# mikelodder7/bls-bn254

Hardware: AMD Instinct MI355X
Metric: BN254 pairings/sec (= BLS verifies/sec) (higher is better)
Workload: dtype int64; 1 GPU; 262144 batched single-sig BLS verifies per GPU (BASELINE configs[1]), unique 32-byte messages, 1024-key pool, 1/64 invalid tuples; key de-duplication + hash-to-G1 + per-key G2 checks and line tables + 2-pair Miller loop + final exp; tuples_per_gpu=262144, tuples_total=262144, key_pool=1024

## Files before the change

### bls-bn254_amd/csrc/bn254_consts.h

```cpp
#pragma once
#include <stdint.h>

#ifndef BN_CONST
#define BN_CONST static constexpr
#endif

namespace bnc {
BN_CONST int32_t P[9] = {410844487, 17064118, 477274959, 47522512, 361093496, 47923392, 10936641, 240920116, 3171406};
BN_CONST int32_t PINV = 75916169;
BN_CONST int32_t ONE[9] = {360500257, 337389400, 408039635, 21759001, 178483129, 490881230, 299191303, 86689704, 903222};
BN_CONST int32_t R2[9] = {94088208, 219480995, 25171640, 279645352, 40052281, 46143135, 379321683, 294034764, 2757030};
BN_CONST int32_t R3[9] = {237179570, 381705378, 197673865, 484389131, 296595421, 53368462, 493544588, 282381599, 2540242};
BN_CONST int32_t LC_QINV = 1420063842;
BN_CONST int32_t THREE[9] = {7758947, 475297290, 150377082, 65277005, 535449387, 398901866, 360702999, 260069113, 2709666};
BN_CONST int32_t INV2[9] = {385672372, 177226759, 174221841, 303076213, 269788312, 269402311, 155063972, 163804910, 2037314};
BN_CONST int32_t B2[18] = {189306456, 13619797, 266050167, 47090167, 3383508, 443974981, 116276700, 275414465, 1651051, 463465696, 132959441, 275378631, 215966963, 22334433, 231877312, 116106472, 422158901, 2635577};
BN_CONST int32_t B2_3[18] = {157074881, 23795273, 320875542, 93747989, 185927940, 210259726, 337893461, 48452367, 1781748, 31837202, 364750088, 408456887, 15984952, 418558132, 62914238, 326446135, 247765559, 1563920};
BN_CONST int32_t GAMMA1[5][18] = {{168567705, 446838140, 21606957, 76005147, 193575774, 320063457, 492961205, 101471925, 3016032, 466013235, 394132337, 371054763, 25204381, 93145077, 448361909, 29518381, 483951129, 39811}, {77959568, 116720857, 200831163, 387972444, 449106301, 79574741, 198110247, 444835091, 2396851, 286535409, 187804871, 492312764, 403373079, 442701694, 360078139, 294614062, 104485018, 1269326}, {455018104, 57932550, 320278461, 408777911, 37819167, 383878197, 519288526, 32534274, 1918653, 430327765, 436072363, 496131354, 220163167, 145517765, 530932250, 323946238, 161949718, 1410845}, {276953182, 328873349, 306900296, 55370336, 434202341, 186067288, 221116544, 233072759, 1472337, 258042488, 93586473, 404468614, 107881851, 15098452, 202552781, 251052073, 472003299, 457208}, {122035596, 70559408, 351843991, 185247759, 294359775, 74527549, 415682662, 131659696, 1090544, 515197319, 148204830, 209777112, 355922816, 112506023, 137088316, 422875504, 397322748, 530422}};
BN_CONST int32_t GAMMA2[5][9] = {{239698866, 192365459, 64358326, 265999499, 489041563, 23351122, 297356679, 439555315, 2382159}, {416069521, 391846970, 193189602, 244240497, 310558434, 69340804, 535036287, 352865610, 1478937}, {50344230, 216545630, 69235323, 25763511, 182610367, 93913074, 248616249, 154230411, 2268184}, {171145621, 361569571, 412916632, 318393925, 408922844, 24572269, 250450874, 338235712, 789246}, {531645878, 162088059, 284085356, 340152927, 50535061, 515453500, 12771265, 424925417, 1692468}};
BN_CONST int32_t GAMMA3[5][18] = {{241843517, 234894524, 489670951, 377358109, 130864789, 78929213, 242247822, 507627824, 1062952, 256797489, 98403818, 382339799, 433159222, 464404099, 29325343, 50434485, 281019966, 1260793}, {325889741, 432474136, 497955025, 42907526, 200183625, 441570494, 324828416, 301853753, 830815, 115639766, 437132463, 279613835, 73502212, 128670103, 395362884, 114011013, 518486521, 2516630}, {492697295, 496002479, 156996497, 175615513, 323274328, 200916107, 28519026, 208385841, 1252753, 517387634, 117862666, 518014516, 364230256, 215575730, 53862054, 223861314, 78970397, 1760561}, {184051396, 109191840, 495742184, 2670331, 316545484, 294905530, 164669302, 459358945, 1341039, 164889335, 177818119, 378890167, 153193343, 453739841, 53273248, 261318439, 380451190, 765836}, {51698174, 235788407, 418091187, 111773928, 225157088, 39558942, 371182386, 248871861, 1328219, 456881720, 277261468, 92031488, 462668576, 36360912, 212656789, 36108422, 250118305, 1231319}};
BN_CONST int32_t SVDW1_C2[9] = {25172115, 376708271, 303053117, 281317211, 91305183, 315391993, 392743580, 77115205, 1134092};
BN_CONST int32_t SVDW1_C3[9] = {457867599, 493380231, 379858106, 195829369, 20951404, 495257235, 515507638, 211660318, 1792024};
BN_CONST int32_t SVDW1_C4[9] = {109710923, 387889788, 190128975, 352751795, 248555410, 536056522, 40444610, 278758817, 2582763};
BN_CONST int32_t SVDW2_C1[18] = {12935801, 351009198, 137218890, 68849169, 181866637, 397985299, 415468004, 362104169, 2554273, 463465696, 132959441, 275378631, 215966963, 22334433, 231877312, 116106472, 422158901, 2635577};
// ... 39 lines not shown
 {115099161, 361079548, 480148518, 71065809, 413241065, 213126723, 432045244, 299309372, 2268741, 479074021, 348462957, 481692425, 148329581, 64011363, 70419451, 521873344, 159891040, 1324744, 119836463, 250094397, 193017529, 386788224, 428020408, 460771368, 482124439, 421522847, 2425238, 114910552, 328830817, 11540419, 482736450, 81017752, 486418694, 265295458, 205803990, 2412182, 471973933, 150650886, 367600592, 532165343, 430851147, 71155045, 529417599, 178863249, 2191828, 149969822, 426570128, 207472835, 315629756, 133685872, 381189636, 408236876, 327074418, 2188814},
 {2478238, 482236155, 501863109, 216695776, 28133897, 438520593, 478660467, 318003266, 1199697, 192081406, 317937999, 456709271, 526466273, 394728539, 38972406, 212519731, 400106547, 2012913, 378934760, 47780458, 414894863, 300049921, 288627557, 408469358, 444317404, 488663036, 2672762, 13086186, 54236397, 108682135, 92393923, 530514305, 27778254, 105809252, 74710849, 1556614, 209361150, 110510140, 95590690, 157282884, 446948412, 348799352, 455938463, 212273705, 163832, 22070713, 354671070, 84392107, 19937692, 97762133, 428281814, 341164088, 59197099, 2715522},
 {323421647, 351258179, 370279306, 155471307, 424415674, 102275476, 212021690, 87559554, 2340702, 24917374, 235021524, 380342478, 363149794, 227411753, 120703908, 347780407, 368601500, 1628846, 507626604, 130345934, 352142788, 446766788, 227299145, 486890448, 454258698, 432658924, 408411, 387464107, 181431778, 517543077, 450507408, 274152061, 386795811, 316647274, 2653065, 905024, 198687098, 19198232, 468880961, 497531179, 72028957, 445451261, 151597031, 505066845, 266617, 206165872, 383877063, 381756925, 495881619, 309259073, 79698217, 517080274, 394408755, 2370170},
 {330978764, 415936193, 276560320, 10789241, 32709856, 415578960, 204566554, 49026968, 543671, 401282904, 295457946, 459543498, 302532038, 234545929, 435390597, 51269616, 516181269, 989503, 266870546, 37427281, 314094762, 90273590, 90847638, 271513304, 186487054, 352454449, 2617924, 121748973, 147192770, 247959206, 301823486, 444621093, 436582923, 209240503, 422347226, 2002793, 420766975, 95012043, 358452079, 193159195, 332239088, 408573222, 533896885, 168668931, 923997, 225978358, 445442889, 464494416, 256553974, 330088769, 112529492, 268007525, 39581098, 1275248},
 {185059858, 384384543, 195532834, 80761347, 97799465, 380065039, 58976876, 123141856, 1462600, 186838709, 402104131, 276126867, 284741457, 500488675, 514410526, 383061266, 124796755, 2244826, 358011933, 4036403, 469238339, 440068960, 527373348, 334506535, 314766696, 488109457, 2091722, 220763289, 483546112, 315308719, 294479989, 264693218, 504773378, 400722538, 128766796, 1203159, 65502050, 407313301, 102089550, 95898178, 179009806, 249585945, 234878215, 121313140, 2105165, 522286217, 258485470, 418821949, 263539889, 530843810, 16465869, 522864618, 524681011, 866705},
 {491409221, 429532559, 480645853, 526305085, 519184946, 320384023, 366557187, 456445003, 2372451, 46004574, 88114142, 272844542, 240504887, 245152710, 72343087, 452772496, 490931390, 1930332, 365820376, 405670191, 215780242, 398527698, 97510772, 57808733, 25497632, 300993947, 1861604, 101472942, 268743662, 483215740, 262103703, 80623359, 433243363, 270577248, 136079810, 1692806, 526258616, 299110836, 467583615, 175386471, 241633693, 128812340, 475159413, 424889297, 1355872, 334828240, 46302060, 197547862, 437505136, 209280222, 106201003, 250871306, 428783560, 1572123},
 {65131922, 410853902, 281504673, 233607083, 165164706, 161931360, 387368130, 258266354, 2803919, 334380832, 303564680, 469329650, 483978437, 60138085, 65833456, 505774265, 488845355, 732811, 194000581, 438170323, 339874851, 141778324, 114422087, 230441886, 438429275, 99559190, 2946642, 6220226, 12487337, 220716112, 200924448, 81207124, 390196574, 461793634, 229660081, 2302755, 306224412, 191690856, 481273302, 249777865, 233058066, 485912801, 218562582, 429376852, 1812935, 255465103, 179692905, 1478937, 74345539, 513148142, 382481949, 310578590, 389597509, 1275258},
 {275949305, 3228312, 176617213, 302484708, 457024271, 263059331, 258622837, 245199256, 753406, 83841931, 325585899, 277349460, 285128688, 326328912, 15480993, 328169666, 377039357, 2396459, 113270026, 65870630, 96437477, 351096554, 325570632, 198444115, 76462694, 155120365, 996406, 430904607, 193902953, 272620064, 90269516, 102608309, 337293318, 397393431, 355475286, 1895729, 375002109, 523542794, 420835100, 244089057, 314065940, 170681387, 283594264, 200076913, 2351283, 353523119, 365025453, 508021136, 56738678, 102892269, 28605850, 410461759, 165297750, 821801},
 {121101037, 453866970, 408871889, 451715554, 319641813, 194199547, 316486552, 91089131, 808524, 120712549, 135431654, 172072906, 201228322, 470008586, 492966518, 374156269, 532936882, 1168971, 139848472, 40102183, 376920765, 120695385, 9222022, 119036174, 436556597, 431412384, 2480448, 23738614, 100086658, 394051529, 460935441, 426465533, 18451757, 232407558, 515618330, 3011560, 519254845, 256846000, 49605046, 137916175, 344616592, 289345685, 442010228, 227801899, 2750281, 504706552, 99608927, 62959779, 78824121, 378301691, 404974492, 52973827, 431879000, 2103752},
 {57437006, 445209922, 267906252, 61434842, 322380891, 448223867, 314779795, 384467504, 98050, 334623576, 504282724, 410457003, 436857817, 525051919, 379539104, 397162175, 488788414, 1675650, 128798474, 528278283, 271532147, 514886753, 436331545, 85538213, 175830542, 327291145, 2932702, 208811182, 439681250, 485915822, 399974237, 30558037, 318044875, 130194579, 172655195, 2132450, 111448047, 492105644, 275356637, 284787949, 242551611, 425462594, 410102729, 25366096, 965123, 377085709, 111491603, 279628206, 536659377, 363545763, 491060748, 301344554, 217747788, 1765858},
 {189278316, 267054422, 240015347, 263190437, 268026589, 217837374, 213394387, 324721961, 1939655, 362977484, 158704421, 436353096, 498602143, 463553294, 108055305, 173810290, 461672636, 189796, 355213020, 343977698, 358822065, 74044511, 88139862, 518079515, 72571544, 488865441, 562373, 93928340, 179514280, 470213355, 1500725, 59659302, 351864698, 514900587, 277607281, 746298, 424483532, 62821806, 533803893, 328740056, 62104696, 109448841, 488087329, 28719095, 615035, 503689154, 324055796, 273308548, 138602345, 93139326, 227059809, 225062543, 520012847, 1690627},
 {434873579, 345866943, 464692431, 147843125, 214244731, 167340668, 8535887, 135091946, 590262, 507331706, 281122125, 71877124, 182009353, 98073037, 426692907, 256966410, 31385127, 323754, 339206185, 397108277, 158683218, 198966473, 323954183, 410647148, 250511836, 182487353, 2192260, 211663655, 166315194, 278738998, 465340566, 135530598, 220476821, 98038085, 475663347, 689443, 238385349, 45648702, 24191268, 223060677, 56805038, 492858003, 15855826, 219362042, 3169653, 55560961, 496756213, 531337177, 231583741, 370701323, 20903764, 26651393, 72508891, 2939698},
 {370857545, 162561793, 349584675, 305666799, 424318849, 265355541, 335744858, 332264862, 2077939, 229675399, 202135034, 507349300, 66038434, 502299596, 462886795, 216432890, 367950568, 434967, 522930393, 349612231, 359055418, 269223224, 415375677, 73806834, 81410003, 7609490, 2168856, 440219586, 266804181, 348682996, 471526334, 56329094, 445035356, 495708785, 177697745, 1049347, 9590362, 463810573, 472790040, 104478950, 123428722, 344683645, 15445838, 441601197, 345029, 127193134, 22917997, 445375356, 264481634, 418186335, 190775382, 385157115, 441341282, 1622947},
 {525120466, 302156262, 14026670, 79200301, 83863473, 269053555, 271350554, 5118602, 814247, 242412219, 10262438, 115069724, 182751693, 222411097, 463282269, 302495598, 467832431, 433135, 381586988, 376949966, 525473891, 378543561, 528450195, 305002078, 5175203, 530287687, 1864236, 8631814, 399428070, 64818853, 409693044, 53480096, 59985746, 424529766, 117917599, 1958550, 211074005, 241353131, 202088806, 153585924, 274879141, 376560831, 74310929, 362992403, 3023538, 304629166, 231842783, 202606994, 59312311, 437826184, 276953349, 202252965, 152929408, 1380202},
 {45243310, 3113997, 475224255, 399655383, 489901630, 394589394, 219453609, 389562620, 647105, 185052378, 203306772, 510086849, 66201807, 28034831, 265674449, 483208661, 117079303, 2245361, 383725158, 56590503, 238874043, 474720702, 354626127, 5216587, 380497232, 382251138, 2156761, 450163084, 327454365, 96195373, 340957541, 93272866, 447418125, 393654147, 336425233, 1261490, 243056404, 202839389, 291276410, 39489301, 522755053, 433239394, 200191913, 132407280, 995738, 87800718, 39891742, 201642557, 267980703, 381147787, 142064039, 166874100, 148109070, 2183155},
 {419483032, 417302961, 209411699, 395420027, 11875312, 472825098, 25023783, 122248361, 428482, 187120796, 434311260, 523941697, 312353488, 185625814, 149803502, 25267919, 437641082, 58048, 482147204, 44437673, 333141396, 416903804, 328735750, 68751396, 54000275, 18754495, 469924, 118281153, 196797377, 510480140, 174090217, 180762717, 327840995, 522381987, 342541943, 526514, 29386787, 379334880, 495343353, 138079880, 149085614, 205670571, 338603247, 518281092, 947371, 28951025, 167201315, 357427458, 165861015, 133055956, 147545106, 497514072, 418967957, 3122782},
 {40100442, 79249802, 481205136, 295669236, 516832659, 295740353, 154473360, 42698217, 616919, 459226082, 367489041, 172493783, 10772752, 310333315, 469796297, 456832918, 360513025, 1387582, 439740854, 47345612, 232672811, 422188955, 500323364, 225266534, 163349333, 306515768, 477242, 1545029, 11878491, 315137521, 386388304, 482799752, 234821666, 494159689, 490739196, 2025658, 285921861, 387365880, 273585049, 37311821, 367688208, 434533702, 464362157, 527184610, 954346, 423936018, 309641240, 457531941, 133017943, 116916181, 145496292, 266826109, 174694208, 2322607},
 {103410007, 80269727, 107803116, 266138348, 159613881, 218210149, 270129094, 176926138, 1971950, 309770860, 398343381, 531806047, 171136374, 168818136, 221670885, 445114296, 275892636, 1101592, 163848103, 166760855, 355771815, 124065591, 415188034, 189131208, 248659651, 402708254, 845530, 148218911, 225224981, 183319510, 1438760, 465281999, 261483438, 422864871, 401738498, 504587, 259044379, 431246755, 284927319, 98392988, 492002560, 58293889, 86402116, 213719941, 265596, 252917965, 237345777, 96756592, 402569146, 168468661, 174375631, 211020977, 148122777, 1839569},
 {129175245, 7036991, 394205927, 109118652, 420701990, 532730783, 488070123, 230275807, 2505420, 321568924, 108179418, 122921434, 177770554, 127113816, 508034739, 2160192, 484284904, 868789, 464634736, 175998503, 492000730, 81605521, 144765489, 520986768, 305919411, 374066204, 1890535, 237833058, 199277185, 484650377, 114512057, 271342938, 136767975, 392520660, 135535363, 237972, 13806109, 25620002, 460701052, 81031906, 83471693, 347825173, 448355234, 165472987, 2836179, 302810733, 180092351, 371937405, 67528704, 521484666, 251274010, 324067318, 98241568, 319197},
 {402590907, 390173797, 9154836, 91637093, 116097568, 135498950, 412674480, 471852445, 2103104, 45623282, 236388520, 320757064, 250739701, 507203558, 20784063, 349913224, 513830445, 2930463, 191231464, 229262617, 499329381, 391457563, 220103625, 381273631, 121452801, 230708984, 498416, 147675469, 451341783, 356690434, 416036715, 453518419, 195069465, 248991557, 21133377, 2515482, 261837599, 70126348, 170486479, 536345815, 457557007, 123485984, 176457550, 352037844, 849911, 261382441, 87117387, 517387878, 11753697, 168073425, 454808552, 195965950, 96105394, 152175},
 {12512508, 150856564, 395596226, 482091269, 260215011, 354438027, 103441014, 126419430, 252738, 185766822, 521899918, 261643314, 35208125, 305510146, 363820929, 116324864, 100331033, 889085, 500803016, 169611288, 74978053, 271459858, 455136968, 68056467, 40076531, 480527470, 1897865, 429796490, 142915065, 500099793, 459002478, 523553815, 134475327, 405370676, 140840092, 549968, 210967111, 414065589, 351375835, 413127406, 104682486, 235355711, 345576955, 518068253, 1825719, 121695489, 84303843, 520551157, 246713071, 76169206, 128032100, 440504967, 283651112, 366320},
 {54903692, 367398404, 389045954, 103195443, 201407156, 480670888, 520034811, 444665162, 3120009, 301192230, 292344168, 276000918, 329190306, 3207403, 16097252, 377466566, 108801895, 994934, 105164645, 400152816, 477217800, 290340033, 389232304, 248469600, 306422360, 405666417, 1265718, 149978886, 10882107, 96650353, 374648105, 145056091, 209481887, 236014373, 478750587, 1172417, 444164896, 369905875, 51408743, 373893873, 98743229, 307012172, 257015135, 227181011, 2381844, 74179049, 426041869, 180979714, 318267506, 239942663, 263940057, 98072905, 311978671, 150141},
 {142543935, 194580705, 343370161, 391345662, 400042802, 407410933, 413139956, 149550188, 1289303, 528816066, 209720920, 443679922, 400086828, 52320843, 454328967, 413721629, 77976075, 2253187, 63450331, 336126245, 200366993, 8503761, 143191089, 388781579, 24290118, 17560612, 1567680, 243745881, 20656753, 365319391, 73839146, 311195635, 406562419, 388374104, 497778204, 3159579, 268334596, 285203294, 517702133, 517615536, 191607223, 305927169, 398996176, 435289825, 2199364, 296375027, 511422668, 142534303, 147541973, 486527664, 61071306, 133290627, 151365941, 1871814},
 {381447695, 112910439, 164681691, 372267774, 388906816, 442672654, 510817020, 138003284, 2517538, 425925494, 321328277, 407413632, 350272519, 159281071, 490821086, 202786933, 286727689, 2119816, 55117854, 313308608, 360606396, 31742223, 248771333, 255469023, 125500679, 80632572, 2951938, 172822145, 292032153, 304786787, 355702891, 253612283, 295485534, 208552501, 432316545, 2682878, 110822812, 210734962, 393571010, 96421268, 38795732, 58694143, 397188728, 387473943, 102932, 206765486, 143677095, 226830287, 496832911, 260610526, 345967722, 332677737, 83704810, 3148352},
 {62108095, 226732454, 161554664, 324339612, 474398800, 445689529, 310205044, 313295877, 1595036, 521570690, 127595162, 438734366, 44995759, 228814373, 19627764, 211169583, 247295664, 1457005, 60863200, 454338684, 63660680, 436100826, 109781091, 65244919, 193527964, 354189242, 1393252, 219704311, 38957286, 110544435, 160893735, 455670807, 348774005, 138075414, 285707688, 2608894, 1804324, 271533511, 299758214, 352967878, 95296562, 186071519, 83272051, 302583396, 3001394, 128153566, 500555465, 271034625, 432533768, 477284868, 92329198, 324969194, 32623276, 130038},
 {215582193, 126912476, 309311231, 10076884, 314222891, 377366770, 530443407, 477083200, 793328, 533386876, 492530023, 503245648, 91516679, 182906897, 194062228, 492389562, 65590782, 1324892, 38561070, 245414554, 189970182, 152394919, 426151917, 512289777, 22015761, 436702070, 1185947, 52392166, 143466253, 184054606, 364397472, 432510246, 197302902, 148253681, 4271025, 931440, 360382279, 38184803, 427074753, 343932430, 308401295, 504780952, 201263072, 266062393, 424201, 111188963, 450073465, 372852080, 68120216, 21855192, 136104731, 230467091, 249100444, 3131167},
 {503242147, 126031175, 99598615, 332469802, 118529903, 103654630, 336983131, 48695070, 1281178, 122799682, 274622884, 507281707, 415629719, 306308862, 223464264, 75647452, 467875001, 1287621, 286610889, 85716239, 122268177, 517793089, 118854096, 284240661, 109341172, 523299060, 2430687, 247263262, 94849538, 54280861, 507432969, 291253094, 256077794, 441645252, 213205037, 2917285, 155215960, 392828217, 154713476, 366149965, 187736848, 395762272, 411133922, 457751113, 1834994, 523850929, 350840427, 299600675, 379383303, 402170387, 224236460, 187366553, 196507477, 392568},
 {261404048, 60806940, 100479668, 287812062, 271915223, 198406602, 238340931, 408086811, 1901426, 324109934, 513219976, 214408304, 345497341, 221162477, 531649800, 49370849, 170138307, 1040769, 332267139, 126565143, 105261738, 156831366, 427218173, 526690558, 398325027, 48992578, 3150187, 148926025, 82340276, 232496043, 105691656, 409427567, 191008174, 462567125, 144338561, 719208, 136997521, 211607581, 55265913, 93560900, 155893330, 50711175, 522835196, 432651475, 1167786, 104425542, 178779151, 290349679, 84423272, 313764025, 519966625, 405776928, 459400273, 2933873},
 {310825741, 384456194, 426889952, 532157184, 489413414, 222371274, 254619296, 305726429, 1200037, 226431895, 191449196, 147394219, 512980816, 112239727, 123673014, 345317845, 68260117, 1834849, 158028187, 373938733, 55317016, 281026384, 386220711, 418030963, 103573954, 71301023, 478347, 23351998, 306678241, 111291365, 453611291, 112088103, 99686904, 79519778, 510270407, 926535, 214206952, 82455080, 241084664, 103779255, 360047249, 26043312, 42338008, 263251530, 2293413, 431541426, 164219745, 91904174, 107196656, 359655013, 207187685, 211089583, 28421216, 2693257},
 {128984559, 408128418, 354064874, 279268254, 470256108, 48320565, 91070471, 175298789, 521515, 339864578, 231958707, 225812807, 90243946, 198929659, 262631414, 187740668, 131953518, 679825, 302468239, 395971309, 196126185, 197552126, 16644241, 520798160, 194513995, 448317350, 2671784, 88087896, 328335140, 144335943, 102062007, 340283116, 286846647, 176155623, 365474765, 2487316, 363197687, 306159665, 453821877, 77580983, 243190174, 115169461, 197970032, 182888387, 163558, 134896947, 35963039, 144316924, 219126585, 120283426, 274799187, 533258181, 527633730, 480391},
 {341746340, 308302796, 430625402, 101511254, 466164565, 480666054, 127770429, 443615350, 2308080, 31431165, 319419446, 227721353, 416355218, 141796468, 120324224, 177014659, 409950156, 1927475, 251290807, 478940226, 446910893, 212080491, 429870139, 311429590, 433888467, 97060592, 2428767, 308935399, 254634792, 494014342, 484461508, 175949596, 222997971, 507697494, 6855563, 198079, 331310478, 8636836, 78610090, 167333250, 276995305, 320565486, 401578983, 468493720, 186082, 443619717, 57975269, 125159984, 199762973, 384348548, 303284969, 146339162, 141845832, 1661690},
 {380822515, 156254098, 174290075, 379414457, 498231268, 451298257, 449171729, 433962997, 1742136, 195831119, 281549253, 311228002, 399685262, 205543257, 93314873, 366022684, 481414289, 964076, 360837042, 96132473, 323506526, 129202646, 438203512, 195211450, 25899375, 118356221, 267310, 276216682, 373509754, 38238354, 220219388, 80173204, 222174402, 128252521, 284030621, 959358, 499785411, 80697964, 282876190, 191336693, 179576951, 247438212, 357625786, 298992331, 1304370, 318099190, 58142073, 352186437, 84637684, 459118970, 185918866, 263207063, 136859350, 17203},
 {22201984, 265618155, 5732562, 312280272, 428285398, 399081532, 390586660, 195672556, 384993, 197544349, 359334084, 379212116, 533597950, 121884326, 345868827, 250766308, 176976589, 2405209, 150296893, 352839861, 187428747, 309943127, 398751357, 183724921, 90389245, 393368450, 1055795, 193582117, 421104415, 345293445, 131519433, 445932976, 357186327, 87574441, 195345724, 2546016, 390825220, 219248238, 282044142, 139758925, 128477841, 37456477, 445576370, 475394833, 2077533, 50169050, 205628584, 22939628, 483296354, 138203379, 489066399, 528359038, 87569497, 1779567},
 {485635694, 91489940, 369095772, 277539277, 69873299, 58285921, 140553732, 404251382, 2338306, 384638836, 65644667, 41235970, 423864904, 172015351, 369068400, 268252068, 306791038, 409687, 30563928, 183319989, 102070816, 85226297, 514801246, 240250988, 532874397, 449593201, 2734700, 207295019, 516870558, 429981826, 110660854, 477085381, 429989041, 52354241, 150924792, 1646533, 113663700, 536839513, 306803055, 112881191, 439661605, 246706288, 18664305, 501459450, 1317964, 341627473, 76166713, 146626525, 1733909, 8778891, 371460037, 535514595, 103941542, 2880078},
 {219122481, 521376588, 48819747, 453090089, 232489950, 529687297, 126590199, 192595820, 2170623, 158964325, 138670954, 70538403, 433509637, 268378921, 159736347, 167078372, 472007564, 2642738, 146711122, 180163548, 79656276, 62999074, 427174551, 174151461, 236927641, 94058253, 827399, 498654006, 153397663, 31817787, 244161073, 334416319, 71911351, 298777560, 319420192, 2250830, 299438274, 421802083, 189128091, 59988885, 196191526, 48343, 23947445, 384065173, 2999593, 222421153, 352796023, 419827954, 204257747, 197219243, 481381734, 483432526, 136798688, 2510232},
 {471399504, 225290108, 479825663, 208285264, 95998907, 247686025, 476587084, 415349662, 2989291, 415430977, 42648197, 36657301, 434095102, 342823308, 92920887, 189264745, 364268235, 3098747, 236437400, 450843323, 95084128, 118707480, 37831298, 505369479, 80648224, 409498161, 516702, 383869702, 412856052, 472404438, 404526549, 520906484, 262355910, 465546569, 176317220, 384400, 307844836, 237693820, 335097902, 439545630, 248997287, 116103597, 43530126, 360074078, 887654, 256539533, 189232881, 521948944, 130137976, 494864697, 533420778, 467441818, 242664914, 2360911},
 {6341116, 258953661, 130165135, 121567663, 85734040, 362525194, 446386664, 221487232, 2418285, 67600948, 254157951, 226775185, 363959709, 120458917, 42640378, 417110163, 232465096, 3078420, 427739614, 188726393, 495980930, 324226172, 384839974, 411097953, 276079125, 472007051, 859799, 164129877, 494401711, 448417012, 366162538, 6462208, 155008799, 72770354, 166128252, 2791168, 227075349, 108651955, 255460112, 376253096, 521726666, 203860061, 217738487, 89258585, 1761282, 438061118, 265245702, 341611701, 71841372, 494561940, 345314017, 454454515, 308232774, 512869},
 {388123801, 82315330, 42726244, 478978184, 473426981, 319753532, 223939613, 159127356, 716500, 91233489, 486241299, 190304271, 364630277, 369664745, 215648258, 16385655, 360116749, 1604186, 292146332, 131277078, 438844626, 524436726, 498055021, 91158254, 171272336, 82826493, 2900140, 237091141, 248682792, 356460465, 216723839, 48245380, 247622337, 483244203, 179351009, 2746259, 116116257, 365456058, 154479586, 192349368, 85192525, 289995721, 112977154, 92335699, 136314, 452992599, 385210575, 1099038, 238791418, 18935313, 89476660, 301485804, 217597180, 2954969},
 {136943908, 18208356, 404922159, 463169914, 311803918, 346171465, 11838672, 423116572, 540100, 141896998, 195863719, 45697336, 192503381, 256542019, 81673477, 43642530, 38848267, 1468289, 508779843, 75730439, 209636058, 457851658, 304698551, 458293478, 392091706, 422667130, 468044, 398299416, 470320832, 173064410, 465823042, 365112625, 59195844, 439497728, 70241388, 2477266, 419402448, 215564443, 199572801, 265196137, 177356156, 176224811, 196089759, 315451236, 108510, 136072149, 428681825, 334127467, 452465188, 203237528, 73965396, 232642935, 428577660, 734022},
 {440860920, 83597737, 71788760, 4773679, 460570279, 223207920, 436035796, 398734372, 656541, 481111816, 66740800, 118181206, 218954997, 242302821, 354825473, 189551084, 288107682, 1228799, 79417144, 142486372, 312428128, 275428832, 316981410, 237485005, 224672500, 191667892, 495131, 412962820, 462769059, 312027323, 119892722, 218910436, 5847613, 239249143, 479317593, 138253, 337396732, 218879545, 30296354, 13955357, 421024186, 57906020, 191012581, 137209362, 2722985, 135005313, 375307002, 418714293, 327448236, 516046957, 298981707, 281311663, 232523326, 787909},
 {421882971, 346072605, 213508351, 124603514, 12713635, 387029899, 153312083, 356938635, 3135484, 185025588, 392430028, 30735720, 162160774, 68103380, 68360853, 56078781, 374528341, 1284754, 97299261, 147709562, 382526238, 25706632, 411103733, 17887524, 102419314, 158212278, 2179507, 68756409, 408623604, 525390344, 331525772, 69339206, 464082682, 137855506, 393884866, 3019165, 300006882, 173952888, 216039979, 255807306, 176378987, 388535127, 280690262, 536698090, 2484175, 468135898, 34190575, 211134462, 454582962, 169066562, 330433300, 483525464, 387667530, 148723},
 {332227983, 57357084, 334050684, 43489651, 482498330, 304681939, 341896219, 443742571, 2437451, 12250895, 160665840, 219191270, 36256471, 386592779, 444851143, 325838334, 352243405, 1474793, 479082934, 431105170, 97846306, 105778213, 138739391, 505974881, 147824753, 72435794, 2757268, 106049943, 25102438, 360775953, 376983765, 122671492, 333355075, 52176328, 435301593, 715756, 532854540, 193948231, 505703644, 523162571, 218455565, 509630947, 8980570, 358113216, 920581, 13158795, 17751672, 57746186, 414675497, 472210620, 4708792, 226710205, 49341192, 1376576},
 {430955708, 264381247, 337096023, 351853749, 20383220, 411008042, 59652391, 330831616, 2659533, 408978128, 191887919, 105571894, 232797019, 43766784, 309332417, 268493775, 33580806, 1649466, 264590990, 346513002, 245153061, 291939935, 302699159, 458351889, 422831022, 172176136, 2582643, 249931154, 155575599, 37643848, 494072352, 83127062, 216595132, 119157193, 144910063, 1938120, 301984105, 187990127, 519334054, 103086537, 482009609, 426075322, 524567878, 105731577, 3056969, 135091568, 190493310, 134058471, 383578297, 451388586, 306348237, 362414496, 152852857, 2313526},
 {156049048, 348569387, 345912211, 108243764, 39862758, 340985293, 526986285, 486529373, 2756757, 70148830, 361656205, 232267683, 499676662, 55080252, 11325608, 388061743, 373594328, 877029, 397671269, 400681839, 65130041, 262490050, 283062759, 405415808, 461459608, 489448736, 2202039, 397115625, 518867667, 227573257, 57170780, 47003329, 192147289, 32943434, 36595122, 2904836, 418071867, 224056616, 380555394, 61600834, 220544322, 101581422, 126185470, 370629032, 1587125, 422449844, 210141206, 495244492, 159725210, 393378025, 459104351, 413093230, 535784292, 2467414},
 {374971361, 189256118, 514349215, 260192216, 201693892, 46684475, 86038945, 45798971, 596475, 354780560, 166199176, 126676648, 20087358, 8163231, 443871444, 380934380, 15879837, 2832889, 52684906, 521371086, 390867791, 101904211, 260915672, 182440845, 68224676, 228157599, 2402653, 8442567, 370238665, 105072341, 281343440, 475493017, 519100621, 421211414, 331232706, 2713541, 415194087, 506485752, 184326039, 87917025, 118769502, 421077858, 366086855, 347850511, 643412, 210607613, 239757828, 257344574, 176541047, 126352649, 461160536, 325971653, 410321501, 1859419},
 {346138147, 183589712, 192669952, 440482540, 335490519, 23087938, 38013450, 414816160, 11088, 402635274, 508754875, 528205898, 260674993, 208706555, 339115408, 323234820, 179171832, 2221386, 426553627, 112047373, 385712345, 300968502, 341498138, 355471730, 142898578, 70820285, 1765035, 281326098, 143615771, 294300190, 343890894, 12537596, 236250928, 171742033, 81667137, 2226899, 25416948, 345664344, 167296106, 520318029, 241956023, 57184892, 494901324, 60468401, 2000935, 2993812, 152844357, 515142068, 274834179, 461835240, 279725567, 239967821, 348485226, 1472537},
 {430272925, 523309779, 159176126, 64114552, 7599812, 275194210, 227486424, 402628020, 2147710, 32902820, 490191070, 54357085, 533266873, 395036647, 424428525, 535518286, 280410232, 2920968, 296779742, 412228251, 503765170, 218914658, 241878384, 230177558, 468682218, 424848977, 1394588, 233801316, 236752259, 172198580, 293699517, 62687391, 221253270, 499455778, 153199542, 3046004, 279442699, 160682080, 321402742, 22130196, 534886950, 418643497, 231459356, 133404613, 1211833, 455283136, 111355409, 446906248, 441602466, 348034517, 263104034, 400474216, 170955027, 2605900},
 {436035161, 247373067, 125798067, 389725623, 6288592, 42833077, 516498379, 521445566, 1886790, 184263419, 48195789, 422452995, 231173944, 533728815, 88671371, 207203408, 367383526, 2267220, 203108664, 193164284, 180890202, 528984086, 354640285, 258786511, 136754148, 530754252, 2435046, 412114265, 158840910, 4204732, 381206110, 524422907, 105857206, 48027475, 171131517, 1288815, 235451170, 399660963, 214158541, 316727956, 497939107, 332057718, 116914421, 231502284, 67606, 420272217, 412168364, 271325459, 335552449, 90905491, 64178567, 201413962, 442922653, 1121259},
 {299184217, 414960404, 318291790, 185622238, 367049483, 402495234, 341748370, 437982520, 2045795, 19477984, 249305720, 429912029, 461389527, 315066191, 275999417, 180961226, 139859282, 2826593, 39144516, 55422143, 4587787, 206150160, 396564513, 477425243, 495183114, 206289587, 6552, 117906371, 101024087, 510444434, 453278004, 175014561, 229819228, 350767294, 441008500, 3142255, 7426088, 133832626, 356941477, 309926291, 274258323, 486660256, 289374288, 235101466, 357776, 34819623, 244190314, 358405397, 443658477, 357664916, 174948832, 204568663, 198916489, 1795169},
 {344880916, 485864836, 128038544, 183700157, 303951303, 417725573, 29735238, 331651302, 1803381, 354013505, 44946024, 97088622, 470300883, 10632754, 49099620, 532392985, 471635872, 444945, 182853991, 422119400, 276418095, 116677872, 48565822, 5255579, 432637183, 237201307, 949170, 402960287, 234588459, 424200806, 60774998, 201936971, 269440315, 135570892, 497241165, 1473037, 98814076, 69597269, 71295596, 514821842, 217886650, 153833815, 131588020, 427103757, 966636, 295915695, 460908713, 377597627, 517877798, 458919916, 225274860, 124292261, 111683940, 2746827},
 {518656702, 488249738, 7278702, 290418227, 225912336, 394700482, 530898514, 259426784, 1978070, 361278641, 183914759, 52646095, 242709033, 72608589, 219216813, 56677820, 330469468, 2371300, 428300565, 180500926, 160633184, 517116766, 10598290, 22285930, 316776114, 126200239, 1447245, 478054283, 132434667, 127134921, 299595849, 231458914, 188088751, 465838830, 156854382, 1010051, 124319470, 431725364, 256338614, 513617633, 270873983, 212643967, 248921239, 519052682, 2280194, 306994602, 241460816, 250923483, 31965397, 19740949, 213555458, 216627367, 45246112, 120116},
 {293160492, 245941755, 73442732, 404135672, 207614525, 120178985, 379937182, 89551655, 621586, 79473740, 337984177, 79264647, 93294149, 7971693, 393334056, 368916157, 81801052, 2106207, 440306136, 503791711, 479588939, 489491137, 410166973, 14621930, 505587363, 488473959, 887037, 380514496, 52096291, 310971389, 45923102, 370044752, 93285453, 332980638, 63634843, 1130600, 392821194, 418824308, 240376313, 224275292, 455434369, 277669007, 371906250, 373704681, 310847, 331214354, 510727251, 123531010, 152463125, 442565065, 42499403, 310012621, 233375412, 1687544},
 {459544001, 391471594, 25575482, 192315806, 512283260, 229830790, 296261571, 189785566, 1994877, 533652656, 511037612, 138939831, 267891826, 271878679, 362676324, 403256550, 7446027, 1593828, 398539344, 524236377, 201010774, 383778641, 315414171, 26786658, 123832312, 185180095, 2602473, 213570084, 481028506, 53314778, 168675715, 346762600, 456335430, 134019067, 372692310, 1393242, 31664457, 47744192, 466416925, 304247197, 340814346, 87836883, 327891107, 332472178, 1815581, 227941551, 222271169, 9261168, 405098383, 161968106, 375092235, 169346447, 46544412, 781100},
 {481548188, 214741736, 240350070, 12012500, 377756157, 270945313, 50135567, 45913065, 884284, 456765927, 289042023, 195839783, 67043321, 432298369, 280901733, 96207641, 420493817, 2718622, 388852431, 322343875, 283482318, 315017940, 465898945, 349554570, 53095133, 226022090, 2016489, 392942489, 334126532, 394229114, 60241890, 35434634, 280761896, 416868051, 351542500, 2734105, 283240893, 88720328, 344233496, 511860616, 128181406, 282487018, 181873990, 6976297, 3167753, 477651976, 456530921, 317767618, 190821317, 233115539, 139469982, 367863448, 58909471, 1662784},
 {202767458, 453256221, 40761137, 446365799, 365985752, 446050190, 497895002, 41047040, 3095360, 74607829, 444889648, 523552515, 145945486, 404457399, 251028894, 93766472, 372001962, 100303, 170138087, 193614804, 318792614, 439536147, 477434124, 228485055, 534091926, 155749842, 2276449, 405215224, 444385000, 524465072, 211904860, 30038886, 442931262, 502463559, 152695011, 2089704, 149956433, 312575983, 59240429, 436435538, 62833367, 11191233, 438260993, 17344802, 1937400, 439218886, 403065571, 193234881, 12915827, 501712098, 93787484, 392498397, 403859438, 1016411},
 {436656284, 359905360, 101223246, 489351504, 3657958, 384101949, 411196791, 380427572, 2571034, 393485923, 208952735, 521386055, 481096, 239270552, 32414421, 179291139, 171927397, 969014, 498233196, 178876263, 470532999, 2665997, 469647577, 229911587, 74856801, 112939172, 2001555, 416183585, 181587888, 175524846, 491051689, 408447450, 455605718, 324931618, 4689734, 488914, 333638614, 401276274, 535821439, 48345823, 316619007, 298189350, 409219897, 220762652, 989429, 186867115, 260273710, 349435877, 403490373, 93917204, 144732036, 175749141, 388077615, 2517682},
 {287574667, 195537458, 497438093, 285360180, 145888726, 33019073, 258962939, 137762083, 2183989, 514390807, 414879403, 400777039, 371818954, 184570898, 380591635, 54817320, 467430913, 420463, 270933454, 498342011, 116808119, 403954222, 342364641, 30811629, 67526331, 369389871, 69412, 109168654, 89512855, 320028402, 418325651, 410409818, 275971329, 98753658, 373947392, 131243, 406899020, 164738448, 66826334, 481117969, 514460024, 117856498, 439611387, 301623572, 881303, 254359548, 150778625, 397147446, 400927161, 311807650, 291267789, 210433882, 458123653, 889392},
 {529634438, 395020387, 108093242, 475767096, 289150317, 237339105, 438871389, 229144053, 863679, 367571939, 57943390, 252342320, 453230619, 534849941, 39507622, 256714209, 97288288, 502696, 476782345, 227320360, 12420741, 239942260, 428908049, 370993522, 524227993, 117952539, 39613, 524531981, 381845637, 465982430, 272568792, 16808060, 153088464, 296339629, 371493215, 2469462, 421277729, 389812836, 167537784, 365554318, 128762787, 447247816, 123616227, 145939449, 928609, 397386148, 336421292, 521321073, 247639461, 229285539, 85996274, 383972709, 258664804, 1653094},
 {206961616, 381079739, 269593227, 402726100, 14538206, 444867933, 70904296, 387084730, 842917, 363453306, 416500523, 467532540, 413073582, 447013703, 179563435, 162474537, 245531731, 1148209, 252576564, 285412103, 88916683, 43311484, 96753579, 364204461, 372433977, 262971741, 1488142, 514833759, 441119544, 214499877, 381724849, 532269602, 170892059, 462648916, 394029910, 3088805, 317182934, 203370385, 229723113, 167901654, 420180670, 421862275, 475961650, 157282786, 606030, 170565178, 133408998, 307215134, 140651646, 274714847, 428926323, 210858395, 437580467, 1611559},
 {428117646, 34022814, 154722467, 132755685, 122068739, 493618771, 139622274, 172498314, 2847252, 291633030, 274194775, 531858012, 144402698, 196681234, 9258711, 314775141, 528082404, 2673935, 463441689, 123768625, 3948302, 86001732, 338857223, 191043638, 119408198, 52181253, 1749096, 359249064, 109688593, 94402094, 181413537, 186492090, 24969004, 488664237, 449160119, 406543, 114508015, 102789443, 459719719, 408889277, 26876464, 115711357, 287223829, 481968893, 1990518, 439490694, 75124594, 294181975, 526377703, 197129499, 271661232, 471150834, 30721416, 2422508},
 {242939259, 412783622, 471303906, 192058816, 105613554, 200351016, 185651272, 116111166, 380075, 116919016, 44980791, 118255186, 336201211, 492185226, 215423527, 535352552, 298494615, 330685, 468809653, 273377370, 415937808, 356085620, 305055772, 234561145, 115126109, 412038193, 2330777, 226531982, 531939410, 196877215, 205982089, 450956423, 184374411, 43456923, 326110495, 1332390, 495507394, 153926551, 386101394, 312990856, 210150327, 83320656, 174813766, 401693105, 2304832, 142919764, 427347211, 262488407, 255935794, 267272831, 363987954, 192572795, 414162563, 311899},
 {492850946, 83178123, 253668660, 474965034, 436447538, 24145095, 79743109, 174938088, 1825060, 319698026, 215683917, 224311769, 170490546, 382977480, 425031066, 458737052, 519196122, 490490, 23400646, 413713278, 183752261, 122853282, 307960228, 485960869, 506338186, 323599517, 2359325, 128015026, 98186099, 186918078, 500109092, 265222921, 384663883, 336091284, 78604597, 1543388, 528217684, 519346581, 136688447, 135308455, 417532446, 532591185, 366571968, 264784252, 1490877, 59145682, 93913550, 246772293, 374924084, 76451296, 496346135, 115518558, 400766082, 2779322},
 {74427174, 316623412, 23675861, 334126763, 13176646, 232809289, 155541939, 72228454, 2041212, 223546547, 39809592, 430026316, 461496123, 103565608, 186511401, 376911596, 173378117, 2013790, 148348236, 428852572, 533703899, 8051787, 259534980, 154770121, 287113594, 176515032, 2128049, 304215290, 285689321, 49950046, 312168505, 56098899, 396352110, 106689639, 83980306, 112317, 428157728, 421524631, 342427138, 493639879, 178570351, 279205191, 19926514, 340648123, 537251, 205965075, 487813757, 479910751, 261176063, 22342432, 483891590, 78435476, 443577918, 40148},
 {245617288, 123175829, 297826511, 458896068, 241764471, 231632607, 359840708, 280803868, 1903173, 208825547, 199996367, 459909105, 234782504, 76292385, 515020774, 464695317, 335518206, 1507300, 443788596, 506199681, 325325070, 285054850, 513447046, 300959514, 350146814, 261232659, 1056560, 511066014, 165963439, 506953704, 224195656, 167564066, 85118324, 450098451, 528850463, 2136823, 454347216, 490807827, 399975633, 229421869, 164096225, 459597559, 326414675, 336617775, 2755194, 373766664, 351697410, 127130679, 260765326, 100562905, 479367856, 368211999, 293492131, 1866570},
 {245059318, 463441635, 322639623, 428310962, 276526834, 259438497, 259460084, 284033542, 1914551, 446196205, 71389884, 28378485, 227051864, 24899243, 319354978, 403507892, 142246580, 1035731, 383275586, 383407055, 62259511, 43124759, 438435885, 220904326, 67527927, 451988882, 1158168, 265697257, 192397136, 283611844, 241128875, 224521733, 507674344, 505150213, 313413044, 2764367, 88931525, 125647936, 210359394, 81090266, 400614554, 488361106, 91717877, 376314259, 2657259, 124767231, 515059692, 169614140, 147285524, 148427957, 469343083, 405195547, 184094142, 2282633},
 {283949290, 224585391, 387868692, 134470700, 303193727, 448046774, 352543777, 211263354, 2798858, 194293620, 393760483, 497938725, 503905221, 429888991, 80080179, 498291004, 175629855, 2516950, 352383472, 134024744, 163753863, 347850850, 85651656, 214018496, 350423646, 346299626, 923916, 247508017, 297963687, 273418374, 173382835, 52468082, 519077880, 116994839, 282382304, 917907, 223092338, 327407993, 65285009, 51077305, 57230120, 288595597, 358338612, 353896855, 3000924, 361066685, 148632114, 424642269, 118560696, 213195914, 102741443, 396098212, 463778511, 80713},
 {283112081, 62163922, 15285746, 184678173, 416946919, 422793912, 427895760, 169272309, 478315, 493550027, 267712255, 22406168, 366289293, 534932369, 314255603, 228325538, 106989998, 2279429, 278652919, 455265061, 491187464, 515942130, 439087513, 55731747, 165162718, 226315791, 1706004, 419312073, 331338263, 501464547, 23996291, 88136940, 346944743, 441707665, 244460432, 1716749, 216670401, 179999684, 532912431, 315997436, 1457314, 463396740, 412632783, 529692613, 1363030, 15814396, 455016475, 358234367, 324799376, 507454070, 191107457, 48521367, 535342990, 469131},
 {353724426, 246951758, 356895745, 263153409, 166221217, 527460908, 408776437, 180329720, 2074466, 350542864, 172693688, 528929391, 449515530, 242628823, 502634791, 325881967, 326418351, 2824014, 6211503, 172822135, 487595616, 235534058, 83694625, 250324374, 59949222, 358315171, 140984, 456021003, 245324642, 478802151, 358788042, 86103668, 11744115, 84313809, 326569761, 1543169, 65445570, 99254724, 261961647, 242735888, 158766603, 422676747, 54714193, 95543337, 2526467, 379539315, 142863568, 420734362, 133156177, 479080502, 331652827, 361501306, 195531172, 476820},
 {317549885, 198697761, 249380953, 495123692, 453947158, 249203722, 86749406, 417148591, 1475877, 237283213, 3241341, 423184088, 18795847, 427863335, 16040214, 110200455, 251524210, 1536713, 107639984, 20072597, 149189468, 428015298, 504385698, 37314867, 385750891, 414404719, 27851, 33958399, 385169620, 498529230, 401284295, 454333519, 321731256, 390462645, 184294845, 3078660, 494095629, 58065239, 58845098, 384312739, 456755048, 286073792, 286791495, 339282540, 2514723, 514391628, 359967790, 36516999, 194259209, 203785548, 255357864, 504836880, 394958850, 726555},
 {311633655, 131811432, 25398033, 403841593, 322115575, 411293880, 18124295, 313074943, 1758952, 465227322, 342407623, 150372597, 248889719, 483108493, 484579230, 497417539, 52196962, 835321, 385381891, 33104285, 128891397, 175809299, 508462802, 113213291, 143378814, 330223714, 3111509, 8907364, 425999037, 12685138, 129991581, 183470742, 354061234, 479225391, 324114126, 794985, 104661603, 134083376, 498763072, 523935167, 84413167, 420274427, 372011915, 266936511, 1832300, 245545999, 459057437, 317368478, 118888668, 205600319, 155899518, 528397898, 148747741, 2503274},
 {281479439, 528562003, 363098899, 336344374, 334922502, 19252294, 219010773, 120096268, 334925, 469435664, 522063190, 321990810, 322313526, 34411411, 155471800, 439756490, 13265237, 2678778, 307714251, 387237933, 281157113, 458703192, 295248262, 150067309, 239439310, 458374633, 294731, 505677572, 418978856, 261146195, 418595975, 48411027, 317828536, 428175647, 395441932, 2462780, 102022309, 268732306, 533037255, 196300118, 309364786, 353571676, 169172951, 455255622, 617142, 100882411, 18013065, 473322700, 1072795, 361513363, 288652241, 15588916, 481236440, 1708153},
 {78571987, 361177887, 443998338, 263075369, 70263042, 493726944, 535962191, 127043271, 240062, 397136396, 210646202, 390127152, 167668320, 248745889, 101020297, 476579152, 219747776, 2761125, 41140832, 184387078, 146744831, 256252326, 49807238, 449542423, 227261990, 260471214, 3062208, 525127283, 301154849, 324701277, 365662396, 341585785, 211435912, 180828780, 33088091, 1542729, 277290806, 363851994, 435830295, 358876156, 309952369, 71088530, 33326580, 365431691, 2484596, 228693420, 442482570, 179541425, 186143321, 468865264, 184526935, 430176262, 329282558, 1978018},
 {334852098, 447934948, 79443961, 129228070, 24354253, 48477975, 454023539, 409993992, 2734970, 252455794, 88354609, 238705096, 337451121, 509324887, 377113426, 353457692, 484461504, 3151075, 30273128, 38294371, 95800251, 283261923, 11148736, 412039228, 283771755, 78282908, 332934, 466452697, 408280540, 68630333, 400795547, 363393231, 451322782, 513557020, 87708113, 2516599, 1474989, 245982418, 413800578, 447897561, 302850044, 426778887, 172716362, 449729011, 905236, 446215920, 174849968, 188780190, 128296608, 187418943, 281206446, 333755580, 368298541, 534803},
 {363697647, 285325938, 434722059, 45579462, 201973848, 474212666, 509636120, 184182192, 2064968, 234715851, 38141659, 178588306, 534136360, 7939644, 350012596, 12958086, 298819088, 2993351, 216734195, 240593912, 425991579, 523032660, 208302347, 46323594, 225474280, 435024773, 620780, 218895451, 112326747, 455023803, 408508051, 293004444, 376821145, 226784757, 60787535, 203412, 89496320, 94265377, 166096921, 444267378, 388934921, 180246479, 82754499, 199580496, 1055662, 397155459, 158822569, 235174623, 386896911, 163916411, 273528224, 411861325, 410622147, 328359},
 {201488625, 50957238, 102304395, 380060116, 223771241, 130517402, 435321712, 299390440, 2235652, 108535259, 444775626, 77579088, 31956246, 210186067, 306243370, 385817896, 372735497, 321894, 385233421, 180622935, 409074521, 198964499, 283286026, 308937856, 399091608, 264124425, 1002653, 96082886, 457455230, 184729783, 483382084, 41502754, 223103679, 41738397, 295708136, 2011427, 226581221, 308353232, 355792123, 466623293, 297947519, 355198579, 2931546, 491778089, 1313650, 64242208, 249109684, 65494917, 93199926, 276018694, 138777245, 129213055, 389657785, 1072199},
 {45705453, 143714487, 86307088, 78913109, 147374975, 180957191, 151133129, 489339976, 1771405, 473819502, 18118557, 535636238, 480177567, 333137611, 375380390, 286843472, 468899487, 2820877, 384183509, 191736051, 225531995, 291298185, 245563785, 502637833, 161583766, 457641843, 725657, 495758470, 499253568, 253172769, 342707160, 105926098, 70835746, 86210055, 18923348, 1992080, 475781590, 43350802, 343223350, 458816390, 91405471, 412690255, 460119077, 198442996, 1152636, 260405015, 266436221, 492905943, 532643754, 101236968, 286896498, 298117023, 69177552, 1088979},
 {142623616, 73447938, 472968444, 281091874, 108821799, 419205582, 252984000, 82673195, 1081090, 370209387, 255472044, 183573082, 80973558, 27971357, 21261924, 281424325, 422863884, 2866203, 226861365, 297493201, 87406300, 200247153, 515720525, 243992102, 251901746, 261600094, 1404379, 30950022, 226078069, 96689508, 302682309, 219162382, 53852572, 307069894, 520566561, 519903, 312360512, 399813465, 147484965, 45860077, 366845051, 485642865, 202533828, 245786935, 2240314, 483140654, 424156184, 171736471, 392447265, 310743250, 285399021, 231132855, 110553928, 1580353},
 {518950315, 166524578, 318973779, 208801084, 203654704, 518574409, 367342361, 212732044, 267211, 346834938, 311664457, 28289258, 166837241, 185476264, 240293064, 27521832, 41500912, 1827852, 192671097, 463723310, 318425315, 219804188, 228021022, 450959355, 320662857, 355567309, 381911, 54390987, 531844638, 277544222, 259123543, 351332576, 198209147, 230796763, 144375015, 1532825, 313852906, 129182620, 290984000, 322011448, 398352613, 263155621, 226583053, 196853404, 1278929, 326310244, 117621872, 410625076, 82125642, 397095880, 409752438, 248834139, 338630724, 1320201},
 {55878625, 108956286, 398558293, 380795966, 327699164, 96727383, 441060671, 240953991, 485316, 335290700, 164606168, 447327121, 346715094, 3829772, 157458878, 207194831, 80360049, 320838, 8715817, 280742723, 46597024, 443039108, 287762215, 93179656, 466061073, 203112441, 2378325, 79434527, 121708912, 229280302, 10141767, 246110096, 93770821, 391394252, 478945112, 696660, 367903438, 292984164, 303749863, 10248808, 474419406, 225020304, 479091881, 505749740, 917582, 155299559, 269273660, 392448063, 36485923, 93297644, 265708075, 431439551, 207339751, 1846136},
 {493808963, 482302668, 204399090, 362293888, 514159840, 378918588, 426691502, 472571071, 2351725, 413910404, 15913881, 204492988, 247758060, 412134986, 115823135, 66968791, 299334015, 1262480, 188930798, 194294115, 45816802, 99693215, 358389925, 168281711, 63684769, 296317229, 2275024, 438763849, 504132989, 531624029, 187379805, 61104814, 363323519, 377087611, 256199988, 2311937, 167379084, 375468130, 502802420, 67689135, 41456191, 503979958, 305671863, 354691468, 317874, 60197100, 137848056, 55566537, 386244007, 258790455, 13634469, 73766086, 292447699, 1528865},
 {248938176, 350466153, 134753901, 435380835, 72917553, 156155176, 291307518, 32259336, 1028390, 379779376, 231645262, 229723036, 193965067, 153531491, 375312851, 491839129, 441506130, 1041786, 115764437, 313016821, 369953093, 454752130, 484813132, 417728943, 512613884, 477427683, 2993031, 253811470, 122990100, 443458760, 301470983, 82635724, 51241845, 135246996, 100410326, 735740, 106669830, 500727615, 185253398, 80759155, 174390583, 427362052, 435938546, 75098748, 2455921, 158248225, 274759410, 28245215, 72408984, 11419683, 86345775, 16182697, 81920639, 3124442},
};
#endif
```

### bls-bn254_amd/csrc/fp29.h

```cpp
#pragma once
#include <stdint.h>
#include "bn254_consts.h"

#if defined(__HIPCC__)
#include <hip/hip_runtime.h>
#define BN_HD __host__ __device__
#else
#define BN_HD
#endif
#define BN_INL BN_HD inline __attribute__((always_inline))
#ifdef BN_FORCE_INLINE
#define BN_FUNC BN_INL
#else
#define BN_FUNC BN_HD inline
#endif

#define BN_UNROLL _Pragma("unroll")
#if defined(__HIP_DEVICE_COMPILE__)
#define BN_SCHED_BARRIER __builtin_amdgcn_sched_barrier(0)
#else
#define BN_SCHED_BARRIER ((void)0)
#endif

#ifdef BN_CHECK
// ... 353 lines not shown
  ok = c < 0;
  return fp_to_mont(x);
}
BN_INL void fp_to_be(uint8_t* b, const Fp& a) {
  Fp c = fp_from_mont(a);
  uint32_t w[8];
  limbs_to_words(w, c.l);
  BN_UNROLL for (int j = 0; j < 8; ++j) store_be32(b + 4 * (7 - j), w[j]);
}
BN_INL Fp fp_from_okm(const uint8_t* okm) {
  uint32_t w[12];
  BN_UNROLL for (int j = 0; j < 12; ++j) w[j] = load_be32(okm + 4 * (11 - j));
  Fp lo, hi;
  BN_UNROLL for (int i = 0; i < NL; ++i) {
    int bit = RB * i, j = bit >> 5, s = bit & 31;
    uint32_t v = w[j] >> s;
    if (s > 32 - RB) v |= w[j + 1] << (32 - s);
    lo.l[i] = (int32_t)(v & (uint32_t)MASK);
  }
  BN_UNROLL for (int i = 0; i < NL; ++i) {
    int bit = RB * (i + NL), j = bit >> 5, s = bit & 31;
    uint32_t v = 0;
    if (j < 12) { v = w[j] >> s; if (s > 32 - RB && j + 1 < 12) v |= w[j + 1] << (32 - s); }
    hi.l[i] = (int32_t)(v & (uint32_t)MASK);
  }
  BN_TRK(set_trk(lo, 0, 1, 0, 1, 170); set_trk(hi, 0, 1, 0, 0, 1e-30);)
  return fp_dot2(lo, fp_const(bnc::R2), hi, fp_const(bnc::R3));
}

struct Exp256 { uint64_t w[4]; };
#define BN_EXP(name) (::bn::Exp256{{bnc::name[0], bnc::name[1], bnc::name[2], bnc::name[3]}})
BN_FUNC Fp fp_pow(const Fp& a, Exp256 e) {
  Fp tab[16];
  tab[0] = fp_one();
  tab[1] = fp_norm(a);
  for (int i = 2; i < 16; ++i) tab[i] = fp_mul(tab[i - 1], tab[1]);
  const uint64_t e0 = e.w[0], e1 = e.w[1], e2 = e.w[2], e3 = e.w[3];
  Fp r = tab[(int)(e3 >> 60)];
  for (int w = 62; w >= 0; --w) {
    uint64_t word = w >= 48 ? e3 : w >= 32 ? e2 : w >= 16 ? e1 : e0;
    int d = (int)((word >> ((w & 15) * 4)) & 15);
    Fp t = tab[d];
    BN_SCHED_BARRIER;
    r = fp_sqr(r); r = fp_sqr(r); r = fp_sqr(r); r = fp_sqr(r);
    r = fp_mul(r, t);
  }
  return r;
}
BN_FUNC Fp fp_inv_pow(const Fp& a) { return fp_pow(a, BN_EXP(EXP_PM2)); }

BN_INL void sg_divsteps29(int32_t& zeta, uint32_t f, uint32_t g, int32_t& u, int32_t& v, int32_t& q, int32_t& r) {
  u = 1; v = 0; q = 0; r = 1;
  BN_UNROLL for (int i = 0; i < RB; ++i) {
    int32_t c1 = zeta >> 31;
    const int32_t c2 = -(int32_t)(g & 1u);
    const uint32_t x = (f ^ (uint32_t)c1) - (uint32_t)c1;
    const int32_t y = (u ^ c1) - c1, z = (v ^ c1) - c1;
    g += x & (uint32_t)c2; q += y & c2; r += z & c2;
    c1 &= c2;
    zeta = (zeta ^ c1) - 1;
    f += g & (uint32_t)c1; u += q & c1; v += r & c1;
    g >>= 1; u *= 2; v *= 2;
  }
}
template <bool MODP>
BN_INL void sg_update(int32_t* a, int32_t* b, int32_t u, int32_t v, int32_t q, int32_t r) {
  int64_t ca = (int64_t)u * a[0] + (int64_t)v * b[0], cb = (int64_t)q * a[0] + (int64_t)r * b[0];
  int32_t ka = 0, kb = 0;
  if (MODP) {
    ka = (int32_t)(((uint32_t)ca * (uint32_t)bnc::PINV) & (uint32_t)MASK); kb = (int32_t)(((uint32_t)cb * (uint32_t)bnc::PINV) & (uint32_t)MASK);
    ca += (int64_t)ka * bnc::P[0]; cb += (int64_t)kb * bnc::P[0];
  }
  ca >>= RB; cb >>= RB;
  BN_UNROLL for (int i = 1; i < NL; ++i) {
    const int32_t ai = a[i], bi = b[i];
    ca += (int64_t)u * ai + (int64_t)v * bi; cb += (int64_t)q * ai + (int64_t)r * bi;
    if (MODP) { ca += (int64_t)ka * bnc::P[i]; cb += (int64_t)kb * bnc::P[i]; }
    a[i - 1] = (int32_t)((uint32_t)ca & (uint32_t)MASK); b[i - 1] = (int32_t)((uint32_t)cb & (uint32_t)MASK);
    ca >>= RB; cb >>= RB;
  }
  a[NL - 1] = (int32_t)ca; b[NL - 1] = (int32_t)cb;
}
constexpr int SG_BATCHES = 21;
BN_FUNC Fp fp_inv(const Fp& a) {
  const Fp x = fp_from_mont(a);
  int32_t f[NL], g[NL], d[NL], e[NL];
  BN_UNROLL for (int i = 0; i < NL; ++i) { f[i] = bnc::P[i]; g[i] = x.l[i]; d[i] = 0; e[i] = i == 0 ? 1 : 0; }
  int32_t zeta = -1;
  for (int b = 0; b < SG_BATCHES; ++b) {
    int32_t u, v, q, r;
    sg_divsteps29(zeta, (uint32_t)f[0] | ((uint32_t)f[1] << RB), (uint32_t)g[0] | ((uint32_t)g[1] << RB), u, v, q, r);
    sg_update<false>(f, g, u, v, q, r);
    sg_update<true>(d, e, u, v, q, r);
  }
  int32_t gnz = 0;
  BN_UNROLL for (int i = 0; i < NL; ++i) gnz |= g[i];
#if defined(__HIP_DEVICE_COMPILE__)
  if (__builtin_amdgcn_ballot_w64(gnz != 0) != 0) return fp_inv_pow(a);
#else
  if (gnz != 0) return fp_inv_pow(a);
#endif
  const bool neg = f[NL - 1] < 0;
  Fp di;
  BN_UNROLL for (int i = 0; i < NL; ++i) di.l[i] = neg ? -d[i] : d[i];
  BN_TRK(set_trk(di, -1, 1, -0.14, 0.14, 22);)
  return fp_mul(di, fp_const(bnc::R2));
}
BN_FUNC Fp fp_sqrt_cand(const Fp& a, bool& is_sq) {
  Fp y = fp_pow(a, BN_EXP(EXP_PP1_4));
  is_sq = fp_eq(fp_sqr(y), a);
  return y;
}

BN_INL uint32_t bn_funnel_shr(uint32_t hi, uint32_t lo, uint32_t k) {
#if defined(__HIP_DEVICE_COMPILE__)
  return __builtin_amdgcn_alignbit(hi, lo, k);
#else
  return (uint32_t)((((uint64_t)hi << 32) | lo) >> k);
#endif
}
BN_FUNC bool fp_is_square(const Fp& x) {
  Fp c = fp_canon(x);
  uint32_t a[8], n[8];
  limbs_to_words(a, c.l);
  limbs_to_words(n, bnc::P);
  uint32_t t = 0;
  for (int it = 0; it < 520; ++it) {
    const uint32_t k = (uint32_t)__builtin_ctz(a[0] | 0x80000000u);
    BN_UNROLL for (int j = 0; j < 7; ++j) a[j] = bn_funnel_shr(a[j + 1], a[j], k);
    a[7] >>= k;
    t ^= k & ((n[0] >> 1) ^ (n[0] >> 2));
    const uint32_t odd = a[0] & 1u;
    uint32_t d[8], borrow = 0;
    BN_UNROLL for (int j = 0; j < 8; ++j) {
      const uint64_t v = (uint64_t)a[j] - n[j] - borrow;
      d[j] = (uint32_t)v; borrow = (uint32_t)(v >> 63);
    }
    const uint32_t swap = odd & borrow;
    t ^= swap & ((a[0] & n[0]) >> 1);
    const uint32_t sm = 0u - swap, om = 0u - odd;
    uint32_t carry = swap, nz = 0;
    BN_UNROLL for (int j = 0; j < 8; ++j) {
      const uint64_t v = (uint64_t)(d[j] ^ sm) + carry;
      carry = (uint32_t)(v >> 32);
      n[j] = swap ? a[j] : n[j];
      a[j] = (a[j] & ~om) | ((uint32_t)v & om);
      nz |= a[j];
    }
#if defined(__HIP_DEVICE_COMPILE__)
    if (__builtin_amdgcn_ballot_w64(nz != 0) == 0) break;
#else
    if (nz == 0) break;
#endif
  }
  return (t & 1u) == 0;
}

}
```

### bls-bn254_amd/csrc/host_verify.hip

```cpp
#include "host_common.h"

extern "C" {


int launch_g2_prepare(blsbn254_ctx* c, hipStream_t s, const uint8_t* pks, const uint32_t* keys, size_t u, int32_t* raw, uint8_t* ok, const uint32_t* d_u) {
  if (c->quad_prep && 8 * u <= c->lanes_per_round)
    return launch(c, s, "g2_prepare", grid_lanes(2 * 256 * (size_t)nblocks(4 * u)), k_g2_prepare_quad, pks, keys, (uint32_t)u, raw, ok, d_u);
  return launch(c, s, "g2_prepare", grid_lanes(2 * 256 * (size_t)nblocks(u)), k_g2_prepare, pks, keys, (uint32_t)u, raw, ok, d_u);
}
int prepare_keys_async(blsbn254_ctx* c, const uint8_t* d_pks, const uint32_t* d_keys, size_t u, int32_t* table, uint8_t* key_ok, const uint32_t* d_u) {
  HIPCHK(c, c->prep_raw.reserve(u * PREP_RAW_LIMBS * 4));
  HIPCHK(c, fork_stream2(c));
  TRY(launch_g2_prepare(c, c->stream2, d_pks, d_keys, u, (int32_t*)c->prep_raw.p, key_ok, d_u));
  TRY(launch(c, c->stream2, "g2_expand", grid_lanes(u * (size_t)BN_NEG_G2_LINES), k_g2_expand, (const int32_t*)c->prep_raw.p, (uint32_t)u, table, d_u));
  HIPCHK(c, hipEventRecord(c->ev_join, c->stream2));
  return 0;
}
int check_key_indices(blsbn254_ctx* c, const uint32_t* d_kid, size_t n, size_t u, uint32_t* hist, const char* what, bool armed) {
  if (!armed) { HIPCHK(c, c->misc.reserve(64)); TRY(min_index_arm(c, (int*)c->misc.p, 1)); }
  int* d_bad = (int*)c->misc.p;
  HIPCHK(c, hipMemsetAsync(hist, 0, 4 * u, c->stream));
  TRY(launch(c, c->stream, "kd_hist", grid_lanes(n), k_kd_hist, d_kid, (uint32_t)n, (uint32_t)u, hist, d_bad));
  int bad;
  TRY(min_index_read(c, d_bad, &bad));
  if (bad >= 0) { c->last_error = std::string("key index out of range at ") + what + " " + std::to_string(bad); return BLSBN254_E_ARG; }
  return 0;
}
int launch_miller_prepared(blsbn254_ctx* c, const uint32_t* perm, const uint32_t* kid, const uint8_t* sigs, const int32_t* h_ws, size_t h_stride,
                           const int32_t* table, const uint8_t* key_ok, size_t n) {
  int32_t* f = (int32_t*)c->f_ws.p; uint8_t* flags = (uint8_t*)c->flags.p;
  if (c->wide_fe && n <= c->wide_fe_max)
    return launch(c, c->stream, "miller_wide_prepared", grid_wide(n), k_miller_wide_prepared, perm, kid, sigs, h_ws, h_stride, table, key_ok, n, f, flags);
  if (n <= c->tri_max && c->tri_miller)
    return launch(c, c->stream, "miller_tri_prepared", grid_tri(n), k_miller_tri_prepared, perm, kid, sigs, h_ws, h_stride, table, key_ok, n, f, flags);
  return launch(c, c->stream, "miller_prepared", grid_lanes(n), k_miller_prepared, perm, kid, sigs, h_ws, h_stride, table, key_ok, n, f, flags);
}
int verify_prepared_dev(blsbn254_ctx* c, const int32_t* table, const uint8_t* key_ok, size_t u, const uint32_t* d_kid, bool hist_done,
                               const uint8_t* d_msgs, const uint64_t* d_off, const uint8_t* d_sigs, size_t n, uint32_t dl, uint8_t* d_bitmap, bool join) {
  HIPCHK(c, c->h_ws.reserve(n * 27 * 4)); HIPCHK(c, c->f_ws.reserve(n * 108 * 4)); HIPCHK(c, c->flags.reserve(n));
  HIPCHK(c, c->kd_hist.reserve(4 * (u + 1))); HIPCHK(c, c->kd_cursor.reserve(4 * (u + 1))); HIPCHK(c, c->kd_perm.reserve(4 * n));
  HIPCHK(c, c->prep_isone.reserve(n)); HIPCHK(c, c->prep_valid.reserve(n));
  uint32_t* hist = (uint32_t*)c->kd_hist.p; uint32_t* cursor = (uint32_t*)c->kd_cursor.p; uint32_t* perm = (uint32_t*)c->kd_perm.p;
  TRY(launch(c, c->stream, "hash_to_g1", grid_lanes(n), k_hash_to_g1, d_msgs, d_off, n, (const uint8_t*)c->dst.p, dl, (int32_t*)c->h_ws.p, n, (uint8_t*)nullptr,
             3));
  if (!hist_done) TRY(check_key_indices(c, d_kid, n, u, hist, "tuple", false));
  TRY(launch(c, c->stream, "kd_scan", Shape{dim3(1), dim3(1024)}, k_scan_excl, (const uint32_t*)hist, (uint32_t)u, cursor));
  TRY(launch(c, c->stream, "kd_scatter", grid_lanes(n), k_kd_scatter, d_kid, (uint32_t)n, (uint32_t)u, cursor, perm));
  if (join) HIPCHK(c, join_stream2(c));
  TRY(launch_miller_prepared(c, perm, d_kid, d_sigs, (const int32_t*)c->h_ws.p, n, table, key_ok, n));
  int rc = run_final_exp(c, (int32_t*)c->f_ws.p, n, n, 4, nullptr, nullptr, nullptr, (uint8_t*)c->prep_isone.p, nullptr);
  if (rc) return rc;
  TRY(launch(c, c->stream, "prep_unsort", grid_lanes(n), k_prep_unsort, (const uint8_t*)c->prep_isone.p, (const uint8_t*)c->flags.p, (const uint32_t*)perm, (uint32_t)n,
             (uint8_t*)c->prep_valid.p));
  return launch(c, c->stream, "pack_bitmap", grid_lanes(n), k_pack_bitmap, (const uint8_t*)c->prep_valid.p, n, d_bitmap);
}
static int dedup_enqueue(blsbn254_ctx* c, const uint8_t* d_pks, size_t n) {
  size_t m = 1;
  while (m < 2 * n) m <<= 1;
  HIPCHK(c, c->kd_slots.reserve(4 * m)); HIPCHK(c, c->kd_rep.reserve(4 * (n + 1))); HIPCHK(c, c->kd_kid.reserve(4 * (n + 1))); HIPCHK(c, c->kd_keys.reserve(4 * (n + 1)));
  HIPCHK(c, c->kd_hist.reserve(4 * (n + 2))); HIPCHK(c, c->kd_cnt.reserve(64));
  HIPCHK(c, hipMemsetAsync(c->kd_slots.p, 0xff, 4 * m, c->stream));
  HIPCHK(c, hipMemsetAsync(c->kd_cnt.p, 0, 4, c->stream));
  TRY(launch(c, c->stream, "kd_insert", grid_lanes(n), k_kd_insert, d_pks, (uint32_t)n, (uint32_t*)c->kd_slots.p, (uint32_t)(m - 1), c->kd_seed, (uint32_t*)c->kd_rep.p));
  return launch(c, c->stream, "kd_assign", grid_lanes(n), k_kd_assign, (const uint32_t*)c->kd_rep.p, (uint32_t)n, (uint32_t*)c->kd_kid.p, (uint32_t*)c->kd_cnt.p, (uint32_t*)c->kd_keys.p);
}
int dedup_keys(blsbn254_ctx* c, const uint8_t* d_pks, size_t n, size_t* u_out) {
  int rc = dedup_enqueue(c, d_pks, n);
  if (rc) return rc;
  uint32_t u = 0;
  TRY(download(c, &u, c->kd_cnt.p, 4));
  *u_out = u;
  return 0;
}
int verify_exact_dev(blsbn254_ctx* c, const uint8_t* d_pks, const uint8_t* d_msgs, const uint64_t* d_off,
                            const uint8_t* d_sigs, size_t n, uint32_t dl, uint8_t* d_bitmap) {
  ++c->stat_exact_chunks;
  HIPCHK(c, c->h_ws.reserve(n * 18 * 4)); HIPCHK(c, c->f_ws.reserve(n * 108 * 4));
  HIPCHK(c, c->flags.reserve(n)); HIPCHK(c, c->sub_ok.reserve(n));
  TRY(launch(c, c->stream, "hash_to_g1", grid_lanes(n), k_hash_to_g1, d_msgs, d_off, n, (const uint8_t*)c->dst.p, dl, (int32_t*)c->h_ws.p, n, (uint8_t*)nullptr, 0));
  TRY(launch(c, c->stream, "g2_check", grid_lanes(n), k_g2_check, d_pks, n, (uint8_t*)c->sub_ok.p, (uint8_t*)nullptr));
  TRY(launch(c, c->stream, "miller_verify", grid_lanes(n), k_miller_verify, d_pks, d_sigs, (const int32_t*)c->h_ws.p, n, (int32_t*)c->f_ws.p, (uint8_t*)c->flags.p));
  return run_final_exp(c, (int32_t*)c->f_ws.p, n, n, 0, (const uint8_t*)c->flags.p, (const uint8_t*)c->sub_ok.p, d_bitmap, nullptr, nullptr);
}
int verify_chunk_dev(blsbn254_ctx* c, const uint8_t* d_pks, const uint8_t* d_msgs, const uint64_t* d_off,
                            const uint8_t* d_sigs, size_t n, uint32_t dl, uint8_t* d_bitmap) {
  Stream2Guard s2_guard(c);
  const bool small = small_for_prepared(c, n, true);
  if (c->auto_prepare && (n >= 1024 || small)) {
    size_t u = 0;
    int rc = dedup_keys(c, d_pks, n, &u);
    if (rc) return rc;
    if ((u * 2 <= n || small) && u <= PREP_MAX_KEYS) {
      HIPCHK(c, c->prep_table.reserve(u * PREP_KEY_LIMBS * 4)); HIPCHK(c, c->prep_ok.reserve(u));
      rc = prepare_keys_async(c, d_pks, (const uint32_t*)c->kd_keys.p, u, (int32_t*)c->prep_table.p, (uint8_t*)c->prep_ok.p, nullptr);
      if (rc) return rc;
      HIPCHK(c, hipMemsetAsync(c->kd_hist.p, 0, 4 * u, c->stream));
      TRY(launch(c, c->stream, "kd_propagate", grid_lanes(n), k_kd_propagate, (const uint32_t*)c->kd_rep.p, (uint32_t)n, (uint32_t)u, (uint32_t*)c->kd_kid.p, (uint32_t*)c->kd_hist.p));
// ... 37 lines not shown
  if (rc) return rc;
  HIPCHK(c, hipMemsetAsync(c->kd_hist.p, 0, 4 * cap, c->stream));
  TRY(launch(c, c->stream, "kd_propagate", grid_lanes(n), k_kd_propagate, (const uint32_t*)c->kd_rep.p, (uint32_t)n, (uint32_t)cap, (uint32_t*)c->kd_kid.p, (uint32_t*)c->kd_hist.p));
  rc = verify_prepared_dev(c, (const int32_t*)c->prep_table.p, (const uint8_t*)c->prep_ok.p, cap, (const uint32_t*)c->kd_kid.p, true,
                           d_msgs, d_off, d_sigs, n, dl, d_bitmap, true);
  if (rc) return rc;
  blsbn254_ctx::PendingVerify& pv = c->pend[slot];
  HIPCHK(c, hipMemcpyAsync(c->pend_host + 2 * slot, d_res, 2 * sizeof(uint32_t), hipMemcpyDeviceToHost, c->stream));
  HIPCHK(c, hipEventRecord(pv.ev, c->stream));
  pv.active = true; pv.d_pks = d_pks; pv.d_msgs = d_msgs; pv.d_off = d_off; pv.d_sigs = d_sigs; pv.n = n; pv.d_bitmap = d_bitmap;
  pv.dst_len = dst_len;
  if (dst_len) std::memcpy(pv.dst, dst, dst_len);
  ++c->pend_count;
  ++c->stat_async_chunks;
  return 0;
}
int resolve_pending(blsbn254_ctx* c, bool blocking) {
  while (c->pend_count) {
    blsbn254_ctx::PendingVerify& pv = c->pend[c->pend_head];
    if (!blocking && hipEventQuery(pv.ev) != hipSuccess) { (void)hipGetLastError(); break; }
    HIPCHK(c, hipEventSynchronize(pv.ev));
    const uint32_t u = c->pend_host[2 * c->pend_head], ok = c->pend_host[2 * c->pend_head + 1];
    const blsbn254_ctx::PendingVerify done = pv;
    pv.active = false;
    c->pend_head = (c->pend_head + 1) & 3; --c->pend_count;
    if (ok) { c->u_hint = u ? u : 1; if (u > c->u_max_seen) c->u_max_seen = u; ++c->stat_prepared_chunks; continue; }
    ++c->stat_async_reruns;
    c->u_hint = 0;
    uint32_t dl; int rc = stage_dst(c, done.dst, done.dst_len, &dl);
    if (rc) return rc;
    rc = verify_chunk_dev(c, done.d_pks, done.d_msgs, done.d_off, done.d_sigs, done.n, dl, done.d_bitmap);
    if (rc) return rc;
  }
  return 0;
}
static int verify_batch_dev_impl(blsbn254_ctx* c, const uint8_t* d_pks, const uint8_t* d_msgs, const uint64_t* d_off,
                                 const uint8_t* d_sigs, size_t n, const uint8_t* dst, size_t dst_len, uint8_t* d_bitmap, bool allow_async) {
  if (!c || (n && (!d_pks || !d_off || !d_sigs || !d_bitmap)) || (dst_len && !dst)) return BLSBN254_E_ARG;
  if (n == 0) return 0;
  HIPCHK(c, hipSetDevice(c->device));
  int rc = resolve_pending(c, !allow_async);
  if (rc) return rc;
  const size_t cap = (allow_async && n <= c->chunk) ? async_capacity(c, n, dst_len) : 0;
  if (c->pend_count && (cap == 0 || c->pend_count == 4)) { rc = resolve_pending(c, true); if (rc) return rc; }
  uint32_t dl; rc = stage_dst(c, dst, dst_len, &dl);
  if (rc) return rc;
  if (cap) return verify_chunk_async(c, d_pks, d_msgs, d_off, d_sigs, n, cap, dl, dst, dst_len, d_bitmap);
  return for_chunks(c, n, [&](size_t lo, size_t m) {
    return verify_chunk_dev(c, d_pks + 128 * lo, d_msgs, d_off + lo, d_sigs + 64 * lo, m, dl, d_bitmap + lo / 8);
  });
}
int blsbn254_verify_batch_dev(blsbn254_ctx* c, const uint8_t* d_pks, const uint8_t* d_msgs, const uint64_t* d_off,
                              const uint8_t* d_sigs, size_t n, const uint8_t* dst, size_t dst_len, uint8_t* d_bitmap) {
  return verify_batch_dev_impl(c, d_pks, d_msgs, d_off, d_sigs, n, dst, dst_len, d_bitmap, true);
}
int blsbn254_internal_verify_batch_dev_sync(blsbn254_ctx* c, const uint8_t* d_pks, const uint8_t* d_msgs, const uint64_t* d_off,
                                            const uint8_t* d_sigs, size_t n, const uint8_t* dst, size_t dst_len, uint8_t* d_bitmap) {
  return verify_batch_dev_impl(c, d_pks, d_msgs, d_off, d_sigs, n, dst, dst_len, d_bitmap, false);
}
int blsbn254_async_stats(blsbn254_ctx* c, uint64_t out[2]) {
  if (!c || !out) return BLSBN254_E_ARG;
  out[0] = c->stat_async_chunks; out[1] = c->stat_async_reruns;
  return 0;
}
int blsbn254_set_async_verify(blsbn254_ctx* c, int on) {
  if (!c) return BLSBN254_E_ARG;
  ENTER(c);
  c->async_verify = on != 0;
  return 0;
}
int blsbn254_g2_prepare_batch(blsbn254_ctx* c, const uint8_t* pks, size_t u, blsbn254_g2prepared** out) {
  if (!c || !out || (u && !pks)) return BLSBN254_E_ARG;
  *out = nullptr;
  if (u + 1 > PREP_MAX_KEYS) { c->last_error = "more than 65535 keys in one prepared table"; return BLSBN254_E_ARG; }
  ENTER(c);
  struct Owner { blsbn254_g2prepared* p; ~Owner() { delete p; } } own{new blsbn254_g2prepared()};
  blsbn254_g2prepared* p = own.p;
  p->ctx = c; p->u = u;
  const size_t u1 = u + 1;
  HIPCHK(c, p->table.reserve(u1 * PREP_KEY_LIMBS * 4)); HIPCHK(c, p->ok.reserve(u1)); HIPCHK(c, c->in_a.reserve(128 * u1)); HIPCHK(c, p->raw.reserve(u1 * PREP_RAW_LIMBS * 4));
  if (u) HIPCHK(c, hipMemcpyAsync(c->in_a.p, pks, 128 * u, hipMemcpyHostToDevice, c->stream));
  HIPCHK(c, hipMemcpyAsync((uint8_t*)c->in_a.p + 128 * u, NEG_G2_BYTES, 128, hipMemcpyHostToDevice, c->stream));
  TRY(launch_g2_prepare(c, c->stream, (const uint8_t*)c->in_a.p, nullptr, u1, (int32_t*)p->raw.p, (uint8_t*)p->ok.p, nullptr));
  TRY(launch(c, c->stream, "g2_expand", grid_lanes(u1 * (size_t)BN_NEG_G2_LINES), k_g2_expand, (const int32_t*)p->raw.p, (uint32_t)u1, (int32_t*)p->table.p, (const uint32_t*)nullptr));
  hipError_t es = hipStreamSynchronize(c->stream);
  if (es != hipSuccess) { (void)hipDeviceSynchronize(); }
  HIPCHK(c, es);
  own.p = nullptr;
  *out = p;
  return 0;
}
void blsbn254_g2prepared_destroy(blsbn254_g2prepared* p) {
  if (!p) return;
  (void)hipSetDevice(p->ctx->device);
  (void)hipStreamSynchronize(p->ctx->stream);
  delete p;
}
size_t blsbn254_g2prepared_count(const blsbn254_g2prepared* p) { return p ? p->u : 0; }
int blsbn254_g2prepared_valid(blsbn254_ctx* c, const blsbn254_g2prepared* p, uint8_t* ok_bitmap) {
  if (!c || !p || p->ctx != c || (p->u && !ok_bitmap)) return BLSBN254_E_ARG;
  if (!p->u) return 0;
  ENTER(c);
  HIPCHK(c, c->bitmap.reserve((p->u + 7) / 8 + 8));
  TRY(launch(c, c->stream, "pack_bitmap", grid_lanes(p->u), k_pack_bitmap, (const uint8_t*)p->ok.p, p->u, (uint8_t*)c->bitmap.p));
  return download(c, ok_bitmap, c->bitmap.p, (p->u + 7) / 8);
}
int blsbn254_verify_batch_prepared(blsbn254_ctx* c, const blsbn254_g2prepared* keys, const uint32_t* key_idx, const uint8_t* msgs, const uint64_t* off,
                                   const uint8_t* sigs, size_t n, const uint8_t* dst, size_t dst_len, uint8_t* bm) {
  if (!c || !keys || keys->ctx != c || !off || (n && (!key_idx || !sigs || !bm)) || (dst_len && !dst)) return BLSBN254_E_ARG;
  if (n == 0) return 0;
  ENTER(c);
  uint32_t dl; int rc = stage_dst(c, dst, dst_len, &dl);
  if (rc) return rc;
  rc = stage_msgs(c, msgs, off, n);
  if (rc) return rc;
  const size_t nb = (n + 7) / 8;
  HIPCHK(c, c->bitmap.reserve(nb + 8));
  TRY(upload(c, c->in_b, sigs, 64 * n));
  TRY(upload(c, c->kd_kid, key_idx, 4 * n));
  TRY(for_chunks(c, n, [&](size_t lo, size_t m) {
    return verify_prepared_dev(c, (const int32_t*)keys->table.p, (const uint8_t*)keys->ok.p, keys->u, (const uint32_t*)c->kd_kid.p + lo, false,
                               (const uint8_t*)c->in_c.p, (const uint64_t*)c->in_off.p + lo, (const uint8_t*)c->in_b.p + 64 * lo, m, dl, (uint8_t*)c->bitmap.p + lo / 8, false);
  }));
  return download(c, bm, c->bitmap.p, nb);
}
int blsbn254_multi_miller_loop_prepared(blsbn254_ctx* c, const blsbn254_g2prepared* keys, const uint32_t* key_idx, const uint8_t* g1, size_t n,
                                        uint8_t ml_out[384]) {
  if (!c || !keys || keys->ctx != c || !ml_out || (n && (!key_idx || !g1))) return BLSBN254_E_ARG;
  if (n == 0) { std::memset(ml_out, 0, 384); ml_out[31] = 1; return 0; }
  CHECK_LANES(c, n);
  ENTER(c);
  const size_t n_lanes = (n + 1) / 2;
  HIPCHK(c, c->h_ws.reserve(n * 18 * 4)); HIPCHK(c, c->f_ws.reserve(n_lanes * 108 * 4));
  HIPCHK(c, c->status.reserve(n)); HIPCHK(c, c->flags.reserve(n)); HIPCHK(c, c->kd_hist.reserve(4 * (keys->u + 1))); HIPCHK(c, c->out.reserve(384));
  TRY(upload(c, c->in_a, g1, 64 * n));
  TRY(upload(c, c->kd_kid, key_idx, 4 * n));
  TRY(check_key_indices(c, (const uint32_t*)c->kd_kid.p, n, keys->u, (uint32_t*)c->kd_hist.p, "pair", false));
  int bad;
  TRY(launch(c, c->stream, "g1_to_ws", grid_lanes(n), k_g1_to_ws_batch, (const uint8_t*)c->in_a.p, n, (int32_t*)c->h_ws.p, (uint8_t*)c->status.p));
  int rc = first_bad(c, (const uint8_t*)c->status.p, n, 1, 1, &bad);
  if (rc) return rc;
  if (bad >= 0) return BLSBN254_ERR_G1;
  const bool wide = c->wide_fe && n <= c->wide_fe_max;
  const size_t f_cnt = wide ? n : n_lanes;
  if (wide) {
    HIPCHK(c, c->f_ws.reserve(n * 108 * 4));
    TRY(launch(c, c->stream, "miller_wide_1p", grid_wide(n), k_miller_wide_1p, (const int32_t*)c->h_ws.p, n, (const uint32_t*)c->kd_kid.p, (const int32_t*)keys->raw.p,
               (const uint8_t*)keys->ok.p, n, (int32_t*)c->f_ws.p, n, (uint8_t*)c->flags.p, (const uint8_t*)c->status.p));
  } else {
    TRY(launch(c, c->stream, "miller_hpk2p", grid_lanes(n_lanes), k_miller_hpk2p, (const int32_t*)c->h_ws.p, n, (const uint32_t*)c->kd_kid.p, (const int32_t*)keys->raw.p,
               (const uint8_t*)keys->ok.p, n, (int32_t*)c->f_ws.p, n_lanes, (uint8_t*)c->flags.p, (const uint8_t*)c->status.p));
  }
  rc = first_bad(c, (const uint8_t*)c->flags.p, n, 1, 1, &bad);
  if (rc) return rc;
  if (bad >= 0) return BLSBN254_ERR_G2;
  int32_t* res; size_t rs;
  rc = fp12_tree(c, (int32_t*)c->f_ws.p, f_cnt, f_cnt, &res, &rs);
  if (rc) return rc;
  TRY(launch(c, c->stream, "fp12_to_bytes", grid_lanes(1), k_fp12_to_bytes, (const int32_t*)res, (size_t)1, rs, (uint8_t*)c->out.p));
  return download(c, ml_out, c->out.p, 384);
}
int blsbn254_aggregate_verify_prepared(blsbn254_ctx* c, const blsbn254_g2prepared* keys, const uint32_t* key_idx, const uint8_t* msgs, const uint64_t* off,
                                       size_t n, const uint8_t agg_sig[64], const uint8_t* dst, size_t dst_len, int* valid) {
  if (!c || !keys || keys->ctx != c || !valid || !agg_sig || !off || (n && !key_idx) || (dst_len && !dst)) return BLSBN254_E_ARG;
  *valid = 0;
  if (n == 0) return 0;
  const size_t np = n + 1, n_lanes = (np + 1) / 2;
// ... 64 lines not shown
```

### bls-bn254_amd/csrc/k_keyprep.hip

```cpp
#define BN_WANT_LINE_TABLE
#define BN_LINE_TABLE_QUAL static __device__ const
#include "lane_ops.h"
#include "kernels.h"
using namespace bn;

namespace {
__device__ inline uint32_t load_u32(const uint8_t* p) { return (uint32_t)p[0] | ((uint32_t)p[1] << 8) | ((uint32_t)p[2] << 16) | ((uint32_t)p[3] << 24); }
__device__ inline uint32_t key_hash(const uint8_t* pk, uint32_t seed) {
  uint32_t h = seed ^ 0x9e3779b9u;
  for (int k = 0; k < 32; ++k) { h ^= load_u32(pk + 4 * k); h *= 0x01000193u; h = (h << 13) | (h >> 19); }
  h ^= h >> 16; h *= 0x85ebca6bu; h ^= h >> 13; h *= 0xc2b2ae35u; h ^= h >> 16;
  return h;
}
__device__ inline bool key_equal(const uint8_t* a, const uint8_t* b) {
  uint32_t d = 0;
  for (int k = 0; k < 32; ++k) d |= load_u32(a + 4 * k) ^ load_u32(b + 4 * k);
  return d == 0;
}
}

__global__ void k_kd_insert(const uint8_t* pks, uint32_t n, uint32_t* slots, uint32_t mask, uint32_t seed, uint32_t* rep) {
  uint32_t i = blockIdx.x * blockDim.x + threadIdx.x;
  if (i >= n) return;
  const uint8_t* mine = pks + 128 * (size_t)i;
  uint32_t s = key_hash(mine, seed) & mask;
  for (;;) {
    uint32_t old = __atomic_load_n(&slots[s], __ATOMIC_RELAXED);
    if (old == 0xffffffffu) old = atomicCAS(&slots[s], 0xffffffffu, i);
    if (old == 0xffffffffu) { rep[i] = i; return; }
    if (key_equal(mine, pks + 128 * (size_t)old)) { rep[i] = old; return; }
    s = (s + 1) & mask;
  }
}
__global__ void k_kd_assign(const uint32_t* rep, uint32_t n, uint32_t* kid, uint32_t* counter, uint32_t* keys) {
  uint32_t i = blockIdx.x * blockDim.x + threadIdx.x;
  if (i >= n || rep[i] != i) return;
  uint32_t id = atomicAdd(counter, 1u);
  kid[i] = id; keys[id] = i;
}
__global__ void __launch_bounds__(256) k_kd_propagate(const uint32_t* rep, uint32_t n, uint32_t u, uint32_t* kid, uint32_t* hist) {
  __shared__ uint32_t lh[8192];
  const uint32_t i = blockIdx.x * blockDim.x + threadIdx.x;
  const bool use_lds = hist != nullptr && u <= 8192u;
  if (use_lds) {
    for (uint32_t k = threadIdx.x; k < u; k += blockDim.x) lh[k] = 0;
    __syncthreads();
  }
  if (i < n) {
    const uint32_t id0 = kid[rep[i]], id = id0 < u ? id0 : 0u;
    kid[i] = id;
    if (use_lds) atomicAdd(&lh[id], 1u);
    else if (hist) atomicAdd(&hist[id], 1u);
  }
  if (use_lds) {
    __syncthreads();
    for (uint32_t k = threadIdx.x; k < u; k += blockDim.x) { uint32_t v = lh[k]; if (v) atomicAdd(&hist[k], v); }
  }
}
__global__ void k_kd_hist(const uint32_t* kid, uint32_t n, uint32_t u, uint32_t* hist, int* bad) {
  uint32_t i = blockIdx.x * blockDim.x + threadIdx.x;
  if (i >= n) return;
  if (kid[i] >= u) { atomicMin(bad, (int)(i > 0x7ffffffeu ? 0x7ffffffeu : i)); return; }
  atomicAdd(&hist[kid[i]], 1u);
}
__global__ void __launch_bounds__(1024) k_scan_excl(const uint32_t* hist, uint32_t u, uint32_t* cursor) {
  __shared__ uint32_t part[1024];
  const uint32_t t = threadIdx.x, per = (u + 1023) / 1024, lo = t * per, hi = (lo + per < u) ? lo + per : u;
  uint32_t s = 0;
  for (uint32_t k = lo; k < hi; ++k) s += hist[k];
  part[t] = s;
  __syncthreads();
  for (uint32_t d = 1; d < 1024; d <<= 1) {
    uint32_t v = t >= d ? part[t - d] : 0;
    __syncthreads();
    part[t] += v;
    __syncthreads();
  }
  uint32_t run = t ? part[t - 1] : 0;
  for (uint32_t k = lo; k < hi; ++k) { cursor[k] = run; run += hist[k]; }
}
__global__ void __launch_bounds__(256) k_kd_scatter(const uint32_t* kid, uint32_t n, uint32_t u, uint32_t* cursor, uint32_t* perm) {
  __shared__ uint32_t cnt[8192];
  const uint32_t i = blockIdx.x * blockDim.x + threadIdx.x;
  const bool live = i < n && kid[i] < u;
  if (u > 8192u) {
    if (live) perm[atomicAdd(&cursor[kid[i]], 1u)] = i;
    return;
  }
  for (uint32_t k = threadIdx.x; k < u; k += blockDim.x) cnt[k] = 0;
  __syncthreads();
  const uint32_t k = live ? kid[i] : 0;
  uint32_t rank = 0;
  if (live) rank = atomicAdd(&cnt[k], 1u);
  __syncthreads();
  for (uint32_t j = threadIdx.x; j < u; j += blockDim.x) { const uint32_t v = cnt[j]; if (v) cnt[j] = atomicAdd(&cursor[j], v); }
  __syncthreads();
  if (live) perm[cnt[k] + rank] = i;
}
BN_KERNEL k_g2_prepare(const uint8_t* pks, const uint32_t* keys, uint32_t u, int32_t* table, uint8_t* key_ok, const uint32_t* d_u) {
  const uint32_t nb = (u + 255u) / 256u;
  const bool check_role = blockIdx.x >= nb;
  const uint32_t k = (check_role ? blockIdx.x - nb : blockIdx.x) * blockDim.x + threadIdx.x;
  if (k >= u || (d_u && k >= *d_u)) return;
  const uint8_t* b = pks + 128 * (size_t)(keys ? keys[k] : k);
  bool okd;
  G2A q = g2_decode(b, okd);
  const bool curve_ok = okd & !q.inf & g2_on_curve(q);
  if (check_role) {
    key_ok[k] = (curve_ok & g2_torsion_free(q)) ? 1 : 0;
  } else {
    q.x = fp2_select(curve_ok, q.x, fp2_const(bnc::G2_GEN_X)); q.y = fp2_select(curve_ok, q.y, fp2_const(bnc::G2_GEN_Y)); q.inf = false;
    g2_prepare_lines(q, Ws{table, 1, k * (uint32_t)(BN_NEG_G2_LINES * 54 * 4), true});
  }
}
BN_KERNEL k_g2_expand(const int32_t* raw, uint32_t u, int32_t* expanded, const uint32_t* d_u) {
  __shared__ int32_t stage[256 * 54];
  const uint32_t e0 = blockIdx.x * blockDim.x, e = e0 + threadIdx.x;
  uint32_t total = u * (uint32_t)BN_NEG_G2_LINES;
  if (d_u && *d_u * (uint32_t)BN_NEG_G2_LINES < total) total = *d_u * (uint32_t)BN_NEG_G2_LINES;
  if (e0 >= total) return;
  const uint32_t here = total - e0 < 256u ? total - e0 : 256u;
  for (uint32_t x = threadIdx.x; x < here * 54u; x += 256u) stage[x] = raw[(size_t)e0 * 54u + x];
  __syncthreads();
  const bool live = threadIdx.x < here;
  const uint32_t t = e % (uint32_t)BN_NEG_G2_LINES;
  const Line a = line_from_table(BN_NEG_G2_LINE_TABLE[t]);
  const Line b = line_load_limbs(Ws{stage, 1, (live ? threadIdx.x : 0u) * (uint32_t)(54 * 4), false});
  __syncthreads();
  BN_UNROLL for (int j = 0; j < 9; ++j) {
    const Fp2 p = j == 0 ? fp2_mul(a.c0, b.c0) : j == 1 ? fp2_mul_xi(fp2_mul(a.c2, b.c2)) : j == 2 ? fp2_mul(a.c1, b.c1) : j == 3 ? fp2_mul(a.c1, b.c2)
                : j == 4 ? fp2_mul(a.c2, b.c1) : j == 5 ? fp2_mul(a.c0, b.c1) : j == 6 ? fp2_mul(a.c1, b.c0) : j == 7 ? fp2_mul(a.c0, b.c2) : fp2_mul(a.c2, b.c0);
    fp2_store_limbs_lazy(Ws{stage, 1, threadIdx.x * (uint32_t)(18 * 4), false}, p);
    __syncthreads();
    for (uint32_t x = threadIdx.x; x < here * 18u; x += 256u) {
      const uint32_t lane = x / 18u, limb = x - 18u * lane;
      expanded[((size_t)e0 + lane) * 162u + 18u * (uint32_t)j + limb] = stage[x];
    }
    __syncthreads();
  }
}
__global__ void k_prep_unsort(const uint8_t* is_one, const uint8_t* flags, const uint32_t* perm, uint32_t n, uint8_t* valid) {
  uint32_t s = blockIdx.x * blockDim.x + threadIdx.x;
  if (s >= n) return;
  valid[perm[s]] = (is_one[s] != 0 && flags[s] != 0) ? 1 : 0;
}
__global__ void __launch_bounds__(256) k_pack_bitmap(const uint8_t* valid, size_t n, uint8_t* bitmap) {
  size_t i = (size_t)blockIdx.x * blockDim.x + threadIdx.x;
  write_ballot(bitmap, n, i, i < n && valid[i] != 0);
}

__global__ void k_kd_decide(const uint32_t* cnt, uint32_t n, uint32_t cap, int small, uint32_t* res) {
  if (blockIdx.x != 0 || threadIdx.x != 0) return;
  const uint32_t u = *cnt;
  res[0] = u;
  res[1] = (u <= cap && (small || 2u * u <= n)) ? 1u : 0u;
}
```

### bls-bn254_amd/csrc/k_miller_prep.hip

```cpp
#include "lane_ops.h"
#include "kernels.h"
using namespace bn;

BN_KERNEL k_miller_prepared(const uint32_t* perm, const uint32_t* kid, const uint8_t* sigs, const int32_t* h_ws, size_t h_stride,
                            const int32_t* table, const uint8_t* key_ok, size_t n, int32_t* f_ws, uint8_t* flags) {
  __shared__ int32_t inv_lds[81 * 256];
  const uint32_t s = blockIdx.x * blockDim.x + threadIdx.x;
  if (s >= n) return;
  const uint32_t i = perm[s], k = kid[i];
  bool oks;
  G1A sig = g1_decode(sigs + 64 * (size_t)i, oks);
  const bool sig_ok = oks & !sig.inf & g1_on_curve(sig);
  G1A gp; gp.x = fp_one(); gp.y = fp_norm(fp_add(fp_one(), fp_one()));
  const Ws inv = {inv_lds, 256, threadIdx.x * 4u, false};
  const Ws hw = {const_cast<int32_t*>(h_ws), h_stride, i * 4u, true};
  const Fp xs = fp_norm(fp_select(sig_ok, sig.x, gp.x)), ys = fp_norm(fp_select(sig_ok, sig.y, gp.y));
  const Fp X = fp_load_mem(hw), Y = fp_load_mem(ws_at(hw, 9)), Z = fp_load_mem(ws_at(hw, 18));
  fp_store_mem(inv, X); fp_store_mem(ws_at(inv, 9), Y); fp_store_mem(ws_at(inv, 18), Z);
  fp_store_mem(ws_at(inv, 27), fp_mul(xs, X)); fp_store_mem(ws_at(inv, 36), fp_mul(ys, Y)); fp_store_mem(ws_at(inv, 45), fp_mul(xs, Z));
  fp_store_mem(ws_at(inv, 54), fp_mul(ys, Z)); fp_store_mem(ws_at(inv, 63), fp_mul(ys, X)); fp_store_mem(ws_at(inv, 72), fp_mul(xs, Y));
  BN_MEM_FENCE;
  const Ws kt = {const_cast<int32_t*>(table), 1, k * (uint32_t)(BN_NEG_G2_LINES * 162 * 4), true};
#ifdef BN_MILLER_UNIFORM_KEY
  const uint32_t k0 = __builtin_amdgcn_readfirstlane(k);
  Fp12 f;
  if (__builtin_amdgcn_ballot_w64(k != k0) == 0)
    f = miller_loop_prepared_uniform(inv, table + (size_t)k0 * (BN_NEG_G2_LINES * 162));
  else
    f = miller_loop_prepared(inv, kt);
  fp12_store_limbs(Ws{f_ws, n, s * 4u, true}, f);
#else
  fp12_store_limbs(Ws{f_ws, n, s * 4u, true}, miller_loop_prepared(inv, kt));
#endif
  flags[s] = (sig_ok && key_ok[k] != 0) ? 1 : 0;
}
```

### bls-bn254_amd/csrc/kernels.h

```cpp
#pragma once
#include <hip/hip_runtime.h>
#include <stddef.h>
#include <stdint.h>

#ifndef BN_WAVES_PER_SIMD
#define BN_WAVES_PER_SIMD 1
#endif
#define BN_KERNEL __global__ void __launch_bounds__(256, BN_WAVES_PER_SIMD)

#if defined(__HIPCC__)
__device__ inline void write_ballot(uint8_t* bitmap, size_t n, size_t i, bool bit) {
  unsigned long long m = __ballot(bit);
  unsigned lane = threadIdx.x & 63;
  size_t base = (i - lane) >> 3;
  size_t nbytes = (n + 7) >> 3;
  if (lane < 8 && base + lane < nbytes) bitmap[base + lane] = (uint8_t)(m >> (8 * lane));
}
#endif

BN_KERNEL k_hash_to_g1(const uint8_t* msgs, const uint64_t* off, size_t n, const uint8_t* dst, uint32_t dst_len,
                       int32_t* h_ws, size_t h_stride, uint8_t* out_bytes, int mode);
BN_KERNEL k_hash_to_g2(const uint8_t* msgs, const uint64_t* off, size_t n, const uint8_t* dst, uint32_t dst_len,
                       uint8_t* out_bytes, int ro);
BN_KERNEL k_g1_check(const uint8_t* g1, size_t n, uint8_t* bitmap);
// ... 7 lines not shown
                         int32_t* f_ws, size_t f_stride, uint8_t* flags, const uint8_t* skip);
BN_KERNEL k_g1_to_ws_batch(const uint8_t* g1, size_t n, int32_t* h_ws, uint8_t* status);
BN_KERNEL k_g1_to_ws(const uint8_t* g1, int32_t* h_ws, size_t slot, size_t stride, uint8_t* ok);
BN_KERNEL k_miller_verify(const uint8_t* pks, const uint8_t* sigs, const int32_t* h_ws, size_t n, int32_t* f_ws, uint8_t* flags);
BN_KERNEL k_fe_easy(const int32_t* in, int32_t* out, size_t n, size_t stride);
BN_KERNEL k_fe_easy_head(const int32_t* in, size_t n, size_t stride, int32_t* head, int32_t* nu);
BN_KERNEL k_fe_inv4(int32_t* nu, size_t n, size_t stride);
BN_KERNEL k_fe_easy_tail(const int32_t* in, int32_t* out, size_t n, size_t stride, const int32_t* head, const int32_t* nu);
BN_KERNEL k_fe_expx(const int32_t* in, int32_t* out, int32_t* slots, size_t n, size_t stride);
BN_KERNEL k_fe_expx_h1(const int32_t* in, int32_t* slots, size_t n, size_t stride, int32_t* a_out, int32_t* b_out);
BN_KERNEL k_fe_expx_h2(const int32_t* in, int32_t* slots, size_t n, size_t stride, int32_t* b_in, int32_t* c_out, int32_t* b2_out, int32_t* d2_out);
BN_KERNEL k_fe_h3(const int32_t* t, const int32_t* a, const int32_t* c, const int32_t* b2, const int32_t* x0, int32_t* tmp, size_t n, size_t stride,
                  const uint8_t* flags, const uint8_t* sub_ok, uint8_t* bitmap, uint8_t* gt_bytes, int* is_one, int mode);
__global__ void __launch_bounds__(128) k_miller_wide_prepared(const uint32_t* perm, const uint32_t* kid, const uint8_t* sigs, const int32_t* h_ws, size_t h_stride,
                                                             const int32_t* table, const uint8_t* key_ok, size_t n, int32_t* f_ws, uint8_t* flags);
__global__ void __launch_bounds__(128) k_miller_wide_1p(const int32_t* h_ws, size_t h_stride, const uint32_t* kid, const int32_t* table, const uint8_t* key_ok, size_t n,
                                                       int32_t* f_ws, size_t f_stride, uint8_t* flags, const uint8_t* skip);
__global__ void __launch_bounds__(128) k_miller_wide_1(const uint8_t* g1, const uint8_t* g2, size_t n, int32_t* f_ws, size_t f_stride, uint8_t* status);
__global__ void __launch_bounds__(128) k_fe_hard_wide(const int32_t* t_ws, size_t n, size_t stride, const uint8_t* flags, const uint8_t* sub_ok,
                                                     uint8_t* one, uint8_t* gt_bytes, int* is_one, int mode);
BN_KERNEL k_fp12_from_bytes(const uint8_t* in, size_t n, int32_t* f_ws, size_t f_stride, uint8_t* status);
BN_KERNEL k_fp12_to_bytes(const int32_t* f_ws, size_t n, size_t stride, uint8_t* out);
BN_KERNEL k_fp12_mul_pairs(const int32_t* in, size_t n_in, size_t in_stride, int32_t* out, size_t out_stride);
BN_KERNEL k_g1_load(const uint8_t* g1, size_t n, int32_t* ws, uint8_t* status);
BN_KERNEL k_g1_add_pairs(const int32_t* in, size_t n_in, size_t in_stride, int32_t* out, size_t out_stride);
BN_KERNEL k_g1_to_bytes(const int32_t* ws, size_t stride, uint8_t* out);
BN_KERNEL k_sign(const uint8_t* sks, const uint8_t* msgs, const uint64_t* off, size_t n, const uint8_t* dst, uint32_t dst_len,
                 uint8_t* sigs, uint8_t* status);
BN_KERNEL k_sk_to_pk(const uint8_t* sks, size_t n, uint8_t* pks, uint8_t* status);
BN_KERNEL k_g1_mul(const uint8_t* g1, const uint8_t* scalars, size_t n, uint8_t* out, uint8_t* status);
BN_KERNEL k_g2_mul(const uint8_t* g2, const uint8_t* scalars, size_t n, uint8_t* out, uint8_t* status);
BN_KERNEL k_g2_load(const uint8_t* g2, size_t n, int32_t* ws, uint8_t* ok);
BN_KERNEL k_g2_seg_sum(const int32_t* in_ws, size_t in_stride, const uint8_t* ok_in, const uint32_t* chunk_start, const uint32_t* chunk_len, size_t m,
                       int32_t* out_ws, size_t out_stride, uint8_t* ok_out);
BN_KERNEL k_pair_ok(const uint8_t* g1, const uint8_t* g2, size_t n, uint8_t* ok);
BN_KERNEL k_fp12_seg_prod(const int32_t* in_ws, size_t in_stride, const uint8_t* ok_in, const uint32_t* chunk_start, const uint32_t* chunk_len,
                          size_t m, int32_t* out_ws, size_t out_stride, uint8_t* ok_out, int carry);
BN_KERNEL k_g2p_to_bytes(const int32_t* ws, size_t stride, const uint8_t* ok, size_t m, uint8_t* out, int poison);
BN_KERNEL k_keygen(const uint8_t* ikm, size_t ikm_len, size_t n, const uint8_t* key_info, size_t key_info_len,
                   uint8_t* sks, uint8_t* status);
BN_KERNEL k_hash_to_scalar(const uint8_t* msgs, const uint64_t* off, size_t n, const uint8_t* dst, uint32_t dst_len, uint8_t* out);
BN_KERNEL k_iota_off(uint64_t* off, size_t n, uint64_t step);
BN_KERNEL k_g1_codec(const uint8_t* in, size_t n, uint8_t* out, uint8_t* status, int mode);
BN_KERNEL k_g2_codec(const uint8_t* in, size_t n, uint8_t* out, uint8_t* status, int mode);
BN_KERNEL k_rlc_prep(const uint8_t* pks, const uint8_t* sigs, const int32_t* h_ws, const uint8_t* sub_ok, const uint8_t* seed,
                     size_t n, size_t n_pad, int32_t* a_ws, int32_t* b_ws, uint8_t* elig);
BN_KERNEL k_fp12_mask_one(int32_t* f_ws, size_t stride, const uint8_t* elig, size_t n_pad);
BN_KERNEL k_fp12_mul_elem(int32_t* a, size_t sa, const int32_t* b, size_t sb, size_t m);
BN_KERNEL k_g1p_to_bytes(const int32_t* ws, size_t stride, size_t m, uint8_t* out);
BN_KERNEL k_rlc_gather(const uint32_t* idx, size_t m, const uint8_t* pks, const uint8_t* sigs, const int32_t* h_ws, size_t n,
                       const uint8_t* sub_ok, uint8_t* c_pks, uint8_t* c_sigs, int32_t* c_h, uint8_t* c_sub);
BN_KERNEL k_rlc2_prep(const uint32_t* perm, const uint8_t* pks, const uint8_t* sigs, const int32_t* h_ws, size_t n, const uint8_t* seed,
                      int32_t* a_ws, int32_t* b_ws, uint8_t* sig_ok);
__global__ void k_rlc2_chunk_counts(const uint32_t* hist, uint32_t u, uint32_t G, uint32_t* cnt);
__global__ void k_rlc2_mark(const uint32_t* perm, const uint32_t* kid, const uint32_t* hist, const uint32_t* run_end, const uint32_t* chunk_base,
                            uint32_t n, uint32_t G, uint32_t* tuple_chunk, uint32_t* chunk_kid, uint32_t* chunk_start, uint32_t* chunk_len);
BN_KERNEL k_rlc2_sum(const int32_t* a_ws, const int32_t* b_ws, size_t n, const uint8_t* sig_ok, const uint32_t* chunk_start, const uint32_t* chunk_len,
                     size_t m, int32_t* sa_ws, int32_t* sb_ws, uint32_t* elig_out);
__global__ void k_rlc2_key_elig(const uint32_t* chunk_kid, const uint32_t* chunk_elig, uint32_t m, uint32_t* key_elig);
BN_KERNEL k_rlc2_virtual(const int32_t* sa_ws, const int32_t* sb_ws, size_t stride, const uint32_t* elig, const uint32_t* list, size_t cnt,
                         uint8_t* c_sig, int32_t* c_h, uint8_t* c_state);
__global__ void k_rlc2_keys_pass(const uint8_t* key_ok, const uint8_t* state, const uint8_t* isone, uint32_t u, uint8_t* key_pass, int* all_pass);
__global__ void __launch_bounds__(256) k_rlc2_chunk_need(const uint32_t* chunk_kid, const uint8_t* key_pass, uint32_t m, uint8_t* need, uint32_t* block_cnt);
__global__ void k_rlc2_chunk_pass(const uint32_t* list, const uint8_t* state, const uint8_t* isone, const uint8_t* flags, uint32_t cnt, uint8_t* chunk_pass);
__global__ void k_rlc2_valid_fast(const uint32_t* perm, const uint32_t* kid, const uint8_t* sig_ok, const uint8_t* key_ok, uint32_t n, uint8_t* valid);
__global__ void k_iota_u32(uint32_t* out, uint32_t n);
__global__ void __launch_bounds__(256) k_rlc2_resolve(const uint32_t* perm, const uint32_t* kid, const uint32_t* tuple_chunk, const uint8_t* sig_ok,
                                                      const uint8_t* key_ok, const uint8_t* chunk_pass, uint32_t n, uint8_t* valid, uint8_t* need, uint32_t* block_cnt);
__global__ void __launch_bounds__(256) k_rlc2_compact(const uint8_t* need, const uint32_t* perm, uint32_t n, const uint32_t* block_base, uint32_t* list);
BN_KERNEL k_g1_seg_sum(const int32_t* in_ws, size_t in_stride, const uint32_t* perm, const uint32_t* chunk_start, const uint32_t* chunk_len, size_t m,
                       int32_t* out_ws, size_t out_stride);
BN_KERNEL k_g1p_to_h_affine(const int32_t* in_ws, size_t in_stride, size_t u, int32_t* h_ws, size_t h_stride, uint8_t* status);
BN_KERNEL k_field_op(int op, const uint8_t* a, const uint8_t* b, size_t n, uint8_t* out, uint8_t* status);
BN_KERNEL k_gt_pow(const uint8_t* gt, const uint8_t* scalars, size_t n, uint8_t* out, uint8_t* status);
BN_KERNEL k_fr_decode(const uint8_t* ids, size_t t, int32_t* x_ws, uint8_t* status);
__global__ void k_kd_insert(const uint8_t* pks, uint32_t n, uint32_t* slots, uint32_t mask, uint32_t seed, uint32_t* rep);
__global__ void k_kd_assign(const uint32_t* rep, uint32_t n, uint32_t* kid, uint32_t* counter, uint32_t* keys);
__global__ void __launch_bounds__(256) k_kd_propagate(const uint32_t* rep, uint32_t n, uint32_t u, uint32_t* kid, uint32_t* hist);
__global__ void k_kd_hist(const uint32_t* kid, uint32_t n, uint32_t u, uint32_t* hist, int* bad);
__global__ void __launch_bounds__(1024) k_scan_excl(const uint32_t* hist, uint32_t u, uint32_t* cursor);
__global__ void __launch_bounds__(256) k_kd_scatter(const uint32_t* kid, uint32_t n, uint32_t u, uint32_t* cursor, uint32_t* perm);
BN_KERNEL k_g2_prepare(const uint8_t* pks, const uint32_t* keys, uint32_t u, int32_t* table, uint8_t* key_ok, const uint32_t* d_u);
BN_KERNEL k_g2_prepare_quad(const uint8_t* pks, const uint32_t* keys, uint32_t u, int32_t* table, uint8_t* key_ok, const uint32_t* d_u);
BN_KERNEL k_g2_expand(const int32_t* raw, uint32_t u, int32_t* expanded, const uint32_t* d_u);
__global__ void k_kd_decide(const uint32_t* cnt, uint32_t n, uint32_t cap, int small, uint32_t* res);
__global__ void k_prep_unsort(const uint8_t* is_one, const uint8_t* flags, const uint32_t* perm, uint32_t n, uint8_t* valid);
__global__ void __launch_bounds__(256) k_pack_bitmap(const uint8_t* valid, size_t n, uint8_t* bitmap);
BN_KERNEL k_miller_prepared(const uint32_t* perm, const uint32_t* kid, const uint8_t* sigs, const int32_t* h_ws, size_t h_stride,
                            const int32_t* table, const uint8_t* key_ok, size_t n, int32_t* f_ws, uint8_t* flags);
BN_KERNEL k_miller_tri_prepared(const uint32_t* perm, const uint32_t* kid, const uint8_t* sigs, const int32_t* h_ws, size_t h_stride,
                                const int32_t* table, const uint8_t* key_ok, size_t n, int32_t* f_ws, uint8_t* flags);
BN_KERNEL k_miller_tri_1(const uint8_t* g1, const uint8_t* g2, size_t n, int32_t* f_ws, size_t f_stride, uint8_t* status);
BN_KERNEL k_miller_tri_1p(const int32_t* h_ws, size_t h_stride, const uint32_t* kid, const int32_t* table, const uint8_t* key_ok, size_t n,
                          int32_t* f_ws, size_t f_stride, uint8_t* flags, const uint8_t* skip);
BN_KERNEL k_fe_tri_hard(const int32_t* t_ws, size_t n, size_t stride, int32_t* vals, const uint8_t* flags, const uint8_t* sub_ok,
                        uint8_t* one, uint8_t* gt_bytes, int* is_one, int mode);
BN_KERNEL k_lagrange_partial(const int32_t* x_ws, size_t t, size_t J, int32_t* pnum, int32_t* pden, uint8_t* dup);
BN_KERNEL k_lagrange_finish(const int32_t* pnum, const int32_t* pden, size_t t, size_t S, uint8_t* scalars, uint32_t* glv_ws);
BN_KERNEL k_msm_window(const uint8_t* g1, const uint32_t* glv_ws, size_t t, int32_t* part, uint8_t* status);
__global__ void __launch_bounds__(64) k_msm_finish(const int32_t* part, size_t n_chunks, uint8_t* out);
BN_KERNEL k_msm_fold(const int32_t* in, size_t n_in, int32_t* out);
BN_KERNEL k_lagrange_seg(const int32_t* x_ws, const uint8_t* id_ok, size_t m, uint32_t lo, const uint32_t* goff, uint32_t ng, uint32_t t_big,
                         uint8_t* scalars, uint32_t* glv_ws, uint32_t* gid, uint32_t* gstat);
BN_KERNEL k_g1_smul_glv(const uint8_t* g1, const uint32_t* glv_ws, const uint32_t* gid, size_t m, int32_t* out_ws, uint32_t* gstat);
__global__ void __launch_bounds__(256) k_th_finish(const uint32_t* gstat, size_t n_groups, uint8_t* out, uint8_t* status);
__global__ void __launch_bounds__(256) k_valu_peak(uint32_t* out, uint32_t seed, int iters, int kind, uint64_t* stamps);
__global__ void k_status_reduce(const uint8_t* status, size_t n, uint8_t want_mask, uint8_t want_val, int* first_bad);
__global__ void k_and_reduce(const uint8_t* flags, const uint8_t* sub_ok, size_t n, int* all_ok);
```

### bls-bn254_amd/csrc/pairing.h

```cpp
#pragma once
#include "curve.h"

namespace bn {

struct G2J { Fp2 x, y, z; };
struct Line { Fp2 c0, c1, c2; };

BN_FUNC Line doubling_step(G2J& r) {
  BN_CTX;
  Fp2 tmp0 = fp2_sqr(r.x);
  Fp2 tmp1 = fp2_sqr(r.y);
  Fp2 tmp2 = fp2_sqr(tmp1);
  Fp2 s3 = fp2_sqr(fp2_norm(fp2_add(tmp1, r.x)));
  Fp2 tmp3 = f_lc3<2, -2, -2>(s3, tmp0, tmp2);
  Fp2 tmp4 = f_lc2<3, 0>(tmp0, tmp0);
  Fp2 tmp6 = fp2_norm(fp2_add(r.x, tmp4));
  Fp2 tmp5 = fp2_sqr(tmp4);
  Fp2 zsq = fp2_sqr(r.z);
  Fp2 nx = f_lc2<1, -2>(tmp5, tmp3);
  Fp2 nz = fp2_norm(fp2_sub(fp2_sub(fp2_sqr(fp2_norm(fp2_add(r.z, r.y))), tmp1), zsq));
  Fp2 ny = f_lc2<1, -8>(fp2_mul(fp2_sub(tmp3, nx), tmp4), tmp2);
  Line l;
  l.c1 = f_lc2<-2, 0>(fp2_mul(tmp4, zsq), zsq);
  Fp2 s6 = fp2_sub(fp2_sub(fp2_sqr(tmp6), tmp0), tmp5);
// ... 264 lines not shown
  g2j_store(pk, T);
  BN_MEM_FENCE;
  Line lb;
  if (KIND == 0) lb = doubling_step(Tb);
  else { Fp2 qx, qy; q_of(1, qx, qy); lb = addition_step(Tb, qx, qy); }
  lb = line_mask(live_b, lb);
  T = g2j_load(pk);
  BN_MEM_FENCE;
  g2j_store(pk, Tb);
  BN_MEM_FENCE;
  la = line_load(lp);
  Fp hax = fp_load_mem(hh), hay = fp_load_mem(ws_at(hh, 9)), hbx = fp_load_mem(ws_at(hh, 18)), hby = fp_load_mem(ws_at(hh, 27));
  return ell2(f_in, la, hax, hay, lb, hbx, hby);
}
BN_FUNC Fp12 miller_loop_2var_ws(const Ws& hh, const Ws& qw, const Ws& park, const Ws& lpark, bool live_a, bool live_b) {
  Fp12 f = fp12_one();
  G2J T = {fp2_load_mem(qw), fp2_load_mem(ws_at(qw, 18)), fp2_one()};
  g2j_store(park, G2J{fp2_load_mem(ws_at(qw, 36)), fp2_load_mem(ws_at(qw, 54)), fp2_one()});
  BN_MEM_FENCE;
  for (int j = bnc::ATE_NAF_LEN - 2; j >= 0; --j) {
    f = fp12_sqr(f);
    f = miller2_step<0>(f, T, park, lpark, hh, qw, false, live_a, live_b);
    int d = ate_naf_digit(j);
    if (d != 0) f = miller2_step<1>(f, T, park, lpark, hh, qw, d < 0, live_a, live_b);
  }
  f = miller2_step<2>(f, T, park, lpark, hh, qw, false, live_a, live_b);
  f = miller2_step<3>(f, T, park, lpark, hh, qw, false, live_a, live_b);
  return f;
}

BN_FUNC Fp12 cyclotomic_exp_x(const Fp12& f) {
  BN_CTX;
  Fp12 r = f;
  for (int i = 61; i >= 0; --i) {
    r = fp12_cyclotomic_sqr(r);
    if ((bnc::BN_X >> i) & 1) r = fp12_mul(r, f);
  }
  return r;
}
BN_FUNC Fp12 cyclotomic_exp_x_chain(const Fp12& f, const Ws& slots, const Ws* park = nullptr) {
  const ChainOp prog[BN_X_CHAIN_LEN] = BN_X_CHAIN;
  fp12_store_mem(slots, f);
  BN_MEM_FENCE;
  Fp12 r = f;
  for (int k = 0; k < BN_X_CHAIN_LEN; ++k) {
    const ChainOp op = prog[k];
    if (op.load >= 0) r = fp12_load_mem(ws_at(slots, 108 * op.load));
    for (int q = 0; q < op.sq; ++q) r = fp12_cyclotomic_sqr(r);
    if (op.mul >= 0) r = fp12_mul_mem(r, ws_at(slots, 108 * op.mul), park);
    if (op.store >= 0) fp12_store_mem(ws_at(slots, 108 * op.store), r);
    if (op.cstore >= 0) { fp6_store_mem(ws_at(slots, 108 * op.cstore), r.c0); fp6_store_mem(ws_at(slots, 108 * op.cstore + 54), fp6_norm(fp6_neg(r.c1))); }
    if (op.store >= 0 || op.cstore >= 0) BN_MEM_FENCE;
  }
  return r;
}
BN_FUNC Fp12 fe_easy(const Fp12& f) {
  Fp12 t = fp12_mul(fp12_conj(f), fp12_inv(f));
  return fp12_mul(fp12_frob<2>(t), t);
}
struct FeEasyHead { Fp2 c0, c1, c2, nrm; Fp nu; };
BN_FUNC FeEasyHead fe_easy_head(const Fp12& a) {
  BN_CTX;
  Fp6 s0 = fp6_sqr(a.c0), s1 = fp6_sqr(a.c1);
  Fp6 d = {fp2_sub_mul_xi(s0.c0, s1.c2), fp2_norm(fp2_sub(s0.c1, s1.c0)), fp2_norm(fp2_sub(s0.c2, s1.c1))};
  Fp2 q0 = fp2_sqr(d.c0), q1 = fp2_sqr(d.c1), q2 = fp2_sqr(d.c2);
  Fp2 m01 = fp2_mul(d.c0, d.c1), m02 = fp2_mul(d.c0, d.c2), m12 = fp2_mul(d.c1, d.c2);
  FeEasyHead h;
  h.c0 = fp2_sub_mul_xi(q0, m12);
  h.c1 = fp2_norm(fp2_sub(fp2_mul_xi(q2), m01));
  h.c2 = fp2_norm(fp2_sub(q1, m02));
  Fp2 u = fp2_add(fp2_mul(d.c2, h.c1), fp2_mul(d.c1, h.c2));
  h.nrm = fp2_add_mul_xi(fp2_mul(d.c0, h.c0), u);
  h.nu = fp_dot2(h.nrm.c0, h.nrm.c0, h.nrm.c1, h.nrm.c1);
  return h;
}
BN_FUNC Fp12 fe_easy_tail(const Fp12& a, const FeEasyHead& h, const Fp& nu_inv) {
  BN_CTX;
  Fp2 ti = {fp_mul(h.nrm.c0, nu_inv), fp_mul(fp_neg(h.nrm.c1), nu_inv)};
  Fp6 t6 = {fp2_mul(h.c0, ti), fp2_mul(h.c1, ti), fp2_mul(h.c2, ti)};
  Fp12 inv = {fp6_mul(a.c0, t6), fp6_norm(fp6_neg(fp6_mul(a.c1, t6)))};
  Fp12 t = fp12_mul(fp12_conj(a), inv);
  return fp12_mul(fp12_frob<2>(t), t);
}
BN_FUNC void fp_inv4(Fp x[4]) {
  BN_CTX;
  bool z[4];
  Fp v[4], pre[4];
  for (int i = 0; i < 4; ++i) { z[i] = fp_is_zero(x[i]); v[i] = fp_select(z[i], fp_one(), fp_norm(x[i])); }
  pre[0] = v[0];
  for (int i = 1; i < 4; ++i) pre[i] = fp_mul(pre[i - 1], v[i]);
  Fp inv = fp_inv(pre[3]);
  for (int i = 3; i >= 1; --i) {
    Fp r = fp_mul(inv, pre[i - 1]);
    inv = fp_mul(inv, v[i]);
    x[i] = fp_select(z[i], fp_zero(), r);
  }
  x[0] = fp_select(z[0], fp_zero(), inv);
}
BN_FUNC void fe_h1(const Fp12& x0, Fp12& a, Fp12& b) {
  a = fp12_cyclotomic_sqr(fp12_conj(x0));
  Fp12 a2 = fp12_cyclotomic_sqr(a);
  b = fp12_mul(a, a2);
}
BN_FUNC void fe_h2(const Fp12& x0, const Fp12& b, Fp12& c, Fp12& b2, Fp12& d2) {
  c = fp12_conj(x0);
  b2 = fp12_mul(c, fp12_conj(b));
  d2 = fp12_cyclotomic_sqr(c);
}
BN_FUNC Fp12 fe_h3(const Fp12& t, const Fp12& a, const Fp12& c, const Fp12& b2, const Fp12& x0) {
  Fp12 e = fp12_mul(b2, x0);
  Fp12 d = fp12_mul(a, e);
  Fp12 l0 = fp12_mul(t, fp12_mul(c, e));
  Fp12 r = fp12_mul(l0, fp12_frob<1>(d));
  r = fp12_mul(r, fp12_frob<2>(e));
  Fp12 l3 = fp12_mul(fp12_conj(t), d);
  return fp12_mul(r, fp12_frob<3>(l3));
}
BN_FUNC Fp12 final_exponentiation(const Fp12& f) {
  Fp12 t = fe_easy(f), a, b, c, b2, d2;
  fe_h1(cyclotomic_exp_x(t), a, b);
  fe_h2(cyclotomic_exp_x(b), b, c, b2, d2);
  return fe_h3(t, a, c, b2, cyclotomic_exp_x(d2));
}

BN_INL void fp2_to_be(uint8_t* out, const Fp2& c) { fp_to_be(out, c.c0); fp_to_be(out + 32, c.c1); }
BN_FUNC void fp12_to_be(uint8_t* out, const Fp12& a) {
  BN_CTX;
  fp2_to_be(out, a.c0.c0); fp2_to_be(out + 64, a.c0.c1); fp2_to_be(out + 128, a.c0.c2);
  fp2_to_be(out + 192, a.c1.c0); fp2_to_be(out + 256, a.c1.c1); fp2_to_be(out + 320, a.c1.c2);
}
BN_INL Fp2 fp2_from_be(const uint8_t* in, bool& ok) {
  bool o0, o1;
  Fp2 c = {fp_from_be(in, o0), fp_from_be(in + 32, o1)};
  ok &= o0 & o1;
  return c;
}
BN_FUNC Fp12 fp12_from_be(const uint8_t* in, bool& ok) {
  BN_CTX;
  ok = true;
  Fp12 a;
  a.c0.c0 = fp2_from_be(in, ok); a.c0.c1 = fp2_from_be(in + 64, ok); a.c0.c2 = fp2_from_be(in + 128, ok);
  a.c1.c0 = fp2_from_be(in + 192, ok); a.c1.c1 = fp2_from_be(in + 256, ok); a.c1.c2 = fp2_from_be(in + 320, ok);
  return a;
}
BN_INL void fp2_store_limbs(int32_t* out, size_t stride, const Fp2& c) {
  Fp c0 = fp_canon(c.c0), c1 = fp_canon(c.c1);
  BN_UNROLL for (int k = 0; k < NL; ++k) { out[(size_t)k * stride] = c0.l[k]; out[(size_t)(9 + k) * stride] = c1.l[k]; }
}
BN_INL void fp2_store_limbs(const Ws& w, const Fp2& c) {
  Fp c0 = fp_canon(c.c0), c1 = fp_canon(c.c1);
  BN_UNROLL for (int k = 0; k < NL; ++k) { ws_store(w, k, c0.l[k]); ws_store(w, 9 + k, c1.l[k]); }
}
BN_FUNC void fp12_store_limbs(const Ws& w, const Fp12& a) {
  BN_CTX;
  fp2_store_limbs(w, a.c0.c0); fp2_store_limbs(ws_at(w, 18), a.c0.c1); fp2_store_limbs(ws_at(w, 36), a.c0.c2);
  fp2_store_limbs(ws_at(w, 54), a.c1.c0); fp2_store_limbs(ws_at(w, 72), a.c1.c1); fp2_store_limbs(ws_at(w, 90), a.c1.c2);
}
BN_INL Fp2 fp2_load_limbs(const Ws& w) {
  Fp2 c;
  BN_UNROLL for (int k = 0; k < NL; ++k) { c.c0.l[k] = ws_load(w, k); c.c1.l[k] = ws_load(w, 9 + k); }
  BN_TRK(set_trk(c.c0, 0, 1, 0, 0.006, 1); set_trk(c.c1, 0, 1, 0, 0.006, 1);)
  return c;
}
BN_FUNC Fp12 fp12_load_limbs(const Ws& w) {
  BN_CTX;
  return {{fp2_load_limbs(w), fp2_load_limbs(ws_at(w, 18)), fp2_load_limbs(ws_at(w, 36))},
          {fp2_load_limbs(ws_at(w, 54)), fp2_load_limbs(ws_at(w, 72)), fp2_load_limbs(ws_at(w, 90))}};
}
BN_FUNC void fp12_store_limbs(int32_t* out, size_t stride, const Fp12& a) {
  BN_CTX;
  fp2_store_limbs(out, stride, a.c0.c0); fp2_store_limbs(out + 18 * stride, stride, a.c0.c1);
  fp2_store_limbs(out + 36 * stride, stride, a.c0.c2); fp2_store_limbs(out + 54 * stride, stride, a.c1.c0);
  fp2_store_limbs(out + 72 * stride, stride, a.c1.c1); fp2_store_limbs(out + 90 * stride, stride, a.c1.c2);
}
BN_INL Fp2 fp2_load_limbs(const int32_t* in, size_t stride) {
  Fp2 c;
  BN_UNROLL for (int k = 0; k < NL; ++k) { c.c0.l[k] = in[(size_t)k * stride]; c.c1.l[k] = in[(size_t)(9 + k) * stride]; }
  BN_TRK(set_trk(c.c0, 0, 1, 0, 0.006, 1); set_trk(c.c1, 0, 1, 0, 0.006, 1);)
  return c;
}
// ... 47 lines not shown
  for (int j = bnc::ATE_NAF_LEN - 2; j >= 0; --j) {
    line_store_limbs(ws_at(out, 54 * (size_t)ti++), doubling_step(T));
    int d = ate_naf_digit(j);
    if (d != 0) line_store_limbs(ws_at(out, 54 * (size_t)ti++), addition_step(T, q.x, d > 0 ? q.y : nqy));
  }
  Fp2 g2 = fp2_const(bnc::GAMMA1[1]), g3 = fp2_const(bnc::GAMMA1[2]);
  Fp2 q1x = fp2_mul(fp2_norm(fp2_conj(q.x)), g2), q1y = fp2_mul(fp2_norm(fp2_conj(q.y)), g3);
  Fp2 q2x = fp2_mul(fp2_norm(fp2_conj(q1x)), g2);
  Fp2 q2y = fp2_norm(fp2_neg(fp2_mul(fp2_norm(fp2_conj(q1y)), g3)));
  line_store_limbs(ws_at(out, 54 * (size_t)ti++), addition_step(T, q1x, q1y));
  line_store_limbs(ws_at(out, 54 * (size_t)ti++), addition_step(T, q2x, q2y));
}
BN_INL void fp_store_limbs_lazy(const Ws& w, const Fp& c) {
  BN_TRK(if (c.lo < -4e-6 || c.hi > 1.0 + 4e-6 || c.tlo < -0.02 || c.thi > 0.02 || c.vb > 1.2) check_fail("pair table entry outside its declared range", c.vb);)
  BN_UNROLL for (int k = 0; k < NL; ++k) ws_store(w, k, c.l[k]);
}
BN_INL Fp fp_load_limbs_lazy(const Ws& w) {
  Fp c;
  BN_UNROLL for (int k = 0; k < NL; ++k) c.l[k] = ws_load(w, k);
  BN_TRK(set_trk(c, -4e-6, 1.0 + 4e-6, -0.02, 0.02, 1.2); check_actual(c, "pair table entry");)
  return c;
}
BN_INL void fp2_store_limbs_lazy(const Ws& w, const Fp2& c) { fp_store_limbs_lazy(w, c.c0); fp_store_limbs_lazy(ws_at(w, 9), c.c1); }
BN_INL Fp2 fp2_load_limbs_lazy(const Ws& w) {
  Fp2 c;
  BN_UNROLL for (int k = 0; k < NL; ++k) { c.c0.l[k] = ws_load(w, k); c.c1.l[k] = ws_load(w, 9 + k); }
  BN_TRK(set_trk(c.c0, -4e-6, 1.0 + 4e-6, -0.02, 0.02, 1.2); set_trk(c.c1, -4e-6, 1.0 + 4e-6, -0.02, 0.02, 1.2);
         check_actual(c.c0, "pair table entry"); check_actual(c.c1, "pair table entry");)
  return c;
}
BN_FUNC void line_pair_expand(const Line& a, const Line& b, const Ws& out) {
  BN_CTX;
  fp2_store_limbs_lazy(out, fp2_mul(a.c0, b.c0));
  fp2_store_limbs_lazy(ws_at(out, 18), fp2_mul_xi(fp2_mul(a.c2, b.c2)));
  fp2_store_limbs_lazy(ws_at(out, 36), fp2_mul(a.c1, b.c1));
  fp2_store_limbs_lazy(ws_at(out, 54), fp2_mul(a.c1, b.c2));
  fp2_store_limbs_lazy(ws_at(out, 72), fp2_mul(a.c2, b.c1));
  fp2_store_limbs_lazy(ws_at(out, 90), fp2_mul(a.c0, b.c1));
  fp2_store_limbs_lazy(ws_at(out, 108), fp2_mul(a.c1, b.c0));
  fp2_store_limbs_lazy(ws_at(out, 126), fp2_mul(a.c0, b.c2));
  fp2_store_limbs_lazy(ws_at(out, 144), fp2_mul(a.c2, b.c0));
}
BN_INL Fp2 fp2_dot_fp(const Fp2& t, const Fp& s, const Fp2& u, const Fp& r) {
  return {fp_dot2(t.c0, s, u.c0, r), fp_dot2(t.c1, s, u.c1, r)};
}
BN_FUNC Fp12 ell_pair_expanded(const Fp12& f, const Ws& e, const Ws& cw) {
  BN_CTX;
  Fp X = fp_load_mem(cw), Y = fp_load_mem(ws_at(cw, 9)), Z = fp_load_mem(ws_at(cw, 18));
  Fp xsX = fp_load_mem(ws_at(cw, 27)), ysY = fp_load_mem(ws_at(cw, 36)), xsZ = fp_load_mem(ws_at(cw, 45));
  Fp ysZ = fp_load_mem(ws_at(cw, 54)), ysX = fp_load_mem(ws_at(cw, 63)), xsY = fp_load_mem(ws_at(cw, 72));
  Fp6 l0 = {fp2_dot_fp(fp2_load_limbs_lazy(e), ysY, fp2_load_limbs_lazy(ws_at(e, 18)), Z),
            fp2_mul_fp(fp2_load_limbs_lazy(ws_at(e, 36)), xsX),
            fp2_dot_fp(fp2_load_limbs_lazy(ws_at(e, 54)), xsZ, fp2_load_limbs_lazy(ws_at(e, 72)), X)};
  Fp2 l10 = fp2_dot_fp(fp2_load_limbs_lazy(ws_at(e, 90)), ysX, fp2_load_limbs_lazy(ws_at(e, 108)), xsY);
  Fp2 l11 = fp2_dot_fp(fp2_load_limbs_lazy(ws_at(e, 126)), ysZ, fp2_load_limbs_lazy(ws_at(e, 144)), Y);
  Fp6 v0 = fp6_mul(f.c0, l0);
  Fp6 v1 = fp6_mul_by_01(f.c1, l10, l11);
  Fp6 dl = {fp2_norm(fp2_sub(l10, l0.c0)), fp2_norm(fp2_sub(l11, l0.c1)), fp2_norm(fp2_neg(l0.c2))};
  Fp6 w = fp6_mul(fp6_norm(fp6_sub(f.c0, f.c1)), dl);
  return {fp6_add_mul_v(v0, v1), fp6_norm(fp6_add(fp6_add(w, v0), v1))};
}
BN_FUNC Fp12 miller_loop_prepared(const Ws& inv, const Ws& ktab_in) {
  Fp12 f = fp12_one();
  Ws p = inv, kt = ktab_in;
  int ti = 0;
  for (int j = bnc::ATE_NAF_LEN - 2; j >= 0; --j) {
    f = fp12_sqr(f);
    BN_OPAQUE(kt); BN_OPAQUE(p);
    f = ell_pair_expanded(f, ws_at(kt, 162 * (size_t)ti), p);
    ++ti;
    if (ate_naf_digit(j) != 0) {
      BN_OPAQUE(kt); BN_OPAQUE(p);
      f = ell_pair_expanded(f, ws_at(kt, 162 * (size_t)ti), p);
      ++ti;
    }
  }
  for (int e = 0; e < 2; ++e) {
    BN_OPAQUE(kt); BN_OPAQUE(p);
    f = ell_pair_expanded(f, ws_at(kt, 162 * (size_t)ti), p);
    ++ti;
  }
  return f;
}
#if defined(__HIP_DEVICE_COMPILE__)
typedef const __attribute__((address_space(4))) int32_t* bn_const_i32p;
#else
typedef const int32_t* bn_const_i32p;
#endif
BN_INL Fp2 fp2_load_limbs_const(bn_const_i32p e) {
  Fp2 c;
  BN_UNROLL for (int k = 0; k < NL; ++k) { c.c0.l[k] = e[k]; c.c1.l[k] = e[9 + k]; }
  BN_TRK(set_trk(c.c0, -4e-6, 1.0 + 4e-6, -0.02, 0.02, 1.2); set_trk(c.c1, -4e-6, 1.0 + 4e-6, -0.02, 0.02, 1.2);
         check_actual(c.c0, "pair table entry"); check_actual(c.c1, "pair table entry");)
  return c;
}
BN_FUNC Fp12 ell_pair_expanded_uniform(const Fp12& f, bn_const_i32p e, const Ws& cw) {
  Fp X = fp_load_mem(cw), Y = fp_load_mem(ws_at(cw, 9)), Z = fp_load_mem(ws_at(cw, 18));
  Fp xsX = fp_load_mem(ws_at(cw, 27)), ysY = fp_load_mem(ws_at(cw, 36)), xsZ = fp_load_mem(ws_at(cw, 45));
  Fp ysZ = fp_load_mem(ws_at(cw, 54)), ysX = fp_load_mem(ws_at(cw, 63)), xsY = fp_load_mem(ws_at(cw, 72));
  Fp6 l0 = {fp2_dot_fp(fp2_load_limbs_const(e), ysY, fp2_load_limbs_const(e + 18), Z),
            fp2_mul_fp(fp2_load_limbs_const(e + 36), xsX),
            fp2_dot_fp(fp2_load_limbs_const(e + 54), xsZ, fp2_load_limbs_const(e + 72), X)};
  Fp2 l10 = fp2_dot_fp(fp2_load_limbs_const(e + 90), ysX, fp2_load_limbs_const(e + 108), xsY);
  Fp2 l11 = fp2_dot_fp(fp2_load_limbs_const(e + 126), ysZ, fp2_load_limbs_const(e + 144), Y);
  Fp6 v0 = fp6_mul(f.c0, l0);
  Fp6 v1 = fp6_mul_by_01(f.c1, l10, l11);
  Fp6 dl = {fp2_norm(fp2_sub(l10, l0.c0)), fp2_norm(fp2_sub(l11, l0.c1)), fp2_norm(fp2_neg(l0.c2))};
  Fp6 w = fp6_mul(fp6_norm(fp6_sub(f.c0, f.c1)), dl);
  return {fp6_add_mul_v(v0, v1), fp6_norm(fp6_add(fp6_add(w, v0), v1))};
}
BN_FUNC Fp12 miller_loop_prepared_uniform(const Ws& inv, const int32_t* ktab_uniform) {
  Fp12 f = fp12_one();
  Ws p = inv;
  bn_const_i32p kt = (bn_const_i32p)ktab_uniform;
  int ti = 0;
  for (int j = bnc::ATE_NAF_LEN - 2; j >= 0; --j) {
    f = fp12_sqr(f);
    BN_OPAQUE(p);
    f = ell_pair_expanded_uniform(f, kt + 162 * ti, p);
    ++ti;
    if (ate_naf_digit(j) != 0) {
      BN_OPAQUE(p);
      f = ell_pair_expanded_uniform(f, kt + 162 * ti, p);
      ++ti;
    }
  }
  for (int e = 0; e < 2; ++e) {
    BN_OPAQUE(p);
    f = ell_pair_expanded_uniform(f, kt + 162 * ti, p);
    ++ti;
  }
  return f;
}

BN_FUNC Fp12 miller_loop_1prepared(const Ws& hh_in, const Ws& ta_in) {
  Fp12 f = fp12_one();
  Ws hh = hh_in, ta = ta_in;
  int ti = 0;
  for (int j = bnc::ATE_NAF_LEN - 2; j >= 0; --j) {
    f = fp12_sqr(f);
    BN_OPAQUE(ta); BN_OPAQUE(hh);
    f = ell(f, line_load_limbs(ws_at(ta, 54 * (size_t)ti)), fp_load_mem(hh), fp_load_mem(ws_at(hh, 9)));
    ++ti;
    if (ate_naf_digit(j) != 0) {
      BN_OPAQUE(ta); BN_OPAQUE(hh);
      f = ell(f, line_load_limbs(ws_at(ta, 54 * (size_t)ti)), fp_load_mem(hh), fp_load_mem(ws_at(hh, 9)));
      ++ti;
    }
  }
  for (int e = 0; e < 2; ++e) {
    BN_OPAQUE(ta); BN_OPAQUE(hh);
    f = ell(f, line_load_limbs(ws_at(ta, 54 * (size_t)ti)), fp_load_mem(hh), fp_load_mem(ws_at(hh, 9)));
    ++ti;
  }
  return f;
}

BN_FUNC Fp12 ell2_from_tables(const Fp12& f, const Ws& ta_in, const Ws& tb_in, int ti, const Ws& hh_in, bool live_a, bool live_b) {
  Ws hh = hh_in, ta = ta_in, tb = tb_in;
  BN_OPAQUE(ta); BN_OPAQUE(tb); BN_OPAQUE(hh);
  Line la = line_mask(live_a, line_load_limbs(ws_at(ta, 54 * (size_t)ti)));
  Line lb = line_mask(live_b, line_load_limbs(ws_at(tb, 54 * (size_t)ti)));
  Fp hax = fp_load_mem(hh), hay = fp_load_mem(ws_at(hh, 9)), hbx = fp_load_mem(ws_at(hh, 18)), hby = fp_load_mem(ws_at(hh, 27));
  return ell2(f, la, hax, hay, lb, hbx, hby);
}
BN_FUNC Fp12 miller_loop_2prepared(const Ws& hh, const Ws& ta, const Ws& tb, bool live_a, bool live_b) {
  Fp12 f = fp12_one();
  int ti = 0;
  for (int j = bnc::ATE_NAF_LEN - 2; j >= 0; --j) {
    f = fp12_sqr(f);
    f = ell2_from_tables(f, ta, tb, ti++, hh, live_a, live_b);
    if (ate_naf_digit(j) != 0) f = ell2_from_tables(f, ta, tb, ti++, hh, live_a, live_b);
  }
  f = ell2_from_tables(f, ta, tb, ti++, hh, live_a, live_b);
  f = ell2_from_tables(f, ta, tb, ti++, hh, live_a, live_b);
  return f;
}

}
```

Before: 7.243 million verifies/s.

## Normalize pair line tables to unit coefficients with batched Fp2 inversions

Result: faster. 7.322 million verifies/s, median of 6 (+1.1%).

```diff
diff --git a/bls-bn254_amd/csrc/bn254_consts.h b/bls-bn254_amd/csrc/bn254_consts.h
--- a/bls-bn254_amd/csrc/bn254_consts.h
+++ b/bls-bn254_amd/csrc/bn254_consts.h
@@ -145,3 +145,95 @@
  {248938176, 350466153, 134753901, 435380835, 72917553, 156155176, 291307518, 32259336, 1028390, 379779376, 231645262, 229723036, 193965067, 153531491, 375312851, 491839129, 441506130, 1041786, 115764437, 313016821, 369953093, 454752130, 484813132, 417728943, 512613884, 477427683, 2993031, 253811470, 122990100, 443458760, 301470983, 82635724, 51241845, 135246996, 100410326, 735740, 106669830, 500727615, 185253398, 80759155, 174390583, 427362052, 435938546, 75098748, 2455921, 158248225, 274759410, 28245215, 72408984, 11419683, 86345775, 16182697, 81920639, 3124442},
 };
 #endif
+#ifdef BN_WANT_UNIT_LINE_TABLE
+BN_LINE_TABLE_QUAL int32_t BN_NEG_G2_UNIT_LINE_TABLE[88][36] = {
+ {448429663, 213992044, 464726047, 361702903, 163242314, 457193204, 217690972, 204270039, 1976569, 406784824, 320538958, 165772379, 78848451, 530502566, 414448413, 240901472, 292200723, 1231736, 350501726, 119998407, 33598490, 305696541, 62290573, 2029978, 122691778, 359076065, 1817345, 180057908, 282954532, 64370959, 533197261, 323570160, 526703857, 486947605, 273606777, 1376642},
+ {229681845, 476817180, 36789859, 104361835, 340713354, 442174084, 330246424, 33957633, 1838117, 475934161, 241130873, 68115809, 156731198, 163704957, 89875672, 326291953, 288854315, 2391771, 97682960, 502630585, 277857492, 37180399, 111899524, 223768447, 378720672, 88459396, 195593, 11619510, 147401638, 291670075, 449976874, 269008449, 374252245, 84181391, 181385569, 1438560},
+ {90704835, 296154153, 527448317, 483646191, 436468307, 380927981, 403066226, 448664567, 1123329, 102580888, 507269825, 454936762, 176393190, 431462933, 203169500, 240661886, 120001924, 1952679, 223558622, 46422639, 350109364, 121450449, 210233726, 86872857, 511443990, 119786025, 681978, 536493044, 29250511, 101222058, 196316674, 89261311, 257316239, 146849942, 232618346, 920740},
+ {324980528, 110467290, 331914180, 105337506, 271174727, 522683593, 74431607, 296353519, 553, 533168545, 289037008, 329490023, 20909591, 469397491, 409969590, 350890789, 91262698, 443997, 386582316, 421301705, 113170338, 369845066, 120335735, 3538326, 53092454, 175652639, 1238847, 393709293, 146139435, 470127673, 305499751, 214055852, 246172388, 328729575, 526552350, 365510},
+ {122855496, 504174573, 432771186, 92624938, 195073049, 490839836, 222992465, 383721730, 1145704, 251551270, 224247421, 346996764, 221291443, 85360426, 100595607, 475933881, 19805860, 2478840, 375672223, 280390960, 24106509, 26221586, 520810298, 416987392, 297248109, 343869922, 1438833, 149827559, 454258205, 78355568, 146407826, 233256941, 380545412, 106008474, 511143252, 1873457},
+ {305048931, 96027645, 418042098, 97529550, 164224642, 337233024, 276934651, 162396148, 2534077, 182078081, 327155166, 423365946, 391994501, 95931867, 25690822, 193425397, 71454695, 41597, 527960283, 105913182, 328384580, 311973479, 68114651, 45328723, 361839298, 312645862, 768145, 402990343, 357233564, 228692903, 392543353, 226144497, 502397811, 313378317, 93204130, 348565},
+ {276060958, 261353695, 516826928, 497388198, 223232333, 303147650, 292985979, 395211594, 2262403, 312912142, 134482703, 321855093, 214096849, 88671894, 172009631, 124189937, 164543527, 2562458, 139613972, 444067530, 364153961, 150630166, 361014099, 349490664, 218972253, 91136697, 1566342, 315590161, 229953117, 216896671, 316471209, 289320182, 225246378, 26381731, 417826227, 2561646},
+ {393137481, 73462645, 323672554, 184141143, 207479718, 374174546, 302885704, 172409364, 2506082, 188222181, 47739336, 415347409, 418082845, 200547871, 429365341, 994770, 465043703, 2197831, 151753988, 403175369, 104453548, 328109200, 142748054, 78775218, 416222053, 399688185, 2066115, 417149606, 219631341, 234052245, 527563366, 359123307, 117976861, 533332518, 81222930, 1846320},
+ {256389452, 28721752, 480265403, 398764591, 112762564, 404846813, 81008997, 307171288, 2342135, 483998866, 358716487, 405370251, 444185219, 465901664, 535586925, 199542017, 119336408, 1674616, 107140060, 247390343, 528133475, 181915899, 102487246, 271093407, 442052678, 198122903, 2890729, 137467066, 516017507, 516214764, 459337064, 270077982, 78283911, 514910730, 19510905, 2388917},
+ {258624749, 50044621, 352975624, 342206406, 338661056, 240535077, 42568733, 402935909, 1308319, 456666878, 94685999, 395940614, 368224534, 226403877, 46267375, 1711584, 310832645, 2096375, 427052274, 157783080, 450108248, 47094773, 286770847, 91522819, 521590720, 468541321, 488479, 233725301, 334506629, 247975977, 13663129, 484038291, 166459509, 422583095, 470998262, 569719},
+ {27455219, 107822885, 283701321, 263693960, 66809805, 36198456, 432072237, 61087277, 2908267, 313492234, 308981234, 497228424, 244285114, 409227643, 235078502, 63534853, 6280257, 2541545, 338503411, 4325560, 78907252, 468053946, 472505493, 392319776, 384016259, 427840544, 2346469, 53407246, 476408645, 37922279, 359953218, 173390994, 179588377, 455101718, 236835614, 178174},
+ {529582334, 71595404, 370468232, 515992322, 9700544, 218586702, 104172361, 23545478, 1600289, 138018486, 84442182, 451334491, 241420237, 432010869, 512491154, 307374251, 497152381, 2486460, 494922716, 59975625, 209209678, 161335411, 476796993, 493935542, 346846413, 220333888, 914954, 29745140, 296855896, 418188439, 397478355, 74855205, 457843973, 66669388, 272685076, 1794887},
+ {431721494, 28657207, 118831430, 1327191, 415311546, 468176524, 260910812, 535033509, 2979646, 533222676, 117131035, 128766258, 252050966, 13019812, 19993986, 74337255, 237675349, 674052, 241586841, 179457589, 95629767, 38465846, 330817046, 372749331, 240398367, 104391069, 2042095, 146178941, 105277460, 349345807, 252282305, 364158402, 393143744, 43601865, 525998071, 656077},
+ {453621600, 477539462, 443293790, 371214732, 146958256, 82326557, 21991358, 366686961, 1788875, 83328498, 232300841, 237221519, 210246325, 396736120, 432149963, 385431564, 397670152, 1962122, 275959320, 125047198, 345127937, 96452670, 433176076, 62116177, 57792550, 10434664, 1411017, 337193079, 58166493, 466507043, 287546217, 424556700, 512911756, 284374464, 365170996, 1430886},
+ {198321244, 38813305, 142528996, 131800517, 318359093, 127737603, 443841540, 136527418, 2028123, 144531193, 253223926, 244553447, 245110183, 144943042, 479028051, 20466957, 476069070, 1148699, 117134965, 480870439, 392058707, 96709947, 282231690, 509461560, 283584531, 489469389, 694396, 337681481, 485507933, 217081401, 422359202, 79235488, 433850848, 448005290, 147171453, 2248899},
+ {72672586, 467126452, 53922159, 230917586, 172442452, 150524545, 331505849, 525878264, 165308, 451650191, 450879167, 275628792, 12095525, 200540390, 34942034, 344372479, 382857841, 1672061, 113496349, 190232828, 412683721, 91756219, 260022608, 19584075, 106779463, 299418501, 861250, 266098417, 135884281, 248155432, 141537768, 188747334, 303420185, 267861699, 46513426, 1142324},
+ {479021225, 445819160, 535411414, 472534472, 327331794, 21768592, 402944425, 453653177, 2091152, 298936355, 127383149, 306226054, 282446009, 59342910, 11979750, 64795093, 366608389, 202271, 172739890, 353900107, 53211402, 173028570, 516217993, 508594833, 107353712, 414014064, 687205, 112822855, 291551348, 423697980, 106814430, 508474995, 522247900, 504043751, 20301122, 1856735},
+ {210841147, 467973381, 255535447, 413395067, 344086442, 495729993, 489824440, 385361521, 1910561, 211558083, 198199647, 248571937, 226812809, 517975346, 130114225, 347876271, 114487701, 1680937, 197956416, 76222229, 61538456, 246638301, 176180702, 66161930, 16858434, 219902518, 2245192, 5451573, 405007279, 238263757, 472431724, 30837730, 307661953, 191778306, 512781270, 2046613},
+ {160348967, 66731416, 118949499, 404124543, 176104180, 265914449, 513193301, 41024539, 2871228, 70374291, 477439021, 21284991, 13198324, 113125181, 445002265, 347789323, 307018302, 1289913, 134163194, 499468859, 399525242, 327484988, 476117962, 368660873, 396850879, 527348270, 1874754, 255830655, 216605785, 152321056, 347353922, 52386172, 436081306, 81295735, 501427616, 742524},
+ {19042573, 9433895, 367865041, 93393304, 185993900, 112809114, 296714453, 42343515, 1179988, 417029911, 226055676, 510565666, 428155211, 19760433, 194905786, 56058896, 35755278, 1513688, 337584700, 212780396, 535423388, 126872720, 491798932, 19151642, 412921188, 37388820, 2191847, 322654331, 113071611, 18912753, 99129791, 374210877, 157518083, 192915968, 139171944, 2984539},
+ {332352807, 248515943, 9496779, 408860739, 3400102, 516087219, 344414313, 196508336, 1699927, 2752458, 164546269, 297688794, 142885990, 196139200, 100600621, 27422114, 163757494, 3036742, 284371769, 391605895, 469572981, 494680365, 378105682, 92639452, 295237617, 92873586, 1659951, 161061870, 22666638, 102171904, 88222250, 527047975, 529149962, 534010973, 8575468, 1834514},
+ {374830761, 387001357, 519490291, 68582180, 170135940, 224359860, 422234834, 256673476, 1053559, 10647485, 417490461, 477875503, 271427105, 28054153, 26998926, 311420031, 345739000, 2438102, 176305012, 307018633, 318516120, 246242494, 277262917, 254594108, 293719113, 256119627, 2288057, 182385650, 2317651, 139813891, 332359591, 457228669, 401329688, 411009790, 250369723, 2968585},
+ {301492585, 19170905, 459606532, 162872874, 263783935, 328734784, 3758684, 359254378, 757191, 368500873, 333480455, 497765506, 82002219, 466720469, 91664252, 35742679, 183206802, 245785, 360207970, 267462349, 450878390, 292171701, 110458808, 38761816, 115710003, 53136882, 1760148, 399459124, 157193946, 381876443, 366962489, 185634616, 5617901, 353960504, 200603870, 2382891},
+ {478060117, 32624037, 81620611, 469928304, 259266947, 269250567, 454076918, 155203101, 1816827, 332747097, 264717471, 465176432, 175649741, 46933664, 185838952, 427978517, 251765341, 1098782, 233714450, 125378577, 365453948, 140941889, 211832275, 136099284, 409279780, 414356361, 782896, 40745761, 152247619, 142735898, 263863375, 254920144, 352945769, 505390178, 113674395, 989148},
+ {181930859, 83201961, 127510233, 252696138, 180461294, 90871593, 190217380, 24425660, 815703, 483072150, 85601533, 8526488, 325995893, 47670821, 446168363, 81372095, 384518428, 1501446, 137912176, 46518659, 223902486, 421531858, 101659775, 226411506, 117183109, 356845458, 2621752, 169141732, 315095494, 122184983, 375123220, 130188211, 14709619, 88223688, 392598610, 2199886},
+ {502059548, 446016400, 376707506, 519245150, 333200760, 277448784, 200883653, 481155695, 2992446, 520662909, 245010456, 214387782, 73580307, 215744593, 383580053, 18963876, 271729261, 2418963, 240121751, 160342188, 241285616, 445513802, 30730652, 439010368, 98923081, 535745037, 2072691, 146071839, 102092731, 316671695, 388814051, 508286454, 249003433, 334221885, 127176348, 951008},
+ {141875638, 271030836, 302976114, 486325027, 136666985, 55224982, 416867451, 55164896, 1150002, 474846313, 430810980, 441662655, 201706924, 80166015, 196796347, 79646389, 493006970, 1829823, 190759018, 6061452, 388496573, 429076788, 379200368, 304492670, 106512740, 495269716, 1720787, 303702783, 375288637, 49664998, 27005655, 191738700, 394621926, 158554762, 512726521, 1152867},
+ {514824594, 422711543, 314500279, 115432606, 144901888, 259033812, 157602477, 193132118, 2961704, 371694099, 443546998, 70077276, 201763212, 110090942, 471632298, 228621997, 412904355, 263740, 186269922, 186204806, 248534859, 22879117, 131870632, 287200696, 355843418, 357732556, 2535389, 514950795, 261074625, 437418608, 504356639, 128605772, 416427199, 402443857, 419762993, 3092612},
+ {101694058, 405726246, 276508781, 92816892, 75630575, 185414295, 427895310, 424388860, 2131561, 354812314, 37651662, 306528245, 67043786, 379430186, 139619207, 400519735, 396993265, 2928647, 320463528, 502653625, 470536418, 133270926, 126113883, 526689301, 433510660, 414018323, 1630522, 420988486, 27994395, 294423652, 273931569, 299870328, 523719973, 342061324, 461792471, 409755},
+ {479514606, 105261541, 407770610, 225225783, 57990057, 87603969, 243239999, 446194501, 238398, 96288980, 169319362, 455350095, 443426648, 63847693, 491231798, 485019157, 337309680, 308893, 313785761, 339453205, 146109538, 318361100, 197910421, 437703852, 261454799, 195052364, 1878927, 461520707, 23710717, 449086068, 69758335, 305677041, 297883846, 477927574, 410021432, 808770},
+ {533959457, 93587547, 200454771, 170204718, 476037569, 71097352, 46381027, 161953071, 366963, 150973592, 274597753, 215756466, 300846923, 199052501, 350819389, 433924022, 27551928, 2535440, 62401052, 241526370, 157952635, 507888360, 52596485, 369616013, 245459647, 277098108, 395443, 514367534, 51990925, 406385879, 221929847, 301421669, 502827883, 490060562, 505917829, 782125},
+ {471195479, 225124496, 529373447, 105541776, 517689758, 226065104, 221947234, 153958627, 3160067, 215777641, 443148159, 104255998, 90146299, 256473053, 94241030, 425126494, 507392349, 1893320, 407281256, 493517889, 191832566, 358729464, 417921426, 274782476, 396533011, 473818555, 732021, 384814209, 204091896, 26048623, 532939329, 251865914, 400869780, 75905028, 20405913, 641470},
+ {203199274, 431040706, 107257640, 393007512, 141554759, 112132655, 224254200, 534430156, 1331781, 493012638, 16383529, 305893749, 460063737, 532045695, 224688560, 280101002, 301331827, 24903, 180541802, 240424901, 49644240, 387011345, 178336765, 43674111, 296967619, 115729215, 1252059, 158613368, 451854529, 12735848, 433319408, 465293348, 427941369, 483182412, 341697615, 1456708},
+ {318769672, 479494727, 392109832, 150310659, 383144501, 133158253, 3623572, 363512543, 1960697, 409464032, 128991792, 331832729, 434017988, 285307333, 218283790, 347481302, 97254202, 1542891, 106615515, 387629051, 6113128, 306488552, 324193439, 487991075, 229440797, 500802351, 865092, 22709005, 187093682, 134335284, 331962569, 60071739, 280322978, 524929104, 74402201, 54684},
+ {491203125, 291094901, 205319801, 531777691, 418231655, 264160423, 103351298, 248810721, 886620, 388732151, 443702511, 235317471, 50934514, 35208003, 407734541, 495179730, 400558646, 1132794, 108541301, 513547371, 309433080, 440051877, 443991915, 512746369, 426743177, 276474340, 2397376, 129293960, 431615513, 300864458, 377921869, 443131391, 85399640, 109517756, 178883664, 2262141},
+ {299632097, 381358522, 261510797, 408058057, 113992874, 7126420, 535959212, 477469169, 989439, 283033540, 94247420, 447567734, 419502243, 534698337, 105122500, 293406428, 514128556, 384964, 396414461, 444089081, 351264624, 79487698, 194014520, 151992401, 262977609, 321916602, 1948733, 499267028, 409662168, 143032404, 526629228, 312877673, 328894501, 163416407, 147485368, 161712},
+ {300196474, 370191410, 454444212, 412858093, 122667210, 158379892, 312365696, 168579808, 332003, 125063802, 198188807, 92312446, 241201493, 497373912, 57973947, 213087473, 467055768, 1897644, 76405089, 18719411, 479807327, 433545389, 46407967, 422683353, 108293856, 310533588, 791813, 12149282, 161426424, 289108702, 6770673, 364607198, 510339075, 398851793, 430945956, 2274177},
+ {397037674, 465884557, 111980391, 209506516, 500698850, 72328053, 9361882, 51902004, 909329, 244659578, 5104984, 498160246, 233187255, 367930912, 146172262, 35520309, 176484407, 2847770, 372136469, 214403852, 444320650, 424787466, 228963167, 255438884, 472165886, 513529385, 1875144, 411770254, 78285539, 526549696, 108160784, 478172238, 294217911, 48927928, 60354351, 1373719},
+ {454487309, 381041025, 87195584, 236806378, 378250156, 78537762, 272693821, 57339267, 2059226, 399300060, 530883713, 387231354, 416858288, 466186927, 380755602, 274001371, 378050819, 886774, 321429240, 273432758, 309247400, 146629244, 206522693, 459202633, 157998028, 329628673, 630457, 170135520, 216611637, 226655593, 407220304, 118373528, 418087872, 339635442, 58930457, 1786191},
+ {248011148, 178830658, 518604293, 197057318, 525830050, 216131543, 96938059, 160976827, 61165, 416026696, 417496733, 201341410, 248947706, 516722221, 295180859, 423540382, 447492607, 59581, 308389449, 409299199, 306057736, 283925423, 493864223, 516465437, 503657274, 440882326, 2133866, 78136550, 349453479, 410771705, 498238052, 56578136, 471857309, 494958795, 219963894, 1627615},
+ {525019321, 459816534, 62736678, 39891275, 424486557, 88659999, 242959999, 72199683, 1186189, 321145612, 141102, 382516932, 487460707, 192916295, 324096357, 256632037, 241393304, 3057096, 452524712, 412526430, 351459858, 268070837, 243853843, 205751635, 389857687, 12419057, 1510997, 11994115, 391947546, 522235396, 292191261, 260976339, 107407896, 258084644, 79712681, 1219414},
+ {277254596, 502384541, 142434083, 484793654, 244127076, 290576233, 76196729, 89142842, 1121665, 397159545, 108178597, 71297871, 479162329, 15522170, 49381092, 430980287, 286273058, 938233, 498029846, 94328865, 222639978, 124245110, 330588907, 425674775, 517740476, 351399499, 1128228, 78722857, 192160187, 377503711, 400789990, 430693470, 98659122, 214183697, 13358875, 1359579},
+ {44476256, 387305228, 264714671, 519150923, 26151899, 451383280, 291971111, 302208667, 2200716, 248880772, 159469864, 63274873, 363400713, 341976673, 63586871, 487695112, 141245795, 196014, 443850554, 286450735, 394103972, 29817476, 267972653, 23075253, 131087487, 298845126, 2774037, 332298822, 42644499, 160313710, 114764443, 22184280, 383436207, 184211682, 20937700, 266553},
+ {372116265, 216975169, 309412663, 335451320, 188375393, 374903569, 143824305, 241921775, 2892455, 162863329, 452578145, 186357448, 1809119, 218679876, 326981667, 358033227, 493934557, 900314, 3798871, 469877982, 228764451, 497057587, 48779123, 482130449, 90785632, 30406721, 1767141, 427166749, 343350602, 103465349, 471409227, 285626175, 373164555, 206597231, 154718539, 2797383},
+ {73722405, 51323131, 104765621, 17240247, 418949542, 310652729, 282061916, 534806343, 1434477, 374121158, 31669859, 462825128, 247764878, 256398372, 535636883, 206813654, 244067397, 1536023, 165518918, 51414794, 14929808, 380732952, 326911463, 2282628, 243064250, 375840159, 1102276, 186729225, 325369407, 293743365, 525254272, 200485758, 2232573, 192389918, 458151233, 3144814},
+ {393796325, 463607989, 248981238, 100502769, 77389131, 418895731, 193323331, 206221614, 457480, 17773770, 379393184, 83890029, 141558867, 181556362, 211967573, 466388819, 278406562, 932876, 426302370, 516574318, 341061835, 369488374, 305935009, 405503895, 474269190, 350611880, 3111689, 292879344, 72056410, 220090501, 113850763, 178008052, 352969025, 215943096, 434721584, 1682461},
+ {366077403, 297421457, 329682847, 24560132, 135997467, 111135017, 2072679, 257041873, 1251665, 266316113, 520385622, 371048660, 245924984, 236989693, 155356523, 282989621, 341118298, 118762, 237770808, 116695744, 348599298, 349361127, 300143300, 246390722, 93882913, 420822337, 2875194, 527304867, 41255491, 365336876, 355242884, 431542600, 319412981, 193115713, 358255792, 88138},
+ {25922711, 450976785, 77746000, 449296059, 270046015, 69034698, 266282578, 37550917, 36048, 9571146, 46766463, 400848184, 185076852, 81619059, 338162494, 217677108, 487087925, 1144882, 423712248, 224397221, 31056870, 443572270, 57132638, 323446311, 258178385, 354633401, 882432, 210536997, 98093388, 101225085, 267668752, 208317657, 487146195, 385087284, 46951637, 2494133},
+ {425221568, 209525047, 361483601, 360253463, 323085427, 250083203, 521833644, 325060701, 810942, 523902224, 532097703, 337672011, 157043159, 273954476, 311234363, 121671881, 193019399, 1655179, 355720740, 489197713, 266947119, 9100292, 69070221, 425972592, 159024130, 31316341, 1843798, 350115150, 398963733, 112464095, 19825686, 466014321, 426644559, 16232597, 182744836, 2180847},
+ {180387777, 275477693, 375482636, 443994505, 124271056, 305958039, 65310141, 478120370, 2135813, 159582137, 173575330, 475286015, 153137530, 407677323, 33362749, 36482947, 208378755, 2634567, 39625905, 269886096, 175198534, 292415363, 235563421, 254179504, 525020842, 353120498, 1123034, 159054547, 4746767, 146685112, 142398882, 30147116, 104746683, 28390849, 183134358, 1888034},
+ {245551513, 27149476, 394514895, 380696066, 490757925, 185641799, 106191698, 491084832, 2279760, 455900667, 335054615, 50415128, 124168765, 355618028, 145237268, 76899312, 462925928, 2658945, 17301540, 118336049, 336173091, 132207366, 368729152, 139116255, 404286757, 355023114, 666693, 103962659, 147575707, 187732055, 371804078, 524571743, 3429267, 74729380, 281244277, 2952761},
+ {322943208, 133582790, 170243276, 79755267, 413874599, 524429485, 378485803, 202792324, 144529, 475776673, 338346437, 336334223, 290734700, 28897814, 120912824, 530539790, 291588682, 1211958, 159607111, 288401366, 452277839, 237887509, 293234063, 183353321, 128642820, 202097520, 1600060, 261596081, 57038087, 154752136, 45578394, 307429962, 531130344, 194069042, 256059607, 1519339},
+ {223138788, 135904432, 8570659, 261417741, 241220687, 109547050, 505930495, 70407213, 2795188, 446787075, 212011378, 7807059, 320765677, 454324707, 492926870, 519054895, 439428609, 2837968, 458982832, 38588582, 356803110, 348706522, 470762212, 354198172, 158448161, 174279190, 2944473, 513440207, 479076504, 110260565, 279117026, 269506612, 219741577, 534772823, 214994002, 74468},
+ {286032097, 487168653, 20616588, 274538872, 306981884, 103158009, 322504077, 168008659, 3101130, 418391878, 127654626, 98977224, 285649074, 93846228, 205809303, 57234445, 55428675, 2997085, 348987865, 36907017, 515400082, 183816912, 422032594, 187275453, 522642452, 89469212, 3068242, 454300359, 438602100, 164048665, 404073081, 448309103, 255008048, 331759177, 415444383, 1721665},
+ {190853494, 257313468, 314815019, 434432171, 218109693, 249730122, 417831424, 514068323, 2815461, 310405942, 502934048, 160163961, 132158871, 79171454, 34466809, 464632106, 297962863, 336319, 414024135, 369831654, 184533546, 483392964, 473404420, 327324499, 258504010, 489400792, 173920, 498083691, 385596060, 499986710, 108788172, 166034841, 134766899, 397484993, 442847763, 2500294},
+ {478210256, 131261369, 110188062, 63794567, 473870366, 180038996, 472876172, 286559073, 972026, 480376692, 18219710, 372460716, 356873130, 75639920, 114898893, 419515199, 427347242, 2362169, 73112227, 308072160, 193743189, 68997034, 455875790, 56163685, 6552856, 16518950, 294067, 503423261, 523872976, 470619154, 532463801, 431792873, 396634369, 379616857, 204550699, 2071004},
+ {362421709, 149200317, 136964145, 462135286, 396870995, 168854419, 209773846, 20077718, 1674514, 327347586, 473605913, 13764510, 447728830, 36998979, 99040138, 180594788, 280334112, 2206662, 120735663, 463397291, 334118794, 223910742, 57000651, 466130581, 505984677, 379221550, 753359, 397053804, 438624406, 436119724, 405154653, 267942311, 101950600, 118548064, 188037048, 3164726},
+ {172285398, 109055271, 270322932, 329677264, 379009195, 253448943, 88894721, 418065165, 1769389, 439247106, 83039425, 88658421, 261598724, 249309456, 532655361, 76405527, 82416760, 179122, 491946045, 94414005, 330864614, 289784125, 44748717, 426601893, 253467934, 152201951, 969091, 275362870, 501649964, 390402528, 250958787, 30120414, 392007398, 165754127, 352029778, 550518},
+ {176724255, 465619987, 415280083, 522086491, 326365456, 128505254, 440159698, 41617731, 104460, 377276405, 490951683, 99553752, 75698745, 96983192, 478689774, 283237294, 161111081, 312321, 431992288, 375307771, 534145893, 339507651, 277976689, 208467884, 209116933, 347881009, 314719, 203340140, 8653268, 322159003, 423525219, 19235435, 237573762, 432216065, 353469142, 2227032},
+ {257407569, 456196611, 376408222, 153329898, 15764686, 358844689, 393870494, 390952397, 2107892, 425297849, 180944424, 193427108, 302199165, 310013627, 1254557, 64954526, 425462308, 1497785, 233352739, 306651365, 100614650, 242255692, 426367615, 483732449, 504080917, 50763100, 1827018, 256657636, 439496687, 228437038, 38851888, 266251660, 135553808, 23719396, 156835857, 183507},
+ {229134990, 436864263, 61757668, 75705717, 187684007, 184260275, 44119630, 395804436, 938489, 475244643, 496278423, 221653923, 405995418, 419803623, 454859000, 331917674, 174661253, 1522198, 375752330, 26752103, 366902916, 511168423, 509710999, 458737551, 20973411, 73263099, 2583602, 281653786, 453270977, 513671468, 428859738, 193066103, 479514250, 326569373, 424848159, 2194084},
+ {417867528, 307154249, 346293865, 113403279, 213204314, 505199505, 504700610, 116351059, 2864892, 130605578, 211214615, 12689023, 216480525, 53046693, 243444915, 307959206, 231931747, 2445465, 224883674, 510474439, 409826490, 46145133, 124531575, 7357638, 467596558, 427253547, 1804335, 312963892, 390702054, 88837155, 431413781, 445292586, 497927313, 246121621, 504126060, 856889},
+ {476022249, 187203723, 270910645, 70477281, 422100328, 298532239, 528253639, 185454012, 2698596, 178503412, 200478289, 439499030, 87654446, 53327399, 504082583, 108353848, 155651299, 2372927, 435583085, 221997564, 28532353, 276590269, 215355185, 412760024, 529804986, 28300596, 996680, 242030138, 249739074, 149880721, 524455897, 413176529, 293742276, 183620786, 376402189, 2711215},
+ {201727294, 331531564, 500390135, 450256765, 98756460, 221764953, 281825102, 271567338, 2152725, 305061090, 380227747, 94691158, 222810998, 234434489, 85961565, 282382964, 345456259, 1885931, 336979899, 456951009, 170410180, 236363721, 23091894, 213059611, 394352490, 287628596, 2993509, 383243600, 287890787, 49356345, 328847859, 56305503, 260500855, 139210693, 105644878, 766561},
+ {136004075, 276624695, 536558516, 7117260, 123557755, 396869475, 465894936, 425159966, 1955124, 366311266, 255175971, 180527424, 8157465, 46100805, 353900269, 201261584, 209968840, 2648338, 372382052, 311549884, 231250957, 84951038, 73623411, 27309760, 69475405, 206630921, 1787328, 220048558, 217645470, 112431922, 247008717, 71890679, 179706056, 293559331, 190955894, 1110522},
+ {208988979, 50872611, 95031048, 33497221, 467847184, 201905138, 451626618, 69242325, 1790482, 498592141, 395194073, 20437961, 306903658, 296165192, 10531671, 210535325, 92893704, 2912794, 332257897, 104604907, 81832766, 104382173, 10550025, 172622308, 20861983, 47594724, 2768161, 400181074, 303876852, 389260988, 383638692, 4477726, 488415385, 495915846, 473999016, 1576902},
+ {387667046, 92934239, 522280996, 534213887, 400649191, 359559180, 530279801, 110573893, 1287073, 345816551, 6612953, 299903857, 169782758, 150914405, 512972825, 135841910, 532749650, 2003517, 51683515, 42133123, 58204025, 254184896, 235756738, 437873990, 416454456, 426073730, 170153, 221524987, 490730246, 81799523, 52351639, 408537759, 115376664, 252891309, 332475436, 2347136},
+ {316304129, 272484114, 120048366, 196260233, 190191626, 530622047, 416297456, 287200896, 1653371, 98979414, 369596619, 202944699, 241813960, 317397786, 430284769, 101656292, 211587835, 2911039, 42167165, 183521926, 15384605, 227770864, 211544789, 353933218, 220808448, 334232796, 2724544, 86297110, 374821043, 359526750, 118148369, 473794522, 464187082, 51016481, 294159263, 1993200},
+ {71109643, 256266738, 513726793, 241490155, 98596561, 76870420, 382238768, 380058921, 1218559, 436867938, 108110076, 445122226, 60320618, 366998573, 168455440, 264991005, 202288293, 2173483, 274389129, 123663636, 26774191, 388542333, 248458273, 241130224, 170129092, 300197882, 101539, 187065023, 177605858, 378952292, 110035150, 99640911, 438509714, 335916957, 184981543, 782420},
+ {82759794, 512568327, 463362559, 88046097, 456091826, 113509682, 235761268, 250148888, 857289, 59519338, 270251934, 342489113, 183637966, 162648605, 187400172, 526199944, 34017191, 1381694, 406390090, 415747440, 404115556, 458622376, 364384162, 144525925, 83505155, 223814270, 1191985, 162822968, 435339801, 533471386, 518771512, 177583311, 164848667, 362233914, 111375062, 1342610},
+ {10164917, 400275717, 42492026, 353156302, 287676323, 3234127, 272490395, 525637087, 334583, 195378028, 76743135, 156099601, 266974567, 337389689, 52636220, 29001625, 355260333, 1142337, 367253873, 420260211, 227123798, 393178485, 31162269, 150732249, 129449149, 170209817, 2487776, 255580443, 9105295, 241190345, 306094296, 333304990, 291938702, 122952192, 76383138, 210347},
+ {237538436, 33273078, 217382693, 167460287, 161186369, 395080403, 144862560, 496781428, 585936, 392203794, 130759093, 380245245, 168304681, 268632492, 529824551, 238243846, 390199745, 2460598, 75558160, 464706844, 388353047, 497450423, 488193604, 231571090, 309990261, 374515009, 2514866, 531876721, 112821284, 41423982, 520899539, 525539588, 369691349, 337289247, 385006308, 1438399},
+ {205645884, 136781226, 529343114, 211228952, 129672317, 141197636, 439446355, 124837932, 1264724, 254159292, 80925133, 341737679, 318470632, 106679577, 129154473, 108256766, 205480617, 1666338, 353834957, 69077323, 213337300, 492290877, 67200718, 105622947, 24909001, 307523955, 455174, 525339646, 230674536, 525093674, 62955509, 380457256, 72456509, 122690247, 403328401, 1472635},
+ {191242874, 259697009, 131701100, 313493272, 105940500, 509957003, 234652234, 40720197, 1539373, 148981811, 115132757, 335157380, 328992859, 280372242, 425303918, 231223592, 322149631, 1566561, 150179772, 294963792, 103462720, 314639921, 444508976, 531570852, 414448591, 51648943, 2252484, 303932117, 532270752, 200304675, 248778333, 54045825, 348763662, 115005358, 423750983, 1772724},
+ {288020483, 100085008, 56171585, 32202843, 345113955, 166236236, 405933197, 330970368, 1506779, 144685298, 349301957, 289210635, 77603824, 497877758, 303489212, 536735767, 229745895, 530722, 63886992, 170609635, 160241551, 368696661, 512959133, 165381621, 446457902, 175595747, 2267606, 501825299, 521179628, 295361595, 53288379, 313553868, 392701224, 507137257, 149914060, 1941303},
+ {131846732, 483346524, 406071187, 177511683, 457912704, 330643597, 88341079, 392011035, 2447981, 117673425, 311755097, 249785735, 332669034, 200062867, 523124317, 151462326, 110959242, 1584021, 371885622, 377847697, 235468489, 207836487, 121629455, 464349851, 41870786, 253886115, 19688, 228313311, 438254272, 136645296, 137862279, 288735868, 299604177, 390909759, 493344976, 2685889},
+ {243073103, 238313850, 116385907, 32127829, 382226932, 36110236, 333859028, 47605960, 2536049, 238989462, 273319435, 226769104, 319378123, 479939703, 295711156, 474329042, 178653853, 2148404, 17430349, 304071354, 24172513, 188694380, 1005685, 489092914, 357944397, 371158937, 2814366, 171373294, 174545293, 212165901, 8359670, 514960966, 106812470, 212986864, 60644029, 2713561},
+ {281734097, 455207045, 264171497, 217895511, 505071597, 183686395, 79184832, 494585318, 1371369, 282028706, 344548540, 370409498, 98935206, 266026172, 218678867, 29715169, 210537279, 1542485, 315334929, 203354829, 447168329, 530212572, 511887015, 346332456, 514962654, 166672828, 870688, 64947383, 382678871, 137514142, 353283834, 53672393, 253299312, 442877296, 64951052, 1167643},
+ {239208921, 494593324, 502467434, 390559601, 402146209, 287700344, 155302597, 95626061, 1506250, 421975919, 352327808, 122524538, 279985175, 503020484, 268696884, 328440332, 25723857, 3084962, 526107953, 230551632, 86681459, 178205489, 137014843, 132282385, 340480948, 478783188, 1413353, 172075802, 139966475, 294734223, 385833133, 375202288, 295667016, 502860420, 422856945, 2872730},
+ {201152303, 517835612, 247899629, 447912289, 491205426, 398824953, 215538157, 204077989, 1895549, 106879486, 312984764, 206253810, 435805287, 529051969, 180758266, 367576780, 241172146, 1928227, 317439535, 273463829, 370355026, 111567961, 426172439, 456680133, 135894972, 91477910, 617600, 470161914, 152338375, 408457674, 195889650, 450771409, 168005179, 259609779, 157306851, 1872539},
+ {422247527, 423104272, 51395846, 333135870, 524461682, 92577535, 123259256, 77271820, 1921835, 52875247, 367067242, 168807004, 310274298, 421488233, 166212628, 323138785, 227188634, 3018674, 289304669, 238094726, 324018141, 526596698, 333938938, 29284101, 35065579, 75693192, 1069616, 161391692, 287600393, 275037147, 154431979, 186478453, 322744292, 426908506, 498918685, 2860767},
+ {475211833, 24183996, 25861872, 452492947, 73639716, 264941956, 217299445, 303601421, 2725892, 461237194, 363906852, 532764694, 523334646, 218191497, 515900525, 131238276, 250150188, 774562, 174750828, 521247708, 334011646, 210011852, 102281993, 301936926, 256790166, 476584508, 1663933, 353972197, 503695859, 343343185, 507646095, 382537237, 9968477, 101156255, 528477708, 1578507},
+ {19909421, 465146410, 72478593, 2473914, 196597936, 361510930, 93024526, 531954388, 1267227, 62431948, 440296894, 68696285, 260277839, 439851527, 218892828, 530882146, 480104558, 2847768, 458865069, 343719801, 394948310, 317390727, 74006085, 226955259, 338304652, 515277337, 417926, 156758023, 162088444, 81744722, 417804114, 334894365, 208106775, 239758164, 236801114, 1227543},
+ {77466985, 369666109, 65014019, 300453640, 64398167, 130915598, 112662632, 182009950, 106571, 394908027, 360740936, 359739088, 500871179, 473733676, 127521723, 252104200, 90731948, 2527963, 197247261, 444632143, 10047415, 199165622, 210225328, 342562424, 343610147, 523353054, 2772690, 510569964, 192934738, 534192704, 379166422, 82279505, 16731520, 333428483, 242554505, 241916},
+ {149544767, 474380742, 441311651, 74811817, 447034723, 228143528, 382970772, 69850411, 564520, 179434469, 38702910, 284140792, 412607266, 59908946, 292197025, 250545276, 422602647, 1345098, 418238686, 200665219, 282684353, 119013332, 494038972, 49787968, 362589421, 487714786, 3108489, 248989756, 123995103, 387230087, 66503437, 443175296, 423850773, 11099961, 124920566, 2541499},
+ {369619512, 478087019, 518393742, 165065188, 101279908, 189883320, 222721282, 246020878, 537293, 120504604, 418422016, 256070395, 369998072, 146528612, 296076450, 252065852, 43915205, 161830, 361952115, 209624645, 379271966, 490231918, 38264857, 272913325, 457307750, 342396464, 1632310, 337027675, 42653544, 117188270, 81351147, 150353229, 235327242, 312429090, 167532542, 13320},
+ {231735031, 124036273, 130778572, 157183609, 530625971, 418383659, 436899773, 527597689, 576954, 46811389, 112776186, 99675912, 49466462, 464368443, 341944834, 59703566, 130595340, 680709, 375049743, 80957434, 435175338, 442383379, 242022504, 171882547, 271563078, 324841729, 1629218, 224536456, 508951031, 254038678, 289183898, 47799104, 520714581, 527823264, 391241407, 2675190},
+ {458031219, 43761586, 177679545, 401841403, 90395118, 58479252, 162982237, 527329627, 2456854, 340972140, 396883035, 37678903, 164826651, 227934674, 104880318, 290588162, 58664770, 1659467, 104745225, 362519892, 56618554, 54491984, 275956349, 286587448, 48335380, 230375883, 2683039, 125283359, 482151927, 124744663, 167459190, 247881839, 258789012, 29035201, 238438381, 1569012},
+};
+#endif
diff --git a/bls-bn254_amd/csrc/fp29.h b/bls-bn254_amd/csrc/fp29.h
--- a/bls-bn254_amd/csrc/fp29.h
+++ b/bls-bn254_amd/csrc/fp29.h
@@ -459,7 +459,7 @@
   a[NL - 1] = (int32_t)ca; b[NL - 1] = (int32_t)cb;
 }
 constexpr int SG_BATCHES = 21;
-BN_FUNC Fp fp_inv(const Fp& a) {
+BN_FUNC Fp fp_inv_divsteps(const Fp& a, bool& done) {
   const Fp x = fp_from_mont(a);
   int32_t f[NL], g[NL], d[NL], e[NL];
   BN_UNROLL for (int i = 0; i < NL; ++i) { f[i] = bnc::P[i]; g[i] = x.l[i]; d[i] = 0; e[i] = i == 0 ? 1 : 0; }
@@ -472,16 +472,22 @@
   }
   int32_t gnz = 0;
   BN_UNROLL for (int i = 0; i < NL; ++i) gnz |= g[i];
-#if defined(__HIP_DEVICE_COMPILE__)
-  if (__builtin_amdgcn_ballot_w64(gnz != 0) != 0) return fp_inv_pow(a);
-#else
-  if (gnz != 0) return fp_inv_pow(a);
-#endif
+  done = gnz == 0;
   const bool neg = f[NL - 1] < 0;
   Fp di;
   BN_UNROLL for (int i = 0; i < NL; ++i) di.l[i] = neg ? -d[i] : d[i];
   BN_TRK(set_trk(di, -1, 1, -0.14, 0.14, 22);)
   return fp_mul(di, fp_const(bnc::R2));
+}
+BN_FUNC Fp fp_inv(const Fp& a) {
+  bool done;
+  const Fp r = fp_inv_divsteps(a, done);
+#if defined(__HIP_DEVICE_COMPILE__)
+  if (__builtin_amdgcn_ballot_w64(!done) != 0) return fp_inv_pow(a);
+#else
+  if (!done) return fp_inv_pow(a);
+#endif
+  return r;
 }
 BN_FUNC Fp fp_sqrt_cand(const Fp& a, bool& is_sq) {
   Fp y = fp_pow(a, BN_EXP(EXP_PP1_4));
diff --git a/bls-bn254_amd/csrc/host_verify.hip b/bls-bn254_amd/csrc/host_verify.hip
--- a/bls-bn254_amd/csrc/host_verify.hip
+++ b/bls-bn254_amd/csrc/host_verify.hip
@@ -12,7 +12,7 @@
   HIPCHK(c, c->prep_raw.reserve(u * PREP_RAW_LIMBS * 4));
   HIPCHK(c, fork_stream2(c));
   TRY(launch_g2_prepare(c, c->stream2, d_pks, d_keys, u, (int32_t*)c->prep_raw.p, key_ok, d_u));
-  TRY(launch(c, c->stream2, "g2_expand", grid_lanes(u * (size_t)BN_NEG_G2_LINES), k_g2_expand, (const int32_t*)c->prep_raw.p, (uint32_t)u, table, d_u));
+  TRY(launch(c, c->stream2, "g2_expand", grid_lanes(u * (size_t)BN_NEG_G2_LINES), k_g2_expand, (const int32_t*)c->prep_raw.p, (uint32_t)u, table, d_u, key_ok));
   HIPCHK(c, hipEventRecord(c->ev_join, c->stream2));
   return 0;
 }
@@ -216,7 +216,7 @@
   if (u) HIPCHK(c, hipMemcpyAsync(c->in_a.p, pks, 128 * u, hipMemcpyHostToDevice, c->stream));
   HIPCHK(c, hipMemcpyAsync((uint8_t*)c->in_a.p + 128 * u, NEG_G2_BYTES, 128, hipMemcpyHostToDevice, c->stream));
   TRY(launch_g2_prepare(c, c->stream, (const uint8_t*)c->in_a.p, nullptr, u1, (int32_t*)p->raw.p, (uint8_t*)p->ok.p, nullptr));
-  TRY(launch(c, c->stream, "g2_expand", grid_lanes(u1 * (size_t)BN_NEG_G2_LINES), k_g2_expand, (const int32_t*)p->raw.p, (uint32_t)u1, (int32_t*)p->table.p, (const uint32_t*)nullptr));
+  TRY(launch(c, c->stream, "g2_expand", grid_lanes(u1 * (size_t)BN_NEG_G2_LINES), k_g2_expand, (const int32_t*)p->raw.p, (uint32_t)u1, (int32_t*)p->table.p, (const uint32_t*)nullptr, (uint8_t*)p->ok.p));
   hipError_t es = hipStreamSynchronize(c->stream);
   if (es != hipSuccess) { (void)hipDeviceSynchronize(); }
   HIPCHK(c, es);
diff --git a/bls-bn254_amd/csrc/k_keyprep.hip b/bls-bn254_amd/csrc/k_keyprep.hip
--- a/bls-bn254_amd/csrc/k_keyprep.hip
+++ b/bls-bn254_amd/csrc/k_keyprep.hip
@@ -1,4 +1,4 @@
-#define BN_WANT_LINE_TABLE
+#define BN_WANT_UNIT_LINE_TABLE
 #define BN_LINE_TABLE_QUAL static __device__ const
 #include "lane_ops.h"
 #include "kernels.h"
@@ -113,7 +113,7 @@
     g2_prepare_lines(q, Ws{table, 1, k * (uint32_t)(BN_NEG_G2_LINES * 54 * 4), true});
   }
 }
-BN_KERNEL k_g2_expand(const int32_t* raw, uint32_t u, int32_t* expanded, const uint32_t* d_u) {
+BN_KERNEL k_g2_expand(const int32_t* raw, uint32_t u, int32_t* expanded, const uint32_t* d_u, uint8_t* key_ok) {
   __shared__ int32_t stage[256 * 54];
   const uint32_t e0 = blockIdx.x * blockDim.x, e = e0 + threadIdx.x;
   uint32_t total = u * (uint32_t)BN_NEG_G2_LINES;
@@ -122,15 +122,29 @@
   const uint32_t here = total - e0 < 256u ? total - e0 : 256u;
   for (uint32_t x = threadIdx.x; x < here * 54u; x += 256u) stage[x] = raw[(size_t)e0 * 54u + x];
   __syncthreads();
+  if (threadIdx.x < 64u) {
+    const uint32_t g = 4u * threadIdx.x;
+    const bool lg = g < here;
+    Fp2 x[4];
+    bool zero[4];
+    for (int q = 0; q < 4; ++q) x[q] = fp2_load_limbs(Ws{stage, 1, ((lg ? g + (uint32_t)q : 0u) * 54u + 18u) * 4u, false});
+    fp2_inv4(x, zero);
+    if (lg) {
+      for (int q = 0; q < 4; ++q) {
+        int32_t* o = stage + (g + (uint32_t)q) * 54u + 18u;
+        BN_UNROLL for (int l = 0; l < NL; ++l) { o[l] = x[q].c0.l[l]; o[NL + l] = x[q].c1.l[l]; }
+        if (zero[q]) key_ok[(e0 + g + (uint32_t)q) / (uint32_t)BN_NEG_G2_LINES] = 0;
+      }
+    }
+  }
+  __syncthreads();
   const bool live = threadIdx.x < here;
   const uint32_t t = e % (uint32_t)BN_NEG_G2_LINES;
-  const Line a = line_from_table(BN_NEG_G2_LINE_TABLE[t]);
-  const Line b = line_load_limbs(Ws{stage, 1, (live ? threadIdx.x : 0u) * (uint32_t)(54 * 4), false});
+  const Ws bw = {stage, 1, (live ? threadIdx.x : 0u) * (uint32_t)(54 * 4), false};
+  const UnitPair up = unit_pair_of(BN_NEG_G2_UNIT_LINE_TABLE[t], fp2_load_limbs(bw), fp2_load_limbs_lazy(ws_at(bw, 18)), fp2_load_limbs(ws_at(bw, 36)));
   __syncthreads();
   BN_UNROLL for (int j = 0; j < 9; ++j) {
-    const Fp2 p = j == 0 ? fp2_mul(a.c0, b.c0) : j == 1 ? fp2_mul_xi(fp2_mul(a.c2, b.c2)) : j == 2 ? fp2_mul(a.c1, b.c1) : j == 3 ? fp2_mul(a.c1, b.c2)
-                : j == 4 ? fp2_mul(a.c2, b.c1) : j == 5 ? fp2_mul(a.c0, b.c1) : j == 6 ? fp2_mul(a.c1, b.c0) : j == 7 ? fp2_mul(a.c0, b.c2) : fp2_mul(a.c2, b.c0);
-    fp2_store_limbs_lazy(Ws{stage, 1, threadIdx.x * (uint32_t)(18 * 4), false}, p);
+    fp2_store_limbs_lazy(Ws{stage, 1, threadIdx.x * (uint32_t)(18 * 4), false}, unit_pair_entry(up, j));
     __syncthreads();
     for (uint32_t x = threadIdx.x; x < here * 18u; x += 256u) {
       const uint32_t lane = x / 18u, limb = x - 18u * lane;
diff --git a/bls-bn254_amd/csrc/k_miller_prep.hip b/bls-bn254_amd/csrc/k_miller_prep.hip
--- a/bls-bn254_amd/csrc/k_miller_prep.hip
+++ b/bls-bn254_amd/csrc/k_miller_prep.hip
@@ -4,7 +4,7 @@
 
 BN_KERNEL k_miller_prepared(const uint32_t* perm, const uint32_t* kid, const uint8_t* sigs, const int32_t* h_ws, size_t h_stride,
                             const int32_t* table, const uint8_t* key_ok, size_t n, int32_t* f_ws, uint8_t* flags) {
-  __shared__ int32_t inv_lds[81 * 256];
+  __shared__ int32_t inv_lds[72 * 256];
   const uint32_t s = blockIdx.x * blockDim.x + threadIdx.x;
   if (s >= n) return;
   const uint32_t i = perm[s], k = kid[i];
@@ -16,21 +16,10 @@
   const Ws hw = {const_cast<int32_t*>(h_ws), h_stride, i * 4u, true};
   const Fp xs = fp_norm(fp_select(sig_ok, sig.x, gp.x)), ys = fp_norm(fp_select(sig_ok, sig.y, gp.y));
   const Fp X = fp_load_mem(hw), Y = fp_load_mem(ws_at(hw, 9)), Z = fp_load_mem(ws_at(hw, 18));
-  fp_store_mem(inv, X); fp_store_mem(ws_at(inv, 9), Y); fp_store_mem(ws_at(inv, 18), Z);
-  fp_store_mem(ws_at(inv, 27), fp_mul(xs, X)); fp_store_mem(ws_at(inv, 36), fp_mul(ys, Y)); fp_store_mem(ws_at(inv, 45), fp_mul(xs, Z));
-  fp_store_mem(ws_at(inv, 54), fp_mul(ys, Z)); fp_store_mem(ws_at(inv, 63), fp_mul(ys, X)); fp_store_mem(ws_at(inv, 72), fp_mul(xs, Y));
+  bool inv_ok;
+  const bool unit = miller_unit_coords(xs, ys, X, Y, Z, inv, inv_ok);
   BN_MEM_FENCE;
   const Ws kt = {const_cast<int32_t*>(table), 1, k * (uint32_t)(BN_NEG_G2_LINES * 162 * 4), true};
-#ifdef BN_MILLER_UNIFORM_KEY
-  const uint32_t k0 = __builtin_amdgcn_readfirstlane(k);
-  Fp12 f;
-  if (__builtin_amdgcn_ballot_w64(k != k0) == 0)
-    f = miller_loop_prepared_uniform(inv, table + (size_t)k0 * (BN_NEG_G2_LINES * 162));
-  else
-    f = miller_loop_prepared(inv, kt);
-  fp12_store_limbs(Ws{f_ws, n, s * 4u, true}, f);
-#else
-  fp12_store_limbs(Ws{f_ws, n, s * 4u, true}, miller_loop_prepared(inv, kt));
-#endif
-  flags[s] = (sig_ok && key_ok[k] != 0) ? 1 : 0;
+  fp12_store_limbs(Ws{f_ws, n, s * 4u, true}, miller_loop_prepared_unit(inv, kt, unit));
+  flags[s] = (sig_ok && inv_ok && key_ok[k] != 0) ? 1 : 0;
 }
diff --git a/bls-bn254_amd/csrc/kernels.h b/bls-bn254_amd/csrc/kernels.h
--- a/bls-bn254_amd/csrc/kernels.h
+++ b/bls-bn254_amd/csrc/kernels.h
@@ -113,7 +113,7 @@
 __global__ void __launch_bounds__(256) k_kd_scatter(const uint32_t* kid, uint32_t n, uint32_t u, uint32_t* cursor, uint32_t* perm);
 BN_KERNEL k_g2_prepare(const uint8_t* pks, const uint32_t* keys, uint32_t u, int32_t* table, uint8_t* key_ok, const uint32_t* d_u);
 BN_KERNEL k_g2_prepare_quad(const uint8_t* pks, const uint32_t* keys, uint32_t u, int32_t* table, uint8_t* key_ok, const uint32_t* d_u);
-BN_KERNEL k_g2_expand(const int32_t* raw, uint32_t u, int32_t* expanded, const uint32_t* d_u);
+BN_KERNEL k_g2_expand(const int32_t* raw, uint32_t u, int32_t* expanded, const uint32_t* d_u, uint8_t* key_ok);
 __global__ void k_kd_decide(const uint32_t* cnt, uint32_t n, uint32_t cap, int small, uint32_t* res);
 __global__ void k_prep_unsort(const uint8_t* is_one, const uint8_t* flags, const uint32_t* perm, uint32_t n, uint8_t* valid);
 __global__ void __launch_bounds__(256) k_pack_bitmap(const uint8_t* valid, size_t n, uint8_t* bitmap);
diff --git a/bls-bn254_amd/csrc/pairing.h b/bls-bn254_amd/csrc/pairing.h
--- a/bls-bn254_amd/csrc/pairing.h
+++ b/bls-bn254_amd/csrc/pairing.h
@@ -370,20 +370,23 @@
   Fp12 t = fp12_mul(fp12_conj(a), inv);
   return fp12_mul(fp12_frob<2>(t), t);
 }
-BN_FUNC void fp_inv4(Fp x[4]) {
+template <bool POW_FALLBACK = true>
+BN_FUNC bool fp_inv4(Fp x[4]) {
   BN_CTX;
   bool z[4];
   Fp v[4], pre[4];
   for (int i = 0; i < 4; ++i) { z[i] = fp_is_zero(x[i]); v[i] = fp_select(z[i], fp_one(), fp_norm(x[i])); }
   pre[0] = v[0];
   for (int i = 1; i < 4; ++i) pre[i] = fp_mul(pre[i - 1], v[i]);
-  Fp inv = fp_inv(pre[3]);
+  bool done = true;
+  Fp inv = POW_FALLBACK ? fp_inv(pre[3]) : fp_inv_divsteps(pre[3], done);
   for (int i = 3; i >= 1; --i) {
     Fp r = fp_mul(inv, pre[i - 1]);
     inv = fp_mul(inv, v[i]);
     x[i] = fp_select(z[i], fp_zero(), r);
   }
   x[0] = fp_select(z[0], fp_zero(), inv);
+  return done;
 }
 BN_FUNC void fe_h1(const Fp12& x0, Fp12& a, Fp12& b) {
   a = fp12_cyclotomic_sqr(fp12_conj(x0));
@@ -597,52 +600,92 @@
   }
   return f;
 }
-#if defined(__HIP_DEVICE_COMPILE__)
-typedef const __attribute__((address_space(4))) int32_t* bn_const_i32p;
-#else
-typedef const int32_t* bn_const_i32p;
-#endif
-BN_INL Fp2 fp2_load_limbs_const(bn_const_i32p e) {
-  Fp2 c;
-  BN_UNROLL for (int k = 0; k < NL; ++k) { c.c0.l[k] = e[k]; c.c1.l[k] = e[9 + k]; }
-  BN_TRK(set_trk(c.c0, -4e-6, 1.0 + 4e-6, -0.02, 0.02, 1.2); set_trk(c.c1, -4e-6, 1.0 + 4e-6, -0.02, 0.02, 1.2);
-         check_actual(c.c0, "pair table entry"); check_actual(c.c1, "pair table entry");)
-  return c;
-}
-BN_FUNC Fp12 ell_pair_expanded_uniform(const Fp12& f, bn_const_i32p e, const Ws& cw) {
-  Fp X = fp_load_mem(cw), Y = fp_load_mem(ws_at(cw, 9)), Z = fp_load_mem(ws_at(cw, 18));
-  Fp xsX = fp_load_mem(ws_at(cw, 27)), ysY = fp_load_mem(ws_at(cw, 36)), xsZ = fp_load_mem(ws_at(cw, 45));
-  Fp ysZ = fp_load_mem(ws_at(cw, 54)), ysX = fp_load_mem(ws_at(cw, 63)), xsY = fp_load_mem(ws_at(cw, 72));
-  Fp6 l0 = {fp2_dot_fp(fp2_load_limbs_const(e), ysY, fp2_load_limbs_const(e + 18), Z),
-            fp2_mul_fp(fp2_load_limbs_const(e + 36), xsX),
-            fp2_dot_fp(fp2_load_limbs_const(e + 54), xsZ, fp2_load_limbs_const(e + 72), X)};
-  Fp2 l10 = fp2_dot_fp(fp2_load_limbs_const(e + 90), ysX, fp2_load_limbs_const(e + 108), xsY);
-  Fp2 l11 = fp2_dot_fp(fp2_load_limbs_const(e + 126), ysZ, fp2_load_limbs_const(e + 144), Y);
-  Fp6 v0 = fp6_mul(f.c0, l0);
+BN_FUNC void fp2_inv4(Fp2 x[4], bool zero[4]) {
+  BN_CTX;
+  Fp2 n[4];
+  Fp nu[4];
+  for (int i = 0; i < 4; ++i) { n[i] = fp2_norm(x[i]); nu[i] = fp_dot2(n[i].c0, n[i].c0, n[i].c1, n[i].c1); }
+  const bool done = fp_inv4<false>(nu);
+  for (int i = 0; i < 4; ++i) {
+    zero[i] = !done | fp_is_zero(nu[i]);
+    x[i] = {fp_mul(n[i].c0, nu[i]), fp_mul(fp_neg(n[i].c1), nu[i])};
+  }
+}
+BN_INL Fp2 fp2_unit_line_const(const int32_t* c) {
+  Fp2 r;
+  BN_UNROLL for (int i = 0; i < NL; ++i) { r.c0.l[i] = c[i]; r.c1.l[i] = c[NL + i]; }
+  BN_TRK(set_trk(r.c0, 0, 1, 0, 0.006, 1); set_trk(r.c1, 0, 1, 0, 0.006, 1);)
+  return r;
+}
+struct UnitPair { Fp2 a0, a4, u0, u4; };
+BN_FUNC UnitPair unit_pair_of(const int32_t* au, const Fp2& b0, const Fp2& b3_inv, const Fp2& b4) {
+  BN_CTX;
+  return {fp2_unit_line_const(au), fp2_unit_line_const(au + 18), fp2_mul(b0, b3_inv), fp2_mul(b4, b3_inv)};
+}
+BN_INL Fp2 unit_pair_entry(const UnitPair& q, int j) {
+  return j == 0 ? fp2_mul(q.a0, q.u0) : j == 1 ? fp2_mul_xi(fp2_mul(q.a4, q.u4)) : j == 2 ? fp2_one() : j == 3 ? q.u4 : j == 4 ? q.a4
+       : j == 5 ? q.a0 : j == 6 ? q.u0 : j == 7 ? fp2_mul(q.a0, q.u4) : fp2_mul(q.a4, q.u0);
+}
+BN_FUNC void line_pair_expand_unit(const int32_t* au, const Fp2& b0, const Fp2& b3_inv, const Fp2& b4, const Ws& out) {
+  BN_CTX;
+  const UnitPair q = unit_pair_of(au, b0, b3_inv, b4);
+  for (int j = 0; j < 9; ++j) fp2_store_limbs_lazy(ws_at(out, 18 * (size_t)j), unit_pair_entry(q, j));
+}
+BN_FUNC bool miller_unit_coords(const Fp& xs, const Fp& ys, const Fp& X, const Fp& Y, const Fp& Z, const Ws& cw, bool& ok) {
+  BN_CTX;
+  const Fp xsX = fp_mul(xs, X);
+  const bool unit = !fp_is_zero(xsX);
+  const Fp s = fp_select(unit, fp_inv_divsteps(xsX, ok), fp_one());
+  const Fp Xs = fp_mul(X, s), Ys = fp_mul(Y, s), Zs = fp_mul(Z, s);
+  fp_store_mem(cw, Ys); fp_store_mem(ws_at(cw, 9), Zs);
+  fp_store_mem(ws_at(cw, 18), fp_mul(ys, Ys)); fp_store_mem(ws_at(cw, 27), fp_mul(xs, Zs)); fp_store_mem(ws_at(cw, 36), fp_mul(ys, Zs));
+  fp_store_mem(ws_at(cw, 45), fp_mul(ys, Xs)); fp_store_mem(ws_at(cw, 54), fp_mul(xs, Ys)); fp_store_mem(ws_at(cw, 63), Xs);
+  return unit;
+}
+BN_FUNC Fp6 fp6_mul_unit1(const Fp6& a, const Fp2& b0, const Fp2& b2, bool unit) {
+  BN_CTX;
+  const Fp2 b1 = fp2_select(unit, fp2_one(), fp2_zero());
+  Fp2 v0 = fp2_mul(a.c0, b0), v1 = fp2_select(unit, a.c1, fp2_zero()), v2 = fp2_mul(a.c2, b2);
+  Fp2 w0 = fp2_mul(fp2_sub(a.c1, a.c2), fp2_sub(b1, b2));
+  Fp2 w1 = fp2_mul(fp2_sub(a.c0, a.c1), fp2_sub(b0, b1));
+  Fp2 w2 = fp2_mul(fp2_sub(a.c0, a.c2), fp2_sub(b0, b2));
+  Fp2 t0 = fp2_sub(fp2_add(v1, v2), w0);
+  Fp2 t1 = fp2_sub(fp2_add(v0, v1), w1);
+  Fp2 t2 = fp2_sub(fp2_add(v0, v2), w2);
+  return {fp2_add_mul_xi(v0, t0), fp2_add_mul_xi(t1, v2), fp2_norm(fp2_add(t2, v1))};
+}
+BN_FUNC Fp12 ell_pair_unit(const Fp12& f, const Ws& e, const Ws& cw, bool unit) {
+  BN_CTX;
+  Fp Y = fp_load_mem(cw), Z = fp_load_mem(ws_at(cw, 9)), ysY = fp_load_mem(ws_at(cw, 18)), xsZ = fp_load_mem(ws_at(cw, 27));
+  Fp ysZ = fp_load_mem(ws_at(cw, 36)), ysX = fp_load_mem(ws_at(cw, 45)), xsY = fp_load_mem(ws_at(cw, 54)), X = fp_load_mem(ws_at(cw, 63));
+  Fp2 l00 = fp2_dot_fp(fp2_load_limbs_lazy(e), ysY, fp2_load_limbs_lazy(ws_at(e, 18)), Z);
+  Fp2 l02 = fp2_dot_fp(fp2_load_limbs_lazy(ws_at(e, 54)), xsZ, fp2_load_limbs_lazy(ws_at(e, 72)), X);
+  Fp2 l10 = fp2_dot_fp(fp2_load_limbs_lazy(ws_at(e, 90)), ysX, fp2_load_limbs_lazy(ws_at(e, 108)), xsY);
+  Fp2 l11 = fp2_dot_fp(fp2_load_limbs_lazy(ws_at(e, 126)), ysZ, fp2_load_limbs_lazy(ws_at(e, 144)), Y);
+  Fp6 v0 = fp6_mul_unit1(f.c0, l00, l02, unit);
   Fp6 v1 = fp6_mul_by_01(f.c1, l10, l11);
-  Fp6 dl = {fp2_norm(fp2_sub(l10, l0.c0)), fp2_norm(fp2_sub(l11, l0.c1)), fp2_norm(fp2_neg(l0.c2))};
+  Fp6 dl = {fp2_norm(fp2_sub(l10, l00)), fp2_norm(fp2_sub(l11, fp2_select(unit, fp2_one(), fp2_zero()))), fp2_norm(fp2_neg(l02))};
   Fp6 w = fp6_mul(fp6_norm(fp6_sub(f.c0, f.c1)), dl);
   return {fp6_add_mul_v(v0, v1), fp6_norm(fp6_add(fp6_add(w, v0), v1))};
 }
-BN_FUNC Fp12 miller_loop_prepared_uniform(const Ws& inv, const int32_t* ktab_uniform) {
-  Fp12 f = fp12_one();
-  Ws p = inv;
-  bn_const_i32p kt = (bn_const_i32p)ktab_uniform;
+BN_FUNC Fp12 miller_loop_prepared_unit(const Ws& cw, const Ws& ktab_in, bool unit) {
+  Fp12 f = fp12_one();
+  Ws p = cw, kt = ktab_in;
   int ti = 0;
   for (int j = bnc::ATE_NAF_LEN - 2; j >= 0; --j) {
     f = fp12_sqr(f);
-    BN_OPAQUE(p);
-    f = ell_pair_expanded_uniform(f, kt + 162 * ti, p);
+    BN_OPAQUE(kt); BN_OPAQUE(p);
+    f = ell_pair_unit(f, ws_at(kt, 162 * (size_t)ti), p, unit);
     ++ti;
     if (ate_naf_digit(j) != 0) {
-      BN_OPAQUE(p);
-      f = ell_pair_expanded_uniform(f, kt + 162 * ti, p);
+      BN_OPAQUE(kt); BN_OPAQUE(p);
+      f = ell_pair_unit(f, ws_at(kt, 162 * (size_t)ti), p, unit);
       ++ti;
     }
   }
   for (int e = 0; e < 2; ++e) {
-    BN_OPAQUE(p);
-    f = ell_pair_expanded_uniform(f, kt + 162 * ti, p);
+    BN_OPAQUE(kt); BN_OPAQUE(p);
+    f = ell_pair_unit(f, ws_at(kt, 162 * (size_t)ti), p, unit);
     ++ti;
   }
   return f;
```
